# Team766/ros_vision

Hardware: AMD Instinct MI355X
Metric: frames/sec + p50 per-frame latency, 1280x720 AprilTag detect at 1/2/4/8 MI355X (higher is better)
Workload: dtype u8

## Files before the change

ros_vision_amd/csrc/at_api.cpp:

```cpp
#include <hip/hip_runtime.h>

#include <algorithm>
#include <chrono>
#include <cmath>
#include <cstdio>
#include <cstdlib>
#include <cstring>
#include <map>
#include <string>
#include <thread>
#include <vector>

#include "../../include/at_api.h"
#include "at_common.h"
#include "at_gp.h"
#include "at_mjpg.h"
#include "at_mjpg_entropy.h"

namespace at {
hipError_t launch_tap_sizes(const uint8_t* thr, const uint32_t* par, const uint32_t* size, uint32_t* out, int Wd,
                            int Hd, hipStream_t st);
hipError_t launch_tap_labels(const uint8_t* thr, const uint32_t* par, uint32_t* out, int Wd, int Hd, hipStream_t st);
hipError_t launch_gp_preprocess(const uint8_t* src, int w, int h, float* out, int ow, int oh, int c, hipStream_t st);
hipError_t launch_draw(const DrawPrim* prims, int n, uint32_t* last, uint8_t* bgr, int W, int H, hipStream_t st);
// ... 72 lines not shown
    fd.bitx[n] = (int8_t)(d / 2 + 1);
    fd.bity[n] = (int8_t)(d / 2 + 1);
  }
  return fd;
}
}

using namespace at;

static_assert(kMjpgInvalid == AT_E_INVALID && kMjpgUnsupported == AT_E_UNSUPPORTED && kMjpgOk == AT_OK,
              "at_mjpg.h carries the ABI's codes");
static_assert(kJpg420 == AT_JPEG_420 && kJpg422 == AT_JPEG_422 && kJpg444 == AT_JPEG_444 && AT_E_CAPACITY == -3,
              "at_mjpg.h carries the ABI's sampling codes");

enum { kCtlNpts, kCtlNpairs, kCtlNdets, kCtlNquads, kCtlStatus, kCtlNpent, kCtlNqcand, kCtlCclOvf, kCtlNlr,
       kCtlPerFrame };
enum { kCtlWorkhead = 0, kCtlQhead = 1, kCtlWorkheadSmall = 2, kCtlBlobPts = 3, kCtlNcls = 5,
       kCtlDetHead = kCtlNcls + kNumCls, kCtlDecDone = kCtlDetHead + 1, kCtlWorkheadMid = kCtlDecDone + 1,
       kCtlScalars = kCtlWorkheadMid + 1 };

static constexpr unsigned kTimingEventFlags = hipEventDisableSystemFence;

struct at_detector {
  at_config cfg;
  at_camera cam;
  Geom g;
  Params prm;
  int B;
  int device;
  int nblobwg;
  hipStream_t st;
  hipStream_t st2;
  hipEvent_t ev_fork, ev_join;
  DevBufs d;
  std::vector<void*> allocs;
  uint8_t* d_in;
  size_t in_stride;
  const uint8_t** h_ftab;
  uint32_t* d_ctrl;
  size_t ctrl_words;
  size_t kstamp_word;
  double wclk_khz;
  double kd_ms;
  long long kd_n;
  uint32_t* h_ctrl;
  DevDetection* h_dets;
  std::vector<int> res_idx, res_n;
  std::vector<const DevDetection*> res_base;
  std::vector<std::vector<DevDetection>> res_ovf;
  int last_nframes;
  int last_fmt;
  int last_gray;
  int last_sizes;
  int last_staged;
  int last_gp;
  int last_mj_color;
  int pending;
  hipEvent_t ev_done;
  hipEvent_t ev_ext;
  int use_graphs;
  std::map<int, hipGraphExec_t> graphs;
  struct SplitGraphs { hipGraphExec_t seg[3]; };
  std::map<int, SplitGraphs> split_graphs;
  std::vector<hipGraph_t> cap_segs;
  KernelTimer kt;
  double kt_ms;
  long long kt_n;
  int profiling;
  hipEvent_t ev_stage[kNumStages + 1];
  double stage_ms[kNumStages];
  long stage_batches;
  double host_wait_us, host_tail_us;
  DrawPrim* d_prims;
  size_t prims_cap;
  uint32_t* d_last;
  uint8_t* mj_host[2];
  uint8_t* d_mj;
  size_t mj_slot;
  int mj_cur;
  int mj_threads;
  std::vector<at::MjpgDecoder> mj_dec;
  std::vector<int> mj_rc;
  std::vector<size_t> mj_bytes;
  std::vector<uint8_t> mj_dense;
  uint64_t mj_stats[9];
  hipEvent_t ev_mj[3];
  int mj_timed;
  int mj_color;
  int mj_color_bufs;
  uint8_t* d_mj_planes;
  size_t mj_plane;
  uint8_t* d_mj_bgr;
  int mj_dev_ent;
  int mj_subseq;
  uint8_t* mj_ent_host[2];
  size_t mj_ent_cap;
  at::EntBufs ent;
  uint32_t* h_ent_info;
  int mj_ent_batch;
  hipEvent_t ev_ent[2];
  int mj_ent_timed;
  at::JpgBufs jpg;
  size_t jpg_out_cap;
  uint32_t* h_jpg_total;
  uint8_t jpg_hdr[at::kJpgHeaderMax];
  size_t jpg_hdr_len;
  int jpg_hdr_q, jpg_hdr_s;
  uint64_t jpg_stats[2];
  hipEvent_t ev_jpg[2];
  at::GpParseBufs gp;
  at::GpBox* h_gp_out;
  uint32_t* h_gp_info;
  uint64_t gp_stats[4];
  hipEvent_t ev_gp[2];
};

static const char* knob(const char* name) {
#ifdef AT_EXPERIMENTS
  return getenv(name);
#else
  (void)name;
  return nullptr;
#endif
}
static int knob_int(const char* name, int dflt) {
  const char* v = knob(name);
  return v ? atoi(v) : dflt;
}

static int hip_fail(hipError_t e) {
  if (e != hipSuccess) {
    fprintf(stderr, "at_api: HIP error %s\n", hipGetErrorString(e));
    return AT_E_HIP;
  }
  return AT_OK;
}
#define HIPCHK(x)                          \
  do {                                     \
    hipError_t e_ = (x);                   \
    if (e_ != hipSuccess) return hip_fail(e_); \
  } while (0)

extern "C" {

int at_abi_version(void) { return AT_ABI_VERSION; }

const char* at_strerror(int code) {
  switch (code) {
    case AT_OK: return "ok";
    case AT_E_INVALID: return "invalid argument or unsupported frame geometry";
    case AT_E_HIP: return "HIP runtime error";
    case AT_E_CAPACITY: return "frame exceeded a fixed capacity";
    case AT_E_FAMILY: return "unknown tag family";
    case AT_E_NOMEM: return "out of memory";
    case AT_E_UNSUPPORTED: return "unsupported JPEG stream (not baseline 8-bit 4:4:4 / 4:2:2 / 4:2:0 / gray)";
    default: return "unknown error";
  }
}

int at_family_num_known(const char* family) {
  const FamilyInfo* f = find_family(family);
  return f ? f->ncodes : AT_E_FAMILY;
}

int at_family_entry(const char* family, int i, int* id, uint64_t* code) {
  const FamilyInfo* f = find_family(family);
  if (!f) return AT_E_FAMILY;
  if (i < 0 || i >= f->ncodes) return AT_E_INVALID;
  if (id) *id = f->codes[i].id;
  if (code) *code = f->codes[i].code;
  return AT_OK;
}

int at_config_default(at_config* cfg, int width, int height) {
  if (!cfg) return AT_E_INVALID;
  memset(cfg, 0, sizeof(*cfg));
  cfg->width = width;
  cfg->height = height;
  cfg->family = "tag36h11";
  cfg->quad_decimate = 2.0f;
  cfg->refine_edges = 1;
  cfg->decode_sharpening = 0.25;
  cfg->min_white_black_diff = 5;
  cfg->min_cluster_pixels = 5;
  cfg->max_nmaxima = 10;
  cfg->max_line_fit_mse = 10.0f;
  cfg->cos_critical_rad = cos(10.0 * M_PI / 180.0);
  cfg->device = 0;
  cfg->max_batch = 1;
  cfg->tag_size = 0.1651;
  return AT_OK;
}

void at_destroy(at_detector* d) {
  if (!d) return;
  (void)hipSetDevice(d->device);
  if (d->st) (void)hipStreamSynchronize(d->st);
  if (d->st2) (void)hipStreamSynchronize(d->st2);
  for (auto& kv : d->graphs) (void)hipGraphExecDestroy(kv.second);
  d->graphs.clear();
  for (auto& kv : d->split_graphs)
    for (auto* g : kv.second.seg) (void)hipGraphExecDestroy(g);
  d->split_graphs.clear();
  for (void* p : d->allocs) (void)hipFree(p);
  if (d->h_ftab) (void)hipHostFree(d->h_ftab);
  if (d->h_ctrl) (void)hipHostFree(d->h_ctrl);
  if (d->h_dets) (void)hipHostFree(d->h_dets);
  if (d->d_prims) (void)hipFree(d->d_prims);
  if (d->d_last) (void)hipFree(d->d_last);
  for (uint8_t* p : d->mj_host)
    if (p) (void)hipHostFree(p);
  for (hipEvent_t e : d->ev_mj)
    if (e) (void)hipEventDestroy(e);
  for (uint8_t* p : d->mj_ent_host)
    if (p) (void)hipHostFree(p);
  if (d->h_ent_info) (void)hipHostFree(d->h_ent_info);
  for (hipEvent_t e : d->ev_ent)
    if (e) (void)hipEventDestroy(e);
  for (hipEvent_t e : d->ev_jpg)
    if (e) (void)hipEventDestroy(e);
  if (d->h_jpg_total) (void)hipHostFree(d->h_jpg_total);
  for (hipEvent_t e : d->ev_gp)
    if (e) (void)hipEventDestroy(e);
  if (d->h_gp_out) (void)hipHostFree(d->h_gp_out);
  if (d->h_gp_info) (void)hipHostFree(d->h_gp_info);
  if (d->ev_done) (void)hipEventDestroy(d->ev_done);
  if (d->ev_ext) (void)hipEventDestroy(d->ev_ext);
  for (int i = 0; i <= kNumStages; i++)
    if (d->ev_stage[i]) (void)hipEventDestroy(d->ev_stage[i]);
  if (d->kt.t0) (void)hipEventDestroy(d->kt.t0);
  if (d->kt.t1) (void)hipEventDestroy(d->kt.t1);
  if (d->ev_fork) (void)hipEventDestroy(d->ev_fork);
  if (d->ev_join) (void)hipEventDestroy(d->ev_join);
  if (d->st2) (void)hipStreamDestroy(d->st2);
  if (d->st) (void)hipStreamDestroy(d->st);
  delete d;
}

int at_create(const at_config* cfg, const at_camera* cam, at_detector** out) {
  if (!cfg || !cam || !out) return AT_E_INVALID;
  *out = nullptr;
  const FamilyInfo* fam = find_family(cfg->family);
  if (!fam || fam->ncodes > kMaxCodes) return AT_E_FAMILY;
  const int W = cfg->width, H = cfg->height;
  if (W <= 16 || H <= 16 || W % 8 || H % 8 || (long)W * H >= (1L << 22)) return AT_E_INVALID;
  if (cfg->quad_decimate != 2.0f || cfg->max_nmaxima != 10 || cfg->max_batch < 1 || cfg->max_batch > kMaxBatch)
    return AT_E_INVALID;
  if (2 * (W + H) > kSortCap) return AT_E_INVALID;
  int ndev = 0;
  if (hipGetDeviceCount(&ndev) != hipSuccess || ndev <= cfg->device) return AT_E_HIP;
  at_detector* d = new at_detector();
  d->cfg = *cfg;
  d->cfg.family = fam->name;
  d->cam = *cam;
  d->device = cfg->device;
  d->B = cfg->max_batch;
  d->mj_threads = 1;
  d->mj_subseq = at::kEntSubseqDefault;
  Geom& g = d->g;
  g.W = W; g.H = H; g.Wd = W / 2; g.Hd = H / 2;
  g.TW = g.Wd / 4; g.TH = g.Hd / 4;
  g.BW = g.Wd / 2; g.BH = g.Hd / 2;
  g.ctw = d->B < kWideBlobMaxBatch ? 32 : 64;
  if (knob("AT_CCL_TILE")) g.ctw = knob_int("AT_CCL_TILE", 64) == 32 ? 32 : 64;
  g.nlarge = g.ctw == 32 ? std::max(kNumLargeCls, std::min(kNumCls, knob_int("AT_NLARGE", kNumLargeCls)))
                        : kNumLargeCls;
  g.CTX = (g.Wd + g.ctw - 1) / g.ctw;
  g.CTY = (g.Hd + kCclTileH - 1) / kCclTileH;
  g.merge_cap = g.ctw == 64 ? std::min(kMergeCapMax, 80 * g.CTX * g.CTY) : 0;
  g.merge_lds = std::min(g.merge_cap * 12 + 8192, kMergeLdsMax);
  if (g.CTX * g.CTY > kMaxCclTiles) {
    at_destroy(d);
    return AT_E_INVALID;
  }
  g.cap_pts = 4 * (g.Wd - 2) * (g.Hd - 2);
  g.BTX = (g.Wd - 2 + 63) / 64;
  g.BTY = (g.Hd - 2 + 4 * kBndRows - 1) / (4 * kBndRows);
  g.ntb = g.BTX * g.BTY;
  g.bnd_region = kBndPts;
  g.bnd_region = std::max(kBndStage, std::min(kBndPts, knob_int("AT_BND_REGION", kBndPts)));
  if (g.ntb > kMaxTilesPerFrame) {
    at_destroy(d);
    return AT_E_INVALID;
  }
  g.min_cluster = (uint32_t)std::max(24, cfg->min_cluster_pixels);
  g.max_cluster = (uint32_t)(2 * (W + H));
  g.min_tag_width = std::max(3, (fam->d + 2) / 2);
  Params& p = d->prm;
  p.min_white_black_diff = cfg->min_white_black_diff;
  p.max_line_fit_mse = cfg->max_line_fit_mse;
  p.cos_critical_rad = cfg->cos_critical_rad;
  p.decode_sharpening = cfg->decode_sharpening;
  p.refine_edges = cfg->refine_edges;
  p.fx = cam->fx; p.fy = cam->fy; p.cx = cam->cx; p.cy = cam->cy;
  p.k1 = cam->k1; p.k2 = cam->k2; p.p1 = cam->p1; p.p2 = cam->p2; p.k3 = cam->k3;
  p.diag_stop = knob_int("AT_DIAG_BLOB_STOP", 0);
  p.probe = knob_int("AT_PHASE_PROBE", 0);
  p.taps = 0;
  p.wide_blob = knob_int("AT_WIDE_BLOB", 0);
  p.pipe_stop = knob_int("AT_DIAG_PIPE_STOP", 0);
  p.lblob_wg = knob("AT_LBLOB_WG") ? std::max(16, knob_int("AT_LBLOB_WG", 0)) : 0;
  p.sblob_wg = knob("AT_SBLOB_WG") ? std::max(16, knob_int("AT_SBLOB_WG", 0)) : 0;
  p.dec_wg = knob("AT_DEC_WG") ? std::max(16, knob_int("AT_DEC_WG", 0)) : 0;
  p.fam = family_desc(*fam);
  d->use_graphs = !knob_int("AT_NO_GRAPH", 0);
  if (!(cfg->tag_size >= 0) || !std::isfinite(cfg->tag_size)) {
    at_destroy(d);
    return AT_E_INVALID;
  }
  p.tag_size = cfg->tag_size;

  auto fail = [&](int code) {
    at_destroy(d);
    return code;
  };
  if (hipSetDevice(d->device) != hipSuccess) return fail(AT_E_HIP);
  if (hipStreamCreateWithFlags(&d->st, hipStreamNonBlocking) != hipSuccess) return fail(AT_E_HIP);
  if (hipEventCreateWithFlags(&d->ev_done, hipEventDisableTiming) != hipSuccess) return fail(AT_E_HIP);
  if (hipEventCreateWithFlags(&d->ev_ext, hipEventDisableTiming) != hipSuccess) return fail(AT_E_HIP);
  const bool fork = d->B < kWideBlobMaxBatch && !knob_int("AT_NO_FORK", 0);
  if (fork && hipStreamCreateWithFlags(&d->st2, hipStreamNonBlocking) != hipSuccess) return fail(AT_E_HIP);
  if (hipEventCreateWithFlags(&d->ev_fork, hipEventDisableTiming) != hipSuccess) return fail(AT_E_HIP);
  if (hipEventCreateWithFlags(&d->ev_join, hipEventDisableTiming) != hipSuccess) return fail(AT_E_HIP);
  d->kt.stage = -1;
  d->kt.split = nullptr;
  d->kt.ctx = nullptr;
  if (hipEventCreateWithFlags(&d->kt.t0, kTimingEventFlags) != hipSuccess ||
      hipEventCreateWithFlags(&d->kt.t1, kTimingEventFlags) != hipSuccess)
    return fail(AT_E_HIP);
  int ncu = 0;
  (void)hipDeviceGetAttribute(&ncu, hipDeviceAttributeMultiprocessorCount, d->device);
  int wclk = 0;
  (void)hipDeviceGetAttribute(&wclk, hipDeviceAttributeWallClockRate, d->device);
  d->wclk_khz = wclk > 0 ? (double)wclk : 100000.0;
  d->nblobwg = std::max(64, ncu * 2);
  if (knob("AT_BLOB_WG")) d->nblobwg = std::max(16, knob_int("AT_BLOB_WG", 0));

  const size_t B = (size_t)d->B;
  const size_t npix = (size_t)W * H, nd = (size_t)g.Wd * g.Hd, nt = (size_t)g.TW * g.TH * 2;
  bool oom = false;
  auto dalloc = [&](size_t bytes) -> void* {
    void* ptr = nullptr;
    if (hipMalloc(&ptr, std::max<size_t>(bytes, 256)) != hipSuccess) {
      oom = true;
      return nullptr;
    }
    d->allocs.push_back(ptr);
    return ptr;
  };
  d->in_stride = (npix * 3 + 255) & ~(size_t)255;
  d->d_in = (uint8_t*)dalloc(B * d->in_stride);
  DevBufs& b = d->d;
  b.gray = (uint8_t*)dalloc(B * npix);
  b.dec = (uint8_t*)dalloc(B * nd);
  b.mm = (uint8_t*)dalloc(B * nt);
  b.thr = (uint8_t*)dalloc(B * nd);
  b.par = (uint32_t*)dalloc(B * nd * 4);
  b.lroot = (uint32_t*)dalloc(B * (size_t)g.CTX * g.CTY * kCclTileNodesMax * 4);
  b.nlroot = (uint32_t*)dalloc(B * (size_t)g.CTX * g.CTY * 4);
  b.lcnt = (uint32_t*)dalloc(B * (size_t)g.CTX * g.CTY * kCclTileNodesMax * 4);
  b.cdesc = (uint32_t*)dalloc(B * (size_t)g.CTX * g.CTY * CclDesc::kWords * 4);
  b.size = (uint32_t*)dalloc(B * nd * 4);
  const size_t ntb = (size_t)g.ntb;
  b.pts = (uint64_t*)dalloc(B * ntb * (size_t)g.bnd_region * 8);
  b.tcnt = (uint32_t*)dalloc(B * ntb * 4);
  b.tent = (uint32_t*)dalloc(B * ntb * 4);
  b.grp = (uint32_t*)dalloc(B * g.cap_pts * 4);
  b.keys = (uint64_t*)dalloc(B * g.cap_pts * 8);
  b.pent_key = (uint64_t*)dalloc(B * ntb * kLdsPairSlots * 8);
  b.pent_cnt = (uint32_t*)dalloc(B * ntb * kLdsPairSlots * 4);
  b.povf_key = (uint64_t*)dalloc(B * kPairEntCap * 8);
  b.povf_cnt = (uint32_t*)dalloc(B * kPairEntCap * 4);
  b.ht_key = (uint64_t*)dalloc(B * kHashSlots * 8);
  b.ht_cnt = (uint32_t*)dalloc(B * kHashSlots * 4);
  b.ht_rank = (uint32_t*)dalloc(B * kHashSlots * 4);
  b.ht_off = (uint32_t*)dalloc(B * kHashSlots * 4);
  b.ht_cur = (uint32_t*)dalloc(B * kHashSlots * 4);
  b.pair_cnt = (uint32_t*)dalloc(B * kMaxPairs * 4);
  b.pair_off = (uint32_t*)dalloc(B * kMaxPairs * 4);
  b.pair_sel = (uint32_t*)dalloc(B * kMaxPairs * 4);
  b.wcap = (uint32_t)(B * kMaxPairs);
  b.work = (uint32_t*)dalloc((size_t)kNumCls * B * kMaxPairs * 4);
  b.probe = (uint64_t*)dalloc(kProbeWords * 8);
  b.dets = (DevDetection*)dalloc(B * kMaxDets * sizeof(DevDetection));
  b.det_work = (uint32_t*)dalloc(B * kMaxDets * 4);
  b.quads = (QuadRecord*)dalloc(B * kMaxPairs * sizeof(QuadRecord));
  b.qpend = (QuadPend*)dalloc(B * kMaxPairs * sizeof(QuadPend));
  d->kstamp_word = (kCtlPerFrame * B + kCtlScalars + 1) & ~(size_t)1;
  d->ctrl_words = d->kstamp_word + 5;
  d->d_ctrl = (uint32_t*)dalloc(((d->ctrl_words * 4 + 15) / 16) * 16);
  b.npts = d->d_ctrl + kCtlNpts * B;
  b.npairs = d->d_ctrl + kCtlNpairs * B;
  b.ndets = d->d_ctrl + kCtlNdets * B;
  b.nquads = d->d_ctrl + kCtlNquads * B;
  b.status = d->d_ctrl + kCtlStatus * B;
  b.npent = d->d_ctrl + kCtlNpent * B;
  b.qc_words = (uint32_t)(B * kQcStride);
  b.nqcand = (uint32_t*)dalloc((size_t)b.qc_words * 4);
  b.ccl_ovf = d->d_ctrl + kCtlCclOvf * B;
  b.nlr_tot = d->d_ctrl + kCtlNlr * B;
  uint32_t* sc = d->d_ctrl + kCtlPerFrame * B;
  b.workhead = sc + kCtlWorkhead;
  b.qhead = sc + kCtlQhead;
  b.workhead_small = sc + kCtlWorkheadSmall;
  b.workhead_mid = sc + kCtlWorkheadMid;
  b.blob_pts = sc + kCtlBlobPts;
  b.ncls = sc + kCtlNcls;
  b.det_head = sc + kCtlDetHead;
  b.dec_done = sc + kCtlDecDone;
  b.kt_stage = -1;
  b.kstamp = reinterpret_cast<uint64_t*>(d->d_ctrl + d->kstamp_word);
  b.kgrid = d->d_ctrl + d->kstamp_word + 4;
  b.kwg_cap = (uint32_t)(B * 1024 + 4096);
  b.kwg = (uint64_t*)dalloc((size_t)b.kwg_cap * 2 * 8);
  b.qcand_cap = (uint32_t)(B * kQuadCandPerFrame);
  b.qcand = (QuadCand*)dalloc((size_t)b.qcand_cap * sizeof(QuadCand));
  b.s_pk = (uint64_t*)dalloc((size_t)2 * d->nblobwg * (kSortCap / 2) * 8);
  b.rsamp = (double*)dalloc((size_t)decode_grid(d->nblobwg, d->B) * 2 * (kMaxRefineSamples - kLdsRefine) * 8);
  if (oom) return fail(AT_E_NOMEM);
  if (prepare_kernels(g) != hipSuccess) return fail(AT_E_HIP);
  if (hipHostMalloc((void**)&d->h_ftab, B * sizeof(void*), hipHostMallocMapped | hipHostMallocCoherent) != hipSuccess)
    return fail(AT_E_NOMEM);
  if (hipHostGetDevicePointer((void**)&b.frames, (void*)d->h_ftab, 0) != hipSuccess) return fail(AT_E_HIP);
  d->res_idx.assign(B * kMaxDets, 0);
  d->res_n.assign(B, 0);
  d->res_base.assign(B, nullptr);
  d->res_ovf.resize(B);
  if (hipHostMalloc((void**)&d->h_ctrl, d->ctrl_words * 4, hipHostMallocMapped) != hipSuccess) return fail(AT_E_NOMEM);
  if (hipHostMalloc((void**)&d->h_dets, B * kDetPoolPerFrame * sizeof(DevDetection), hipHostMallocMapped) != hipSuccess)
    return fail(AT_E_NOMEM);
  if (hipHostGetDevicePointer((void**)&b.hdets, d->h_dets, 0) != hipSuccess ||
      hipHostGetDevicePointer((void**)&b.hctrl, d->h_ctrl, 0) != hipSuccess)
    return fail(AT_E_HIP);
  b.ctrl = d->d_ctrl;
  b.ctrl_words = (uint32_t)d->ctrl_words;
  {
    std::vector<uint64_t> codes(fam->ncodes);
    std::vector<int32_t> ids(fam->ncodes);
    for (int i = 0; i < fam->ncodes; i++) {
      codes[i] = fam->codes[i].code;
      ids[i] = fam->codes[i].id;
    }
    uint64_t* dc = (uint64_t*)dalloc(codes.size() * 8);
    int32_t* di = (int32_t*)dalloc(ids.size() * 4);
    if (oom) return fail(AT_E_NOMEM);
    if (hipMemcpy(dc, codes.data(), codes.size() * 8, hipMemcpyHostToDevice) != hipSuccess ||
        hipMemcpy(di, ids.data(), ids.size() * 4, hipMemcpyHostToDevice) != hipSuccess)
      return fail(AT_E_HIP);
    b.book_code = dc;
    b.book_id = di;
  }
  if (hipMemsetAsync(b.size, 0, B * nd * 4, d->st) != hipSuccess) return fail(AT_E_HIP);
  if (hipStreamSynchronize(d->st) != hipSuccess) return fail(AT_E_HIP);
  *out = d;
  return AT_OK;
}

}

static bool seg_intersect(const double* a0, const double* a1, const double* b0, const double* b1) {
  const double ux = a1[0] - a0[0], uy = a1[1] - a0[1];
  const double vx = b1[0] - b0[0], vy = b1[1] - b0[1];
  const double den = ux * vy - uy * vx;
  if (fabs(den) < 1e-12) return false;
  const double t = ((b0[0] - a0[0]) * vy - (b0[1] - a0[1]) * vx) / den;
  const double w = ((b0[0] - a0[0]) * uy - (b0[1] - a0[1]) * ux) / den;
  return t >= 0 && t <= 1 && w >= 0 && w <= 1;
}
static bool poly_contains(const double poly[4][2], const double* pt) {
  bool inside = false;
  for (int i = 0, j = 3; i < 4; j = i++) {
    if (((poly[i][1] > pt[1]) != (poly[j][1] > pt[1])) &&
        (pt[0] < (poly[j][0] - poly[i][0]) * (pt[1] - poly[i][1]) / (poly[j][1] - poly[i][1]) + poly[i][0]))
      inside = !inside;
  }
  return inside;
}
static bool poly_overlap(const double a[4][2], const double b[4][2]) {
  for (int i = 0; i < 4; i++)
    for (int j = 0; j < 4; j++)
      if (seg_intersect(a[i], a[(i + 1) & 3], b[j], b[(j + 1) & 3])) return true;
  return poly_contains(a, b[0]) || poly_contains(b, a[0]);
}
static int prefer_smaller(int pref, double q0, double q1) {
  if (pref) return pref;
  if (q0 < q1) return -1;
  if (q1 < q0) return 1;
  return 0;
}

static void write_detection(const DevDetection& v, at_detection* o) {
  o->id = v.id;
  o->hamming = v.hamming;
  o->decision_margin = v.decision_margin;
  memcpy(o->H, v.H, sizeof(o->H));
  memcpy(o->c, v.c, sizeof(o->c));
  memcpy(o->p, v.p, sizeof(o->p));
}

static int host_tail(const DevDetection* cand, int* idx, int ncand, at_detection* out, int cap) {
  std::stable_sort(idx, idx + ncand, [&](int a, int b) { return cand[a].blob_rank < cand[b].blob_rank; });
  int n = ncand;
  for (int i0 = 0; i0 < n; i0++) {
    for (int i1 = i0 + 1; i1 < n; i1++) {
      const DevDetection& a = cand[idx[i0]];
      const DevDetection& b = cand[idx[i1]];
      if (a.id != b.id) continue;
      if (!poly_overlap(a.p, b.p)) continue;
      int pref = 0;
      pref = prefer_smaller(pref, a.hamming, b.hamming);
      pref = prefer_smaller(pref, -a.decision_margin, -b.decision_margin);
      for (int k = 0; k < 3; k++) pref = prefer_smaller(pref, a.H[k], b.H[k]);
      if (pref < 0) {
        if (i1 < n - 1) idx[i1] = idx[n - 1];
        n--;
        i1--;
      } else {
        if (i0 < n - 1) idx[i0] = idx[n - 1];
        n--;
        i0--;
        break;
      }
    }
  }
  std::stable_sort(idx, idx + n, [&](int a, int b) { return cand[a].id < cand[b].id; });
  for (int i = 0; i < n && i < cap; i++) write_detection(cand[idx[i]], out + i);
  return n;
}

static hipError_t record_sequence(at_detector* d, int nframes, int fmt, hipStream_t st, hipEvent_t* ev,
                                  const KernelTimer* kt) {
  hipError_t e;
  DevBufs b = d->d;
  b.kt_stage = kt ? kt->stage : -1;
  if ((e = launch_pipeline(b, d->g, d->prm, nframes, fmt, d->nblobwg, st, ev, d->st2, d->ev_fork, d->ev_join, kt)))
    return e;
  if (d->prm.tag_size > 0) return hipSuccess;
  return hipMemcpyAsync(d->h_ctrl, d->d_ctrl, d->ctrl_words * 4, hipMemcpyDeviceToHost, st);
}

static hipError_t split_capture(void* ctx, int ) {
  at_detector* d = (at_detector*)ctx;
  hipGraph_t g = nullptr;
  hipError_t e = hipStreamEndCapture(d->st, &g);
  if (e != hipSuccess) return e;
  d->cap_segs.push_back(g);
  return hipStreamBeginCapture(d->st, hipStreamCaptureModeThreadLocal);
}

static hipError_t instantiate(hipGraph_t g, hipGraphExec_t* exec) {
  const hipError_t e = hipGraphInstantiate(exec, g, nullptr, nullptr, 0);
  (void)hipGraphDestroy(g);
  return e;
}

static int enqueue_split(at_detector* d, int nframes, int fmt) {
  hipStream_t st = d->st;
  const int key = (nframes * 4 + fmt) * 32 + d->kt.stage;
  auto it = d->split_graphs.find(key);
  if (it == d->split_graphs.end()) {
    d->cap_segs.clear();
    KernelTimer kt = d->kt;
    kt.split = split_capture;
    kt.ctx = d;
    HIPCHK(hipStreamBeginCapture(st, hipStreamCaptureModeThreadLocal));
    hipError_t rec = record_sequence(d, nframes, fmt, st, nullptr, &kt);
    hipGraph_t last = nullptr;
    const hipError_t end = hipStreamEndCapture(st, &last);
    if (last) d->cap_segs.push_back(last);
    if (rec == hipSuccess && end == hipSuccess && d->cap_segs.size() != 3) rec = hipErrorInvalidValue;
    if (rec != hipSuccess || end != hipSuccess) {
      for (auto* g : d->cap_segs) (void)hipGraphDestroy(g);
      d->cap_segs.clear();
      HIPCHK(rec);
      HIPCHK(end);
    }
    at_detector::SplitGraphs sg{};
    hipError_t inst = hipSuccess;
    for (int i = 0; i < 3; i++) {
      const hipError_t r = instantiate(d->cap_segs[i], &sg.seg[i]);
      if (r != hipSuccess && inst == hipSuccess) inst = r;
    }
    d->cap_segs.clear();
    if (inst != hipSuccess) {
      for (auto* g : sg.seg)
        if (g) (void)hipGraphExecDestroy(g);
      HIPCHK(inst);
    }
    it = d->split_graphs.emplace(key, sg).first;
  }
  HIPCHK(hipGraphLaunch(it->second.seg[0], st));
  HIPCHK(hipEventRecord(d->kt.t0, st));
  HIPCHK(hipGraphLaunch(it->second.seg[1], st));
  HIPCHK(hipEventRecord(d->kt.t1, st));
  HIPCHK(hipGraphLaunch(it->second.seg[2], st));
  return AT_OK;
}

static int enqueue(at_detector* d, int nframes, int fmt) {
  hipStream_t st = d->st;
  const bool timed = d->kt.stage >= 0;
  const bool timed_on_fork = timed && d->st2 && (d->kt.stage == 8 || d->kt.stage == 9);
  if (d->profiling || !d->use_graphs || timed_on_fork) {
    HIPCHK(record_sequence(d, nframes, fmt, st, d->profiling ? d->ev_stage : nullptr, timed ? &d->kt : nullptr));
  } else if (timed) {
    const int rc = enqueue_split(d, nframes, fmt);
    if (rc != AT_OK) return rc;
  } else {
    const int key = nframes * 4 + fmt;
    auto it = d->graphs.find(key);
    if (it == d->graphs.end()) {
      hipGraph_t graph = nullptr;
      HIPCHK(hipStreamBeginCapture(st, hipStreamCaptureModeThreadLocal));
      const hipError_t rec = record_sequence(d, nframes, fmt, st, nullptr, nullptr);
      const hipError_t end = hipStreamEndCapture(st, &graph);
      HIPCHK(rec);
      HIPCHK(end);
      hipGraphExec_t exec = nullptr;
      HIPCHK(instantiate(graph, &exec));
      it = d->graphs.emplace(key, exec).first;
    }
    HIPCHK(hipGraphLaunch(it->second, st));
  }
  HIPCHK(hipEventRecord(d->ev_done, st));
  d->last_nframes = nframes;
  d->last_fmt = fmt;
  d->last_gray = fmt == AT_FMT_BGR8 || d->prm.taps;
  d->last_sizes = d->g.ctw == 32 || d->prm.taps;
  d->last_gp = d->prm.gp_c && fmt == AT_FMT_BGR8;
  d->last_mj_color = 0;
  d->mj_ent_batch = 0;
  d->pending = 1;
  return AT_OK;
}

static double now_us() {
  return std::chrono::duration<double, std::micro>(std::chrono::steady_clock::now().time_since_epoch()).count();
}

static int collect(at_detector* d, at_detection* out, int cap_per_frame, int* n_per_frame) {
  if (!d->pending) return AT_E_INVALID;
  const double t0 = now_us();
  HIPCHK(hipEventSynchronize(d->ev_done));
  const double t1 = now_us();
  d->host_wait_us += t1 - t0;
  d->pending = 0;
  if (d->profiling) {
    for (int i = 0; i < kNumStages; i++) {
      float ms = 0;
      HIPCHK(hipEventElapsedTime(&ms, d->ev_stage[i], d->ev_stage[i + 1]));
      d->stage_ms[i] += ms;
    }
    d->stage_batches++;
  }
  if (d->mj_timed) {
    float ms = 0;
    HIPCHK(hipEventElapsedTime(&ms, d->ev_mj[0], d->ev_mj[1]));
    d->mj_stats[4] = (uint64_t)((double)ms * 1e6);
    if (d->mj_timed == 2) {
      HIPCHK(hipEventElapsedTime(&ms, d->ev_mj[1], d->ev_mj[2]));
      d->mj_stats[5] = (uint64_t)((double)ms * 1e6);
    }
    d->mj_timed = 0;
  }
  if (d->mj_ent_timed) {
    float ms = 0;
    HIPCHK(hipEventElapsedTime(&ms, d->ev_ent[0], d->ev_ent[1]));
    d->mj_stats[6] = (uint64_t)((double)ms * 1e6);
    d->mj_ent_timed = 0;
  }
  if (d->mj_ent_batch) {
    uint32_t most = 0;
    for (int f = 0; f < d->last_nframes; f++) most = std::max(most, d->h_ent_info[(size_t)f * at::kEntInfoWords + 1]);
    d->mj_stats[8] = most;
  }
  if (d->kt.stage >= 0) {
    float ms = 0;
    HIPCHK(hipEventElapsedTime(&ms, d->kt.t0, d->kt.t1));
    d->kt_ms += ms;
    d->kt_n++;
    uint64_t st[2];
    memcpy(st, d->h_ctrl + d->kstamp_word, sizeof(st));
    st[0] = ~st[0];
    if (st[1] > st[0] && st[0] && d->wclk_khz > 0) {
      d->kd_ms += (double)(st[1] - st[0]) / d->wclk_khz;
      d->kd_n++;
    }
  }
  const int B = d->B;
  int rc = AT_OK;
  bool bad_entropy = false;
  const int nf = d->last_nframes;
  int* cnt = d->res_n.data();
  for (int f = 0; f < nf; f++) {
    cnt[f] = 0;
    if (n_per_frame) n_per_frame[f] = 0;
  }
  for (int f = 0; f < nf; f++) {
    const uint32_t status = d->h_ctrl[kCtlStatus * B + f];
    const int ncand = (int)std::min<uint32_t>(d->h_ctrl[kCtlNdets * B + f], kMaxDets);
    int* idx = d->res_idx.data() + (size_t)f * kMaxDets;
    int n = 0;
    if (status & kStatusPairsCapped) rc = AT_E_CAPACITY;
    if (d->mj_ent_batch && d->h_ent_info[(size_t)f * at::kEntInfoWords]) {
      bad_entropy = true;
    } else if (status & (kStatusPairsOverflow | kStatusHashFull | kStatusPointsOverflow | kStatusQuadsOverflow | kStatusDetsOverflow)) {
      rc = AT_E_CAPACITY;
    } else {
      const DevDetection* cand = d->h_dets + (size_t)f * kDetPoolPerFrame;
      if (ncand > kDetPoolPerFrame) {
        std::vector<DevDetection>& v = d->res_ovf[f];
        v.resize(ncand);
        HIPCHK(hipMemcpyAsync(v.data(), d->d.dets + (size_t)f * kMaxDets, ncand * sizeof(DevDetection),
                              hipMemcpyDeviceToHost, d->st));
        HIPCHK(hipStreamSynchronize(d->st));
        cand = v.data();
      }
      d->res_base[f] = cand;
      for (int i = 0; i < ncand; i++) idx[i] = i;
      n = host_tail(cand, idx, ncand, out ? out + (size_t)f * cap_per_frame : nullptr, out ? cap_per_frame : 0);
    }
// ... 1156 lines not shown
```

ros_vision_amd/csrc/at_common.h:

```cpp
#pragma once

#include <hip/hip_runtime.h>
#include <stdint.h>

#include "at_detmath.h"

namespace at {

template <int TW>
struct CclTile {
  static constexpr int W = TW, H = 32;
  static constexpr int BW = TW / 2, BH = H / 2;
  static constexpr int NT = BW * BH;
  static constexpr int NODES = 3 * NT;
  static constexpr int ROW_NODES = 3 * BW;
};
constexpr int kCclTileH = 32;
constexpr int kCclTileNodesMax = CclTile<64>::NODES;
constexpr int kHashSlots = 4096;
constexpr int kHashBits = 12;
constexpr int kPairEntCap = 65536;
constexpr int kBndRows = 4;
constexpr int kBndPts = 64 * 4 * kBndRows * 4;
constexpr int kBndStage = 2048;
constexpr int kLdsPairSlots = 512;
constexpr uint32_t kTileNarrow = 0x80000000u;
constexpr int kMaxTilesPerFrame = 1024;
constexpr int kMaxCclTiles = 1024;
struct CclDesc {
  static constexpr int Tthr = 0, Bthr = 16, Lthr = 32, Rthr = 40;
  static constexpr int TsF = 48, TsL = 64, TsR = 80, BsF = 96, BsL = 112, BsR = 128;
  static constexpr int LsF = 144, LsL = 152, RsF = 160, RsR = 168;
  static constexpr int kWords = 176;
};
constexpr int kMergeCapMax = 15360;
constexpr int kMergeLdsMax = kMergeCapMax * 10;
constexpr int kMaxPairs = 4096;
constexpr int kSortCap = 8192;
constexpr int kBlobThreads = 256;
constexpr int kWideBlobMaxBatch = 8;
constexpr int kSmallBlob = 512;
constexpr int kNMaxima = 10;
constexpr int kMaxRefineSamples = 1536;
#ifndef AT_LDS_REFINE
#define AT_LDS_REFINE 256
#endif
constexpr int kLdsRefine = AT_LDS_REFINE;
constexpr int kDecodeGridPerBlobWg = 8;
inline int decode_grid(int nblobwg, int B) {
  const int hi = nblobwg * kDecodeGridPerBlobWg, want = 64 * B;
  return nblobwg * 2 > (want < hi ? want : hi) ? nblobwg * 2 : (want < hi ? want : hi);
}

constexpr int kNumStages = 12;
constexpr const char* kStageNames[kNumStages] = {"k_pre",   "k_thr_ccl", "k_ccl_merge", "k_ccl_roots",
                                                 "k_boundary", "k_pairs", "k_group",     "k_extents",
                                                 "k_blob_small", "k_blob", "k_decode",   "k_pose"};

constexpr int kNumCls = 7;
constexpr int kNumLargeCls = 3;

constexpr uint32_t kStatusPairsOverflow = 1u;
constexpr uint32_t kStatusHashFull = 2u;
constexpr uint32_t kStatusDetsOverflow = 4u;
constexpr uint32_t kStatusPointsOverflow = 8u;
constexpr uint32_t kStatusQuadsOverflow = 16u;
constexpr uint32_t kStatusPairsCapped = 32u;
constexpr int kMaxBatch = 256;
constexpr int kQcStride = 32;
constexpr int kQuadCandPerFrame = kMaxPairs;
constexpr int kMaxDets = kQuadCandPerFrame;
constexpr int kDetPoolPerFrame = 128;
constexpr int kMaxCodes = 1024;
constexpr int kMaxFamilyBits = 64;

struct FamilyDesc {
  int nbits;
  int width_at_border;
  int total_width;
  int reversed_border;
  int ncodes;
  int8_t bitx[kMaxFamilyBits], bity[kMaxFamilyBits];
};

struct Geom {
  int W, H, Wd, Hd;
  int TW, TH;
  int BW, BH;
  int CTX, CTY;
  int ctw;
  int merge_cap;
  int merge_lds;
  int nlarge;
  int bnd_region;
  int cap_pts;
  int BTX, BTY, ntb;
  uint32_t min_cluster;
  uint32_t max_cluster;
  int min_tag_width;
};

struct Params {
  int min_white_black_diff;
  float max_line_fit_mse;
  double cos_critical_rad;
  double decode_sharpening;
  int refine_edges;
  double fx, fy, cx, cy, k1, k2, p1, p2, k3;
  int diag_stop;
  double tag_size;
  int probe;
  int taps;
  int wide_blob;
  int pipe_stop;
  int lblob_wg;
  int sblob_wg;
  int dec_wg;
  FamilyDesc fam;
  int gp_w, gp_h, gp_c;
};
constexpr int kProbeWords = 256;

#ifdef AT_EXPERIMENTS
#define AT_DIAG_STOP(prm, n) ((prm).diag_stop == (n))
#define AT_PIPE_STOP(prm) ((prm).pipe_stop)
#define AT_PROBE_ON(prm) ((prm).probe != 0)
#define AT_DIAG_ANY(prm) ((prm).diag_stop != 0)
#else
#define AT_DIAG_STOP(prm, n) false
#define AT_PIPE_STOP(prm) 0
#define AT_PROBE_ON(prm) false
#define AT_DIAG_ANY(prm) false
#endif

struct KernelTimer {
  int stage;
  hipEvent_t t0, t1;
  hipError_t (*split)(void* ctx, int which);
  void* ctx;
};

struct DevDetection {
  int32_t id;
  int16_t hamming;
  uint16_t frame;
  float decision_margin;
  int32_t blob_rank;
  double H[9];
  double c[2];
  double p[4][2];
  double pose_R[9];
  double pose_t[3];
  double pose_err[2];
};

struct QuadCand {
  uint32_t frame, rank;
  float p[4][2];
};

struct QuadRecord {
  uint32_t blob_index, valid, accepted;
  uint16_t indices[4];
  float corners[4][2];
};

struct Moments {
  int32_t Mx, My, W;
  int64_t Mxx, Myy, Mxy;
  int32_t N;
};

struct QuadPend {
  float fit[4][4];
  uint32_t blob_index, valid;
  uint16_t indices[4];
};
static_assert(sizeof(QuadPend) == 80, "QuadPend: 80 B per kept blob");

struct DrawPrim {
  double x0, y0, x1, y1;
  uint8_t bgr[3];
};

struct JpgBufs {
  int16_t* coef;
  const uint32_t* tab;
  uint32_t* blen;
  uint32_t* bits;
  size_t row_words;
  uint32_t* row_raw;
  uint32_t* row_len;
  uint8_t* out;
  uint32_t* total;
};

struct DevBufs {
  const uint8_t* const* frames;
  uint8_t* gray;
  uint8_t* dec;
  uint8_t* mm;
  uint8_t* thr;
  uint32_t* par;
  uint32_t* lroot;
  uint32_t* nlroot;
  uint32_t* lcnt;
  uint32_t* cdesc;
  uint32_t* ccl_ovf;
  uint32_t* nlr_tot;
  uint32_t* size;
  uint64_t* pts;
  uint32_t* tcnt;
  uint32_t* tent;
  uint32_t* grp;
  uint64_t* keys;
  uint64_t* pent_key;
  uint32_t* pent_cnt;
  uint64_t* povf_key;
  uint32_t* povf_cnt;
  uint32_t* npent;
  uint64_t* ht_key;
  uint32_t* ht_cnt;
  uint32_t* ht_rank;
  uint32_t* ht_off;
  uint32_t* ht_cur;
  uint32_t* pair_cnt;
  uint32_t* pair_off;
  uint32_t* pair_sel;
  uint32_t* work;
  uint32_t wcap;
  DevDetection* dets;
  uint32_t* det_work;
  uint32_t* det_head;
  uint32_t* dec_done;
  DevDetection* hdets;
  uint32_t* hctrl;
  uint32_t* ctrl;
  uint32_t ctrl_words;
  QuadRecord* quads;
  QuadPend* qpend;
  uint32_t* npts;
  uint32_t* npairs;
  uint32_t* ndets;
  uint32_t* nquads;
  uint32_t* status;
  uint32_t* ncls;
  uint32_t* workhead;
  uint64_t* probe;
  uint32_t* blob_pts;
  uint32_t* workhead_small;
  uint32_t* workhead_mid;
  uint32_t* nqcand;
  uint32_t qc_words;
  uint32_t* qhead;
  QuadCand* qcand;
  uint32_t qcand_cap;
  double* rsamp;
  const uint64_t* book_code;
  const int32_t* book_id;
  float* gp_out;
  int32_t kt_stage;
  uint64_t* kstamp;
  uint32_t* kgrid;
  uint64_t* kwg;
  uint32_t kwg_cap;
  uint64_t* s_pk;
};

}
```

ros_vision_amd/csrc/at_kernels.hip:

```cpp
#include <limits>
#include <hip/hip_runtime.h>

#include <float.h>
#include <math.h>
#include <stdint.h>

#include "at_common.h"
#include "at_gp.h"
#include "at_mjpg.h"
#include "at_mjpg_entropy.h"
#include "at_pose.h"


namespace at {

__device__ __forceinline__ uint32_t lane_id() { return __lane_id(); }
__device__ __attribute__((noinline)) float det_atan2f_call(float y, float x) { return det_atan2f(y, x); }

__device__ __forceinline__ uint64_t mix_hash(uint64_t k) {
  return (k * 0x9E3779B97F4A7C15ull) >> (64 - kHashBits);
}

__device__ __forceinline__ int dx_of(int dxy) { return dxy == 3 ? -1 : (dxy == 2 ? 0 : 1); }
__device__ __forceinline__ int dy_of(int dxy) { return dxy == 0 ? 0 : 1; }
// ... 1901 lines not shown
      const uint32_t key = lds ? e : 0x80000000u + lane;
      const bool same = lds && wave_shr1(key, 0xffffffffu) == key;
      const uint64_t same_mask = __ballot(same);
      const bool head = lds && !same;
      uint32_t start = 0;
      if (head) start = atomicAdd(&s_cur[e], run_len(same_mask, lane));
      const uint64_t heads = __ballot(head);
      const int hl = (heads & le) ? 63 - __builtin_clzll(heads & le) : (int)lane;
      const uint32_t s0 = (uint32_t)__shfl((int)start, hl);
      if (lds) grp[base + s0 + (lane - (uint32_t)hl)] = narrow_bits(w);
      else if (valid && base == kGrpFallback) place_global(b.pent_key[tb * kLdsPairSlots + e], narrow_bits(w));
    };
#pragma unroll
    for (int k = 0; k < kGrpPre; k++) {
      const uint32_t i = 2 * (tid + 256 * k);
      place((uint32_t)pv[k], i < n);
      place((uint32_t)(pv[k] >> 32), i + 1 < n);
    }
    for (uint32_t i0 = 512 * kGrpPre; i0 < n; i0 += 256) {
      const uint32_t i = i0 + tid;
      place(i < n ? pw[i] : 0u, i < n);
    }
    return;
  }
  for (int i = tid; i < 2 * kGrpEnt; i += 256) s_hk[i] = 0;
  __syncthreads();
  if (tid < kGrpEnt && (uint32_t)tid < ne && ebase != kGrpFallback) {
    s_base[tid] = ebase;
    s_cur[tid] = 0;
    uint32_t h = (uint32_t)(mix_hash(ekey) & (2 * kGrpEnt - 1));
    while (true) {
      const uint64_t prev = atomicCAS((unsigned long long*)&s_hk[h], 0ull, (unsigned long long)ekey);
      if (prev == 0) {
        s_he[h] = (uint32_t)tid;
        break;
      }
      h = (h + 1) & (2 * kGrpEnt - 1);
    }
  }
  __syncthreads();
  const uint32_t lane = lane_id();
  const uint64_t le = lane == 63 ? ~0ull : ((2ull << lane) - 1);
  auto place = [&](uint64_t key, bool valid) {
    const uint64_t r01 = key >> 24;
    uint32_t e = 0xffffffffu;
    if (valid) {
      uint32_t h = (uint32_t)(mix_hash(r01) & (2 * kGrpEnt - 1));
      for (int probe = 0; probe < 2 * kGrpEnt; probe++) {
        const uint64_t k = s_hk[h];
        if (k == r01) { e = s_he[h]; break; }
        if (k == 0) break;
        h = (h + 1) & (2 * kGrpEnt - 1);
      }
    }
    const uint32_t base = e != 0xffffffffu ? s_base[e] : kGrpDrop;
    const bool lds = base != kGrpDrop;
    const uint32_t ek = lds ? e : 0x80000000u + lane;
    const bool same = lds && wave_shr1(ek, 0xffffffffu) == ek;
    const uint64_t same_mask = __ballot(same);
    const bool head = lds && !same;
    uint32_t start = 0;
    if (head) start = atomicAdd(&s_cur[e], run_len(same_mask, lane));
    const uint64_t heads = __ballot(head);
    const int hl = (heads & le) ? 63 - __builtin_clzll(heads & le) : (int)lane;
    const uint32_t s0 = (uint32_t)__shfl((int)start, hl);
    if (lds) grp[base + s0 + (lane - (uint32_t)hl)] = (uint32_t)key & 0xffffffu;
    else if (valid && e == 0xffffffffu) place_global(r01, (uint32_t)key & 0xffffffu);
  };
#pragma unroll
  for (int k = 0; k < kGrpPre; k++) place(pv[k], (uint32_t)(tid + 256 * k) < n);
  for (uint32_t i0 = 256 * kGrpPre; i0 < n; i0 += 256) {
    const uint32_t i = i0 + tid;
    place(i < n ? pts[i] : 0ull, i < n);
  }
}

struct Ext {
  uint32_t min_x, min_y, max_x, max_y, count;
  int32_t gx_sum, gy_sum;
  int64_t pg_sum;
};

__device__ __forceinline__ double ext_cx(const Ext& e) { return (double)((float)(e.min_x + e.max_x) * 0.5f) + 0.05118; }
__device__ __forceinline__ double ext_cy(const Ext& e) {
  return (double)((float)(e.min_y + e.max_y) * 0.5f) + -0.028581;
}
__device__ __forceinline__ float ext_dot(const Ext& e) {
  const int64_t t = e.pg_sum * 2 - (int64_t)((int)(e.min_x + e.max_x) * e.gx_sum) -
                    (int64_t)((int)(e.min_y + e.max_y) * e.gy_sum);
  const double a = (double)t * 0.5;
  const double bq = 0.05118 * (double)e.gx_sum;
  const double c = 0.028581 * (double)e.gy_sum;
  return (float)(a - bq + c);
}

__device__ __forceinline__ int32_t lf_weight(int32_t gx, int32_t gy) {
  const uint32_t sq = (uint32_t)(gx * gx + gy * gy);
  uint32_t r = (uint32_t)__builtin_amdgcn_sqrtf((float)sq);
  r -= r * r > sq ? 1u : 0u;
  r += (r + 1) * (r + 1) <= sq ? 1u : 0u;
  return (int32_t)r + 1;
}

__device__ __forceinline__ void line_normal(float d, float c, float h, double* lp23) {
  const float nx1 = d - h, ny1 = c;
  const float M1 = nx1 * nx1 + ny1 * ny1;
  const float nx2 = c, ny2 = -d - h;
  const float M2 = nx2 * nx2 + ny2 * ny2;
  float nx, ny;
  if (M1 > M2) { nx = nx1; ny = ny1; } else { nx = nx2; ny = ny2; }
  const float len = det_hypotf(nx, ny);
  lp23[0] = (double)(nx / len);
  lp23[1] = (double)(ny / len);
}

__device__ void fit_line(const Moments& m, double* lp01, double* lp23, double* err, double* mse, float* pre = nullptr) {
  const int64_t W = m.W;
  const int64_t Cxx = (int64_t)((uint64_t)m.Mxx * (uint64_t)W - (uint64_t)((int64_t)m.Mx * (int64_t)m.Mx));
  const int64_t Cxy = (int64_t)((uint64_t)m.Mxy * (uint64_t)W - (uint64_t)((int64_t)m.Mx * (int64_t)m.My));
  const int64_t Cyy = (int64_t)((uint64_t)m.Myy * (uint64_t)W - (uint64_t)((int64_t)m.My * (int64_t)m.My));
  const float d = (float)(Cxx - Cyy), c = (float)(2 * Cxy);
  const float px = (float)m.Mx / (float)(m.W * 2), py = (float)m.My / (float)(m.W * 2);
  if (pre) {
    pre[0] = d; pre[1] = c; pre[2] = px; pre[3] = py;
    return;
  }
  const float h = det_hypotf(d, c);
  const float e8 = (float)((double)(W * W) * 8.0);
  const float eig = ((float)(Cxx + Cyy) - h) / e8;
  if (lp01) {
    lp01[0] = (double)px;
    lp01[1] = (double)py;
  }
  if (lp23) line_normal(d, c, h, lp23);
  *err = (double)((float)m.N * eig);
  *mse = (double)eig;
}

template <int NT>
__device__ __forceinline__ void team_sync() {
  if constexpr (NT == 64) {
    __builtin_amdgcn_fence(__ATOMIC_RELEASE, "wavefront");
    __builtin_amdgcn_wave_barrier();
    __builtin_amdgcn_fence(__ATOMIC_ACQUIRE, "wavefront");
  } else {
    __syncthreads();
  }
}

template <int NT>
__device__ __forceinline__ int team_rank() {
  return NT == 64 ? (int)lane_id() : (int)threadIdx.x;
}

template <int NT, typename T, typename Op>
__device__ T team_reduce(T v, Op op, T* s_tmp) {
  if constexpr (NT == 64) {
    return wave_reduce(v, op);
  } else {
    return block_reduce(v, op, s_tmp, NT / 64);
  }
}

template <int NT, typename T>
__device__ T team_incl_scan(T v, T* s_tmp, T* total) {
  if constexpr (NT == 64) {
    v = wave_incl_scan(v, AddOp(), T(0));
    *total = wave_read(v, 63);
    return v;
  } else {
    return block_incl_scan(v, s_tmp, total, NT / 64);
  }
}

template <typename T, int NT>
__device__ void team_bitonic_sort(T* s, int n) {
  const int r = team_rank<NT>();
  for (int k = 2; k <= n; k <<= 1) {
    for (int j = k >> 1; j > 0; j >>= 1) {
      for (int i = r; i < n; i += NT) {
        const int ixj = i ^ j;
        if (ixj > i) {
          const T a = s[i], c = s[ixj];
          const bool up = (i & k) == 0;
          if ((a > c) == up) {
            s[i] = c;
            s[ixj] = a;
          }
        }
      }
      team_sync<NT>();
    }
  }
}


__device__ void redistort(const Params& p, double* x, double* y) {
  const double xP = (*x - p.cx) / p.fx, yP = (*y - p.cy) / p.fy;
  const double rSq = xP * xP + yP * yP;
  const double lin = 1 + p.k1 * rSq + p.k2 * rSq * rSq + p.k3 * rSq * rSq * rSq;
  const double xPP = xP * lin + 2 * p.p1 * xP * yP + p.p2 * (rSq + 2 * xP * xP);
  const double yPP = yP * lin + p.p1 * (rSq + 2 * yP * yP) + 2 * p.p2 * xP * yP;
  *x = xPP * p.fx + p.cx;
  *y = yPP * p.fy + p.cy;
}

__device__ void undistort(const Params& p, double* u, double* v) {
  const double xPP = (*u - p.cx) / p.fx, yPP = (*v - p.cy) / p.fy;
  double xP = xPP, yP = yPP;
  const double x0 = xP, y0 = yP;
  double prev_x, prev_y;
  int it = 0;
  do {
    prev_x = xP;
    prev_y = yP;
    const double rSq = xP * xP + yP * yP;
    const double rad = 1 + (p.k1 * rSq) + (p.k2 * rSq * rSq) + (p.k3 * rSq * rSq * rSq);
    const double rinv = 1 / rad;
    const double tdx = 2 * p.p1 * xP * yP + p.p2 * (rSq + p.k3 * rSq * rSq * rSq);
    const double tdy = p.p1 * (rSq + 2 * yP * yP) + 2 * p.p2 * xP * yP;
    xP = (x0 - tdx) * rinv;
    yP = (y0 - tdy) * rinv;
    if (it > 100) break;
    it++;
  } while (fabs(xP - prev_x) > 1e-6 || fabs(yP - prev_y) > 1e-6);
  *u = xP * p.fx + p.cx;
  *v = yP * p.fy + p.cy;
}

__device__ void hproject(const double* H, double x, double y, double* ox, double* oy) {
  const double xx = H[0] * x + H[1] * y + H[2];
  const double yy = H[3] * x + H[4] * y + H[5];
  const double zz = H[6] * x + H[7] * y + H[8];
  *ox = xx / zz;
  *oy = yy / zz;
}

__device__ int homography_wave(const float (*qc)[2], double* A, double* H) {
  const int lane = (int)lane_id();
  for (int e = lane; e < 72; e += 64) {
    const int row = e / 9, col = e % 9, i = row >> 1;
    const double c0 = (i == 0 || i == 3) ? -1 : 1, c1 = (i == 0 || i == 1) ? -1 : 1;
    const double c2 = qc[i][0], c3 = qc[i][1];
    const int k = (row & 1) ? col - 3 : col;
    const double cz = (row & 1) ? c3 : c2;
    double v = 0;
    if (k == 0) v = c0;
    else if (k == 1) v = c1;
    else if (k == 2) v = 1;
    if (col == 6) v = -c0 * cz;
    else if (col == 7) v = -c1 * cz;
    else if (col == 8) v = cz;
    A[e] = v;
  }
  team_sync<64>();
  for (int col = 0; col < 8; col++) {
    double v = -1.0;
    int row = 64;
    if (lane < 8 - col) {
      row = col + lane;
      v = fabs(A[row * 9 + col]);
      if (!(v > 0.0)) { v = -1.0; row = 64; }
    }
#pragma unroll
    for (int d = 1; d < 8; d <<= 1) {
      const double ov = __shfl_xor(v, d);
      const int orow = __shfl_xor(row, d);
      if (ov > v || (ov == v && orow < row)) { v = ov; row = orow; }
    }
    v = __shfl(v, 0);
    row = __shfl(row, 0);
    if (!(v >= 1e-10)) return -1;
    if (row != col && lane <= 8 - col) {
      const int i = col + lane;
      const double t = A[col * 9 + i];
      A[col * 9 + i] = A[row * 9 + i];
      A[row * 9 + i] = t;
    }
    team_sync<64>();
    const int nc = 8 - col;
    if (lane < (7 - col) * nc) {
      const int i = col + 1 + lane / nc, j = col + 1 + lane % nc;
      const double fct = A[i * 9 + col] / A[col * 9 + col];
      A[i * 9 + j] -= fct * A[col * 9 + j];
    }
    team_sync<64>();
  }
  double x[8];
#pragma unroll
  for (int col = 7; col >= 0; col--) {
    double sum = 0;
#pragma unroll
    for (int i = col + 1; i < 8; i++) sum += A[col * 9 + i] * x[i];
    x[col] = (A[col * 9 + 8] - sum) / A[col * 9 + col];
  }
#pragma unroll
  for (int k = 0; k < 8; k++)
    if (lane == k) H[k] = x[k];
  if (lane == 8) H[8] = 1;
  team_sync<64>();
  return 0;
}

struct GrayModel {
  double A[3][3], B[3], C[3];
};
__device__ void gm_add(GrayModel& g, double x, double y, double gray) {
  g.A[0][0] += x * x; g.A[0][1] += x * y; g.A[0][2] += x;
  g.A[1][1] += y * y; g.A[1][2] += y; g.A[2][2] += 1;
  g.B[0] += x * gray; g.B[1] += y * gray; g.B[2] += gray;
}
__device__ void gm_solve(GrayModel& g) {
  const double* A = &g.A[0][0];
  double L[9], M[9];
  L[0] = sqrt(A[0]); L[3] = A[1] / L[0]; L[6] = A[2] / L[0];
  L[4] = sqrt(A[4] - L[3] * L[3]); L[7] = (A[5] - L[3] * L[6]) / L[4];
  L[8] = sqrt(A[8] - L[6] * L[6] - L[7] * L[7]);
  M[0] = 1 / L[0]; M[3] = -L[3] * M[0] / L[4]; M[4] = 1 / L[4];
  M[6] = (-L[6] * M[0] - L[7] * M[3]) / L[8]; M[7] = -L[7] * M[4] / L[8]; M[8] = 1 / L[8];
  const double t0 = M[0] * g.B[0];
  const double t1 = M[3] * g.B[0] + M[4] * g.B[1];
  const double t2 = M[6] * g.B[0] + M[7] * g.B[1] + M[8] * g.B[2];
  g.C[0] = M[0] * t0 + M[3] * t1 + M[6] * t2;
  g.C[1] = M[4] * t1 + M[7] * t2;
  g.C[2] = M[8] * t2;
}
__device__ __forceinline__ double gm_interp(const GrayModel& g, double x, double y) {
  return g.C[0] * x + g.C[1] * y + g.C[2];
}

__constant__ uint8_t c_combo[210][4] = {{0,1,2,3},{0,1,2,4},{0,1,2,5},{0,1,2,6},{0,1,2,7},{0,1,2,8},{0,1,2,9},{0,1,3,4},{0,1,3,5},{0,1,3,6},{0,1,3,7},{0,1,3,8},{0,1,3,9},{0,1,4,5},{0,1,4,6},{0,1,4,7},{0,1,4,8},{0,1,4,9},{0,1,5,6},{0,1,5,7},{0,1,5,8},{0,1,5,9},{0,1,6,7},{0,1,6,8},{0,1,6,9},{0,1,7,8},{0,1,7,9},{0,1,8,9},{0,2,3,4},{0,2,3,5},{0,2,3,6},{0,2,3,7},{0,2,3,8},{0,2,3,9},{0,2,4,5},{0,2,4,6},{0,2,4,7},{0,2,4,8},{0,2,4,9},{0,2,5,6},{0,2,5,7},{0,2,5,8},{0,2,5,9},{0,2,6,7},{0,2,6,8},{0,2,6,9},{0,2,7,8},{0,2,7,9},{0,2,8,9},{0,3,4,5},{0,3,4,6},{0,3,4,7},{0,3,4,8},{0,3,4,9},{0,3,5,6},{0,3,5,7},{0,3,5,8},{0,3,5,9},{0,3,6,7},{0,3,6,8},{0,3,6,9},{0,3,7,8},{0,3,7,9},{0,3,8,9},{0,4,5,6},{0,4,5,7},{0,4,5,8},{0,4,5,9},{0,4,6,7},{0,4,6,8},{0,4,6,9},{0,4,7,8},{0,4,7,9},{0,4,8,9},{0,5,6,7},{0,5,6,8},{0,5,6,9},{0,5,7,8},{0,5,7,9},{0,5,8,9},{0,6,7,8},{0,6,7,9},{0,6,8,9},{0,7,8,9},{1,2,3,4},{1,2,3,5},{1,2,3,6},{1,2,3,7},{1,2,3,8},{1,2,3,9},{1,2,4,5},{1,2,4,6},{1,2,4,7},{1,2,4,8},{1,2,4,9},{1,2,5,6},{1,2,5,7},{1,2,5,8},{1,2,5,9},{1,2,6,7},{1,2,6,8},{1,2,6,9},{1,2,7,8},{1,2,7,9},{1,2,8,9},{1,3,4,5},{1,3,4,6},{1,3,4,7},{1,3,4,8},{1,3,4,9},{1,3,5,6},{1,3,5,7},{1,3,5,8},{1,3,5,9},{1,3,6,7},{1,3,6,8},{1,3,6,9},{1,3,7,8},{1,3,7,9},{1,3,8,9},{1,4,5,6},{1,4,5,7},{1,4,5,8},{1,4,5,9},{1,4,6,7},{1,4,6,8},{1,4,6,9},{1,4,7,8},{1,4,7,9},{1,4,8,9},{1,5,6,7},{1,5,6,8},{1,5,6,9},{1,5,7,8},{1,5,7,9},{1,5,8,9},{1,6,7,8},{1,6,7,9},{1,6,8,9},{1,7,8,9},{2,3,4,5},{2,3,4,6},{2,3,4,7},{2,3,4,8},{2,3,4,9},{2,3,5,6},{2,3,5,7},{2,3,5,8},{2,3,5,9},{2,3,6,7},{2,3,6,8},{2,3,6,9},{2,3,7,8},{2,3,7,9},{2,3,8,9},{2,4,5,6},{2,4,5,7},{2,4,5,8},{2,4,5,9},{2,4,6,7},{2,4,6,8},{2,4,6,9},{2,4,7,8},{2,4,7,9},{2,4,8,9},{2,5,6,7},{2,5,6,8},{2,5,6,9},{2,5,7,8},{2,5,7,9},{2,5,8,9},{2,6,7,8},{2,6,7,9},{2,6,8,9},{2,7,8,9},{3,4,5,6},{3,4,5,7},{3,4,5,8},{3,4,5,9},{3,4,6,7},{3,4,6,8},{3,4,6,9},{3,4,7,8},{3,4,7,9},{3,4,8,9},{3,5,6,7},{3,5,6,8},{3,5,6,9},{3,5,7,8},{3,5,7,9},{3,5,8,9},{3,6,7,8},{3,6,7,9},{3,6,8,9},{3,7,8,9},{4,5,6,7},{4,5,6,8},{4,5,6,9},{4,5,7,8},{4,5,7,9},{4,5,8,9},{4,6,7,8},{4,6,7,9},{4,6,8,9},{4,7,8,9},{5,6,7,8},{5,6,7,9},{5,6,8,9},{5,7,8,9},{6,7,8,9}};

__constant__ uint8_t c_colex[210] = {0,1,7,28,84,2,8,29,85,13,34,90,49,105,140,3,9,30,86,14,35,91,50,106,141,18,39,95,54,110,145,64,120,155,175,4,10,31,87,15,36,92,51,107,142,19,40,96,55,111,146,65,121,156,176,22,43,99,58,114,149,68,124,159,179,74,130,165,185,195,5,11,32,88,16,37,93,52,108,143,20,41,97,56,112,147,66,122,157,177,23,44,100,59,115,150,69,125,160,180,75,131,166,186,196,25,46,102,61,117,152,71,127,162,182,77,133,168,188,198,80,136,171,191,201,205,6,12,33,89,17,38,94,53,109,144,21,42,98,57,113,148,67,123,158,178,24,45,101,60,116,151,70,126,161,181,76,132,167,187,197,26,47,103,62,118,153,72,128,163,183,78,134,169,189,199,81,137,172,192,202,206,27,48,104,63,119,154,73,129,164,184,79,135,170,190,200,82,138,173,193,203,207,83,139,174,194,204,208,209};

struct LineFitOut {
  double err, mse;
  double p01[2], p23[2];
};

template <bool kP01, bool kP23>
__device__ __forceinline__ LineFitOut fit_line_v(const Moments& m) {
  LineFitOut o;
  fit_line(m, kP01 ? o.p01 : nullptr, kP23 ? o.p23 : nullptr, &o.err, &o.mse);
  return o;
}

struct Mom6 {
  uint32_t Mx, My, W;
  uint64_t Mxx, Myy, Mxy;
};
__device__ __forceinline__ Mom6 mom_zero() { return Mom6{0, 0, 0, 0, 0, 0}; }
__device__ __forceinline__ void mom_add(Mom6& a, const Mom6& c) {
  a.Mx += c.Mx; a.My += c.My; a.W += c.W; a.Mxx += c.Mxx; a.Myy += c.Myy; a.Mxy += c.Mxy;
}
__device__ __forceinline__ void mom_sub(Mom6& a, const Mom6& c) {
  a.Mx -= c.Mx; a.My -= c.My; a.W -= c.W; a.Mxx -= c.Mxx; a.Myy -= c.Myy; a.Mxy -= c.Mxy;
}
__device__ __forceinline__ Mom6 mom_shfl(const Mom6& m, int src) {
  Mom6 r;
  r.Mx = __shfl(m.Mx, src); r.My = __shfl(m.My, src); r.W = __shfl(m.W, src);
  r.Mxx = __shfl(m.Mxx, src); r.Myy = __shfl(m.Myy, src); r.Mxy = __shfl(m.Mxy, src);
  return r;
}
__device__ __forceinline__ Mom6 mom_shfl_up(const Mom6& m, int d) {
  Mom6 r;
  r.Mx = __shfl_up(m.Mx, d); r.My = __shfl_up(m.My, d); r.W = __shfl_up(m.W, d);
  r.Mxx = __shfl_up(m.Mxx, d); r.Myy = __shfl_up(m.Myy, d); r.Mxy = __shfl_up(m.Mxy, d);
  return r;
}

constexpr int kKeyTheta = 32;

__device__ __forceinline__ uint32_t compact_word(uint64_t sk) {
  return (uint32_t)((sk >> 10) & 0x3ff) | ((uint32_t)((sk >> 20) & 0x3ff) << 10) | ((uint32_t)((sk >> 30) & 3) << 20) |
         ((uint32_t)(sk & 0x1ff) << 22);
}

__device__ __forceinline__ Mom6 point_mom(uint32_t cw) {
  const int dxy = (int)((cw >> 20) & 3);
  const uint32_t ix2 = (cw & 0x3ff) * 2 + dx_of(dxy) + 1;
  const uint32_t iy2 = ((cw >> 10) & 0x3ff) * 2 + dy_of(dxy) + 1;
  const uint32_t Wt = cw >> 22;
  Mom6 m;
  m.Mx = Wt * ix2;
  m.My = Wt * iy2;
  m.W = Wt;
  m.Mxx = (uint64_t)(int64_t)(int32_t)(Wt * ix2 * ix2);
  m.Mxy = (uint64_t)(int64_t)(int32_t)(Wt * ix2 * iy2);
  m.Myy = (uint64_t)(int64_t)(int32_t)(Wt * iy2 * iy2);
  return m;
}

__device__ __forceinline__ Moments to_moments(const Mom6& s, int32_t N) {
  Moments m;
  m.Mx = (int32_t)s.Mx; m.My = (int32_t)s.My; m.W = (int32_t)s.W;
  m.Mxx = (int64_t)s.Mxx; m.Myy = (int64_t)s.Myy; m.Mxy = (int64_t)s.Mxy;
  m.N = N;
  return m;
}

__device__ __forceinline__ float window_err(const Mom6& s, int32_t N) {
  const Moments m = to_moments(s, N);
  const uint64_t Wl = (uint32_t)m.W;
  const int64_t Cxx = (int64_t)((uint64_t)m.Mxx * Wl - (uint64_t)((int64_t)m.Mx * (int64_t)m.Mx));
  const int64_t Cxy = (int64_t)((uint64_t)m.Mxy * Wl - (uint64_t)((int64_t)m.Mx * (int64_t)m.My));
  const int64_t Cyy = (int64_t)((uint64_t)m.Myy * Wl - (uint64_t)((int64_t)m.My * (int64_t)m.My));
  auto tof = [](int64_t v) { return (float)(double)v; };
  const float h = det_hypotf(tof(Cxx - Cyy), tof(2 * Cxy));
  const float eig = (tof(Cxx + Cyy) - h) / (float)(8u * (uint32_t)Wl * (uint32_t)Wl);
  return (float)m.N * eig;
}


template <int NT, int CAP>
constexpr int kKeySlots = (NT >= 512 && CAP <= 4096) ? 2 * CAP
                          : CAP < 400 ? 400
                                      : CAP;

struct SegFits {
  double err[kNMaxima][kNMaxima];
  double mse[kNMaxima][kNMaxima];
  double p[kNMaxima][kNMaxima][2];
};

template <int NT, int CAP>
struct BlobShared {
  uint64_t keys[kKeySlots<NT, CAP>];
  uint32_t bcnt[kKeySlots<NT, CAP> / 4];
  uint64_t pks[16];
  uint64_t wtop[NT > 64 ? NT / 64 * 10 : 1];
  uint32_t tMx[21], tMy[21], tW[21];
  uint64_t tMxx[21], tMyy[21], tMxy[21];
  uint32_t bMx[NT > 64 ? NT : 1], bMy[NT > 64 ? NT : 1], bW[NT > 64 ? NT : 1];
  uint64_t bMxx[NT > 64 ? NT : 1], bMyy[NT > 64 ? NT : 1], bMxy[NT > 64 ? NT : 1];
  Mom6 wsum[NT / 64];
  int64_t red7[NT / 64][8];
  double red_f64[16];
  uint32_t red_u32[16];
  uint32_t red_idx[16];
  uint32_t item, nwork, npeaks;
  int32_t pi[16];
  double lines[4][4];
  uint32_t pacc[22];
  uint32_t ph[10];
  uint32_t slow_dt, slow_n, slow_ph[10];
  uint64_t t_last, t_item;
};

constexpr uint64_t kThetaSpan = 50265600;

template <int NT, int CAP>
__device__ bool team_bucket_sort(BlobShared<NT, CAP>& S, int n) {
  constexpr int KEYS = kKeySlots<NT, CAP>;
  if (n < 64 || 2 * n > KEYS) return false;
  const int tid = team_rank<NT>();
  int nb = 32;
  while (2 * nb < n) nb <<= 1;
  auto bucket = [&](uint64_t k) { return (uint32_t)(((k >> kKeyTheta) * (uint64_t)nb) / kThetaSpan); };
  uint32_t* bcnt = S.bcnt;
  for (int i = tid; i < nb / 2; i += NT) bcnt[i] = 0;
  team_sync<NT>();
  for (int t = tid; t < n; t += NT) {
    const uint32_t bk = bucket(S.keys[t]);
    atomicAdd(&bcnt[bk >> 1], 1u << ((bk & 1) * 16));
  }
  team_sync<NT>();
  const int per = nb >= NT ? nb / NT : 1;
  const int b0 = tid * per;
  uint32_t loc = 0, mx = 0;
  uint32_t cval[16];
#pragma unroll
  for (int j = 0; j < 16; j++) {
    cval[j] = 0;
    if (j < per && b0 + j < nb) {
      const uint32_t bb = (uint32_t)(b0 + j);
      cval[j] = (bcnt[bb >> 1] >> ((bb & 1) * 16)) & 0xffffu;
      loc += cval[j];
      mx = cval[j] > mx ? cval[j] : mx;
    }
  }
  uint32_t tot;
  const uint32_t incl = team_incl_scan<NT>(loc, S.red_u32, &tot);
  mx = team_reduce<NT>(mx, MaxOp(), S.red_u32);
  if (mx > 32) return false;
  team_sync<NT>();
  uint32_t run = incl - loc;
#pragma unroll
  for (int j = 0; j < 16; j++) {
    if (j < per && b0 + j < nb && (j & 1) == 0) {
      const uint32_t bb = (uint32_t)(b0 + j);
      if (per >= 2) {
        const uint32_t s0 = run, s1 = run + cval[j];
        bcnt[bb >> 1] = s0 | (s1 << 16);
      }
    }
    if (j < per && b0 + j < nb) run += cval[j];
  }
  if (per == 1 && b0 < nb) {
    const uint32_t mine = incl - loc;
    const uint32_t other = __shfl_down(mine, 1);
    if ((b0 & 1) == 0) bcnt[b0 >> 1] = mine | (other << 16);
  }
  team_sync<NT>();
  uint64_t* T = S.keys + KEYS / 2;
  for (int t = tid; t < n; t += NT) {
    const uint64_t k = S.keys[t];
    const uint32_t bk = bucket(k);
    const uint32_t old = atomicAdd(&bcnt[bk >> 1], 1u << ((bk & 1) * 16));
    T[(old >> ((bk & 1) * 16)) & 0xffffu] = k;
  }
  team_sync<NT>();
  for (int s = tid; s < n; s += NT) {
    const uint64_t k = T[s];
    const uint32_t bk = bucket(k);
    int lo = s, hi = s + 1;
    while (lo > 0 && bucket(T[lo - 1]) == bk) lo--;
    while (hi < n && bucket(T[hi]) == bk) hi++;
    int r = lo;
    for (int j = lo; j < hi; j++) r += T[j] < k;
    S.keys[r] = k;
  }
  team_sync<NT>();
  return true;
}

template <bool kGlob>
__device__ __forceinline__ uint64_t pk_get(const uint64_t* lds, const uint64_t* gpk, int cap, int i) {
  if constexpr (kGlob) return i < cap ? lds[i] : gpk[i - cap];
  else return lds[i];
}
template <bool kGlob>
__device__ __forceinline__ void pk_put(uint64_t* lds, uint64_t* gpk, int cap, int i, uint64_t v) {
  if constexpr (kGlob) {
    if (i < cap) lds[i] = v;
    else gpk[i - cap] = v;
  } else {
    lds[i] = v;
  }
}
template <int NT, bool kGlob>
__device__ void team_bitonic_sort_pk(uint64_t* lds, uint64_t* gpk, int cap, int n) {
  const int r = team_rank<NT>();
  for (int k = 2; k <= n; k <<= 1) {
    for (int j = k >> 1; j > 0; j >>= 1) {
      for (int i = r; i < n; i += NT) {
        const int ixj = i ^ j;
        if (ixj > i) {
          const uint64_t a = pk_get<kGlob>(lds, gpk, cap, i), c = pk_get<kGlob>(lds, gpk, cap, ixj);
          const bool up = (i & k) == 0;
          if ((a > c) == up) {
            pk_put<kGlob>(lds, gpk, cap, i, c);
            pk_put<kGlob>(lds, gpk, cap, ixj, a);
          }
        }
      }
      team_sync<NT>();
    }
  }
}

template <int NT, int CAP>
__device__ __forceinline__ void team_extents(BlobShared<NT, CAP>& S, uint32_t& mnx, uint32_t& mxx, uint32_t& mny,
                                             uint32_t& mxy, int32_t& sgx, int32_t& sgy, int64_t& spg) {
  mnx = wave_reduce(mnx, MinOp()); mxx = wave_reduce(mxx, MaxOp());
  mny = wave_reduce(mny, MinOp()); mxy = wave_reduce(mxy, MaxOp());
  sgx = wave_reduce(sgx, AddOp()); sgy = wave_reduce(sgy, AddOp());
  spg = wave_reduce(spg, AddOp());
  if constexpr (NT > 64) {
    const int w = threadIdx.x >> 6;
    team_sync<NT>();
    if (lane_id() == 0) {
      S.red7[w][0] = mnx; S.red7[w][1] = mxx; S.red7[w][2] = mny; S.red7[w][3] = mxy;
      S.red7[w][4] = sgx; S.red7[w][5] = sgy; S.red7[w][6] = spg;
    }
    team_sync<NT>();
    for (int i = 0; i < NT / 64; i++) {
      mnx = min(mnx, (uint32_t)S.red7[i][0]); mxx = max(mxx, (uint32_t)S.red7[i][1]);
      mny = min(mny, (uint32_t)S.red7[i][2]); mxy = max(mxy, (uint32_t)S.red7[i][3]);
    }
    int32_t gx = 0, gy = 0;
    int64_t pg = 0;
    for (int i = 0; i < NT / 64; i++) {
      gx += (int32_t)S.red7[i][4]; gy += (int32_t)S.red7[i][5]; pg += S.red7[i][6];
    }
    sgx = gx; sgy = gy; spg = pg;
  }
}

template <int NT, int CAP>
__device__ __forceinline__ Mom6 team_excl_scan_mom(BlobShared<NT, CAP>& S, const Mom6& v, Mom6* total) {
  const uint32_t lane = lane_id();
  Mom6 incl;
  incl.Mx = wave_incl_scan(v.Mx, AddOp(), 0u);
  incl.My = wave_incl_scan(v.My, AddOp(), 0u);
  incl.W = wave_incl_scan(v.W, AddOp(), 0u);
  incl.Mxx = wave_incl_scan(v.Mxx, AddOp(), (uint64_t)0);
  incl.Myy = wave_incl_scan(v.Myy, AddOp(), (uint64_t)0);
  incl.Mxy = wave_incl_scan(v.Mxy, AddOp(), (uint64_t)0);
  Mom6 ex = incl;
  mom_sub(ex, v);
  if constexpr (NT > 64) {
    const int w = threadIdx.x >> 6;
    team_sync<NT>();
    if (lane == 63) S.wsum[w] = incl;
    team_sync<NT>();
    Mom6 tot = mom_zero();
// ... 1151 lines not shown
    [[clang::always_inline]] blob_item<64, CAP, FUSE>(b, g, prm, S, nullptr, s_combo, w, pi, pacc);
    w = w1;
    pi = pi1;
    w1 = w2;
  }
  probe_flush(b, prm, pacc, 64, lane == 0);
  probe_flush_slow(b, prm, S, lane == 0);
  if (lane == 0 && pacc[20]) atomicAdd(b.blob_pts + 0, pacc[20]);
  if (lane == 0 && pacc[21]) atomicAdd(b.nquads, pacc[21]);
}

template <int NT, int CAP, bool FUSE = false>
__global__ __launch_bounds__(NT) __attribute__((amdgpu_waves_per_eu(NT == 256 && CAP == 4096 && !FUSE ? 3 : 1))) void k_blob(DevBufs b, Geom g, Params prm, uint32_t nlo, int c0, int c1, int launch) {
  __shared__ BlobShared<NT, CAP> S;
  const int tid = threadIdx.x;
  uint32_t kt_slot = ~0u;
  if (!launch) {
    kt_begin(b, 9);
  } else if (b.kt_stage == 9 && tid == 0) {
    kt_slot = atomicAdd(b.kgrid, 1u);
    if (kt_slot < b.kwg_cap) b.kwg[kt_slot] = wall_clock64();
  }
  __shared__ uint32_t s_combo[420], s_cnt[kNumCls];
  load_combos(s_combo, tid, NT);
  if (tid < kNumCls) s_cnt[tid] = min(b.ncls[tid], b.wcap);
  large_blob_loop<NT, CAP, FUSE>(b, g, prm, S, s_combo, s_cnt, nlo, blockIdx.x, c0, c1, launch);
  if (tid == 0 && !launch) kt_end(b, 9);
  if (tid == 0 && launch && kt_slot < b.kwg_cap) b.kwg[b.kwg_cap + kt_slot] = wall_clock64();
}

#ifndef AT_BS_WAVES
#define AT_BS_WAVES 4
#endif

template <bool FUSE, int CAP = kSmallBlob, int WAVES = AT_BS_WAVES, int STAGE = 8>
__global__ __launch_bounds__(256) __attribute__((amdgpu_waves_per_eu(FUSE ? 2 : WAVES))) void k_blob_small(DevBufs b, Geom g, Params prm,
                                                                                                         int c0, int c1, int launch) {
  __shared__ BlobShared<64, CAP> Ss[4];
  const int wave = threadIdx.x >> 6;
  uint32_t kt_slot = ~0u;
  if (!launch) {
    kt_begin(b, STAGE);
  } else if (b.kt_stage == STAGE && threadIdx.x == 0) {
    kt_slot = atomicAdd(b.kgrid, 1u);
    if (kt_slot < b.kwg_cap) b.kwg[kt_slot] = wall_clock64();
  }
  __shared__ uint32_t s_combo[420], s_cnt[kNumCls];
  load_combos(s_combo, threadIdx.x, 256);
  if (threadIdx.x < kNumCls) s_cnt[threadIdx.x] = min(b.ncls[threadIdx.x], b.wcap);
  __syncthreads();
  small_blob_loop<FUSE, CAP>(b, g, prm, Ss[wave], s_combo, s_cnt, blockIdx.x * 4 + wave, gridDim.x * 4, c0, c1);
  if (b.kt_stage == STAGE) {
    __syncthreads();
    if (threadIdx.x == 0 && !launch) kt_end(b, STAGE);
    if (threadIdx.x == 0 && launch && kt_slot < b.kwg_cap) b.kwg[b.kwg_cap + kt_slot] = wall_clock64();
  }
}

__global__ __launch_bounds__(512) void k_blob_lat(DevBufs b, Geom g, Params prm) {
  using SL = BlobShared<512, 4096>;
  using SS = BlobShared<64, kSmallBlob>;
  static_assert(8 * sizeof(SS) <= sizeof(SL), "eight small-blob waves fit in a large team's LDS");
  __shared__ __attribute__((aligned(16))) unsigned char s_raw[sizeof(SL)];
  __shared__ uint32_t s_combo[420], s_cnt[kNumCls];
  const int tid = threadIdx.x;
  kt_begin(b, 9);
  load_combos(s_combo, tid, 512);
  if (tid < kNumCls) s_cnt[tid] = min(b.ncls[tid], b.wcap);
  const uint32_t team = blockIdx.x >> 1, nteam = gridDim.x >> 1;
  if ((blockIdx.x & 1) == 0) {
    large_blob_loop<512, 4096, true>(b, g, prm, *reinterpret_cast<SL*>(s_raw), s_combo, s_cnt, 0u, team, 0, g.nlarge, 0);
  } else {
    __syncthreads();
    const int wave = tid >> 6;
    small_blob_loop<true>(b, g, prm, reinterpret_cast<SS*>(s_raw)[wave], s_combo, s_cnt, team * 8 + wave, nteam * 8,
                          g.nlarge, kNumCls);
  }
  if (b.kt_stage == 9) {
    __syncthreads();
    if (tid == 0) kt_end(b, 9);
  }
}

__global__ __launch_bounds__(256) void k_quad_fin(DevBufs b, Geom g, Params prm, int c0, int c1) {
  __shared__ uint32_t s_cnt[kNumCls];
  if (threadIdx.x < kNumCls) s_cnt[threadIdx.x] = min(b.ncls[threadIdx.x], b.wcap);
  __syncthreads();
  uint32_t nwork = 0;
  for (int c = c0; c < c1; c++) nwork += s_cnt[c];
  const uint32_t lane = lane_id(), base = lane & ~3u;
  const int k = (int)(lane & 3);
  auto from = [&](double v, int j) { return __shfl(v, (int)base + j); };
  auto fromf = [&](float v, int j) { return __shfl(v, (int)base + j); };
  auto quad_or = [&](int v) {
    v |= __shfl_xor(v, 1);
    return v | __shfl_xor(v, 2);
  };
  for (uint32_t it = (blockIdx.x * 256 + threadIdx.x) >> 2; it < nwork; it += gridDim.x * 64) {
    uint32_t w = 0;
    work_item(b, s_cnt, c0, c1, it, &w);
    const uint32_t f = w >> 16, rank = w & 0xffff;
    const size_t slot = (size_t)f * kMaxPairs + rank;
    if (b.pair_sel[slot] == 0) continue;
    const QuadPend& qp = b.qpend[slot];
    const bool valid = qp.valid != 0;
    float cx = 0.f, cy = 0.f;
    int bad = 0;
    {
      double l[4] = {0, 0, 0, 0};
      if (valid) {
        const float4 pre = *reinterpret_cast<const float4*>(qp.fit[k]);
        l[0] = (double)pre.z;
        l[1] = (double)pre.w;
        line_normal(pre.x, pre.y, det_hypotf(pre.x, pre.y), l + 2);
      }
      double m[4];
#pragma unroll
      for (int j = 0; j < 4; j++) m[j] = from(l[j], (k + 1) & 3);
      if (valid) {
        const double A00 = l[3], A01 = -m[3];
        const double A10 = -l[2], A11 = m[2];
        const double B0 = -l[0] + m[0];
        const double B1 = -l[1] + m[1];
        const double det = A00 * A11 - A10 * A01;
        const double W00 = A11 / det, W01 = -A01 / det;
        if (fabs(det) < 0.001) {
          bad = 1;
        } else {
          const double L0 = W00 * B0 + W01 * B1;
          cx = (float)(l[0] + L0 * A00);
          cy = (float)(l[1] + L0 * A10);
        }
      }
    }
    bool ok = valid && !quad_or(bad);
    float qc[4][2];
#pragma unroll
    for (int j = 0; j < 4; j++) {
      qc[j][0] = fromf(cx, j);
      qc[j][1] = fromf(cy, j);
    }
    if (ok) {
      auto side = [&](int j) {
        const int a2 = j == 0 ? 0 : j == 1 ? 1 : j == 2 ? 2 : j == 3 ? 2 : j == 4 ? 3 : 0;
        const int b2 = j == 0 ? 1 : j == 1 ? 2 : j == 2 ? 0 : j == 3 ? 3 : j == 4 ? 0 : 2;
        return det_hypotf(qc[b2][0] - qc[a2][0], qc[b2][1] - qc[a2][1]);
      };
      const float s0 = side(k), s1 = side(4 + (k & 1));
      float len[6];
#pragma unroll
      for (int j = 0; j < 4; j++) len[j] = fromf(s0, j);
      len[4] = fromf(s1, 0);
      len[5] = fromf(s1, 1);
      float area = 0, pp;
      pp = (len[0] + len[1] + len[2]) / 2;
      area += sqrtf(pp * (pp - len[0]) * (pp - len[1]) * (pp - len[2]));
      pp = (len[3] + len[4] + len[5]) / 2;
      area += sqrtf(pp * (pp - len[3]) * (pp - len[4]) * (pp - len[5]));
      if ((double)area < 0.95 * g.min_tag_width * g.min_tag_width) ok = false;
    }
    if (ok) {
      const int i0 = k, i1 = (i0 + 1) & 3, i2 = (i0 + 2) & 3;
      const float dx1 = qc[i1][0] - qc[i0][0], dy1 = qc[i1][1] - qc[i0][1];
      const float dx2 = qc[i2][0] - qc[i1][0], dy2 = qc[i2][1] - qc[i1][1];
      const float cosd = (dx1 * dx2 + dy1 * dy2) / sqrtf((dx1 * dx1 + dy1 * dy1) * (dx2 * dx2 + dy2 * dy2));
      const int abad = (double)fabsf(cosd) > prm.cos_critical_rad || dx1 * dy2 < dy1 * dx2;
      if (quad_or(abad)) ok = false;
    }
    if (k == 0) {
      QuadRecord rec;
      rec.blob_index = qp.blob_index;
      rec.valid = valid;
      for (int j = 0; j < 4; j++) rec.indices[j] = qp.indices[j];
      QuadCand qcand;
      for (int j = 0; j < 4; j++) {
        const float x = ok ? (qc[j][0] - 0.5f) * 2.0f + 0.5f : 0.f;
        const float y = ok ? (qc[j][1] - 0.5f) * 2.0f + 0.5f : 0.f;
        rec.corners[j][0] = qcand.p[j][0] = x;
        rec.corners[j][1] = qcand.p[j][1] = y;
      }
      rec.accepted = ok;
      if (prm.taps) b.quads[slot] = rec;
      if (ok && !AT_DIAG_STOP(prm, 5)) {
        qcand.frame = f;
        qcand.rank = rank;
        const uint32_t ci = atomicAdd(b.nqcand + (size_t)f * kQcStride, 1u);
        if (ci < (uint32_t)kQuadCandPerFrame) b.qcand[(size_t)f * kQuadCandPerFrame + ci] = qcand;
        else atomicOr(b.status + f, kStatusQuadsOverflow);
      }
    }
  }
}

constexpr int kDecodeThreads = 64;
__device__ __forceinline__ void border_pattern(int p, float wab, float& x0, float& y0, float& dx, float& dy) {
  const float far_ = (p & 1) ? wab - 0.5f : wab + 0.5f;
  const float near_ = (p & 1) ? 0.5f : -0.5f;
  const int side = p >> 1;
  const float a = (side == 0 || side == 2) ? near_ : far_;
  if (side < 2) { x0 = a; y0 = 0.5f; dx = 0; dy = 1; }
  else { x0 = 0.5f; y0 = a; dx = 1; dy = 0; }
}

__device__ __forceinline__ uint64_t rotate90_n(uint64_t w, int nbits) {
  int p = nbits;
  uint64_t l = 0;
  if (nbits % 4 == 1) { p = nbits - 1; l = 1; }
  w = ((w >> l) << (p / 4 + l)) | (w >> (3 * p / 4 + l) << l) | (w & l);
  return w & ((1ull << nbits) - 1);
}
constexpr int kMaxTotalWidth = 12;

__device__ __forceinline__ double readlane_f64(double v, int l) {
  const uint64_t u = __builtin_bit_cast(uint64_t, v);
  const uint32_t lo = (uint32_t)__builtin_amdgcn_readlane((int)(uint32_t)u, l);
  const uint32_t hi = (uint32_t)__builtin_amdgcn_readlane((int)(uint32_t)(u >> 32), l);
  return __builtin_bit_cast(double, (uint64_t)lo | ((uint64_t)hi << 32));
}
__constant__ double c_rot_c[4] = {1.0, 6.123233995736766e-17, -1.0, -1.8369701987210297e-16};
__constant__ double c_rot_s[4] = {0.0, 1.0, 1.2246467991473532e-16, -1.0};

struct DecodeShared {
  double sx[kLdsRefine], sy[kLdsRefine];
  float qc[4][2];
  int nsamp[4], samp_off[4];
  float enx[4], eny[4];
  double lines[4][4];
  double H[9];
  double A[72];
  double gmx[64], gmy[64], gmv[64];
  int gmvalid[64];
  double wC[3], bC[3];
  double values[kMaxTotalWidth * kMaxTotalWidth];
  int ok;
  uint32_t item;
  uint32_t qpre[kMaxBatch + 1];
};

struct PoseHandoff {
  double H[9], p[4][2];
  double R[9], t[3], err[2];
  uint32_t seq, ack, exit;
};
__device__ void pose_worker(PoseHandoff& P, const Params& prm) {
  const uint32_t lane = lane_id();
  uint32_t seen = 0;
  while (true) {
    uint32_t sq;
    bool done = false;
    while ((sq = __hip_atomic_load(&P.seq, __ATOMIC_ACQUIRE, __HIP_MEMORY_SCOPE_WORKGROUP)) == seen) {
      if (__hip_atomic_load(&P.exit, __ATOMIC_ACQUIRE, __HIP_MEMORY_SCOPE_WORKGROUP)) { done = true; break; }
      __builtin_amdgcn_s_sleep(1);
    }
    if (done) return;
    seen = sq;
    double H[9], pc[4][2];
#pragma unroll
    for (int k = 0; k < 9; k++) H[k] = P.H[k];
#pragma unroll
    for (int k = 0; k < 4; k++) { pc[k][0] = P.p[k][0]; pc[k][1] = P.p[k][1]; }
    double R[9], t[3], err[2];
    pose::estimate_tag_pose<true>(H, pc, prm.fx, prm.fy, prm.cx, prm.cy, prm.tag_size, R, t, err, (int)(lane & 3));
    if (lane == 0) {
#pragma unroll
      for (int k = 0; k < 9; k++) P.R[k] = R[k];
#pragma unroll
      for (int k = 0; k < 3; k++) P.t[k] = t[k];
      P.err[0] = err[0];
      P.err[1] = err[1];
      __hip_atomic_store(&P.ack, seen, __ATOMIC_RELEASE, __HIP_MEMORY_SCOPE_WORKGROUP);
    }
  }
}
__device__ void decode_finish(const DevBufs& b, int lane, uint32_t nq) {
  const uint32_t nwg = min(gridDim.x, nq);
  if (blockIdx.x >= max(nwg, 1u)) return;
  uint32_t last = nwg == 0;
  if (lane == 0 && nwg) {
    __threadfence();
    last = atomicAdd(b.dec_done, 1u) == nwg - 1;
  }
  last = __shfl(last, 0);
  if (!last) return;
  __threadfence();
  for (uint32_t w = (uint32_t)lane; w < b.ctrl_words; w += 64)
    b.hctrl[w] = __hip_atomic_load(b.ctrl + w, __ATOMIC_RELAXED, __HIP_MEMORY_SCOPE_AGENT);
}

#ifndef AT_BIG_BLOB_WG
#define AT_BIG_BLOB_WG 256
#endif
#ifndef AT_BIG_NT
#define AT_BIG_NT 512
#endif
#ifndef AT_FORK_SMALL
#define AT_FORK_SMALL 1
#endif
#ifndef AT_POSE_IN_DECODE
#define AT_POSE_IN_DECODE 1
#endif
#ifndef AT_DEC_WAVES
#define AT_DEC_WAVES 4
#endif
template <bool POSE>
__global__ __launch_bounds__(POSE ? 128 : kDecodeThreads) __attribute__((amdgpu_waves_per_eu(POSE ? 1 : AT_DEC_WAVES))) void k_decode(DevBufs b, Geom g, Params prm, int B, int fmt) {
  constexpr int RCAP = kMaxRefineSamples;
  __shared__ DecodeShared S;
  __shared__ PoseHandoff P;
  const int tid = threadIdx.x;
  kt_begin(b, 10);
  if (POSE) {
    if (tid == 0) { P.seq = 0; P.ack = 0; P.exit = 0; }
    __syncthreads();
    if (tid >= 64) {
      pose_worker(P, prm);
      return;
    }
  }
  double* gsx = b.rsamp + (size_t)blockIdx.x * (2 * (kMaxRefineSamples - kLdsRefine));
  double* gsy = gsx + (kMaxRefineSamples - kLdsRefine);
  uint32_t* qpre = S.qpre;
  {
    uint32_t c[kMaxBatch / 64], sum = 0;
#pragma unroll
    for (int k = 0; k < kMaxBatch / 64; k++) {
      const int f = tid * (kMaxBatch / 64) + k;
      c[k] = f < B ? min(b.nqcand[(size_t)f * kQcStride], (uint32_t)kQuadCandPerFrame) : 0u;
      sum += c[k];
    }
    const uint32_t incl = wave_incl_scan(sum, AddOp(), 0u);
    uint32_t acc = incl - sum;
#pragma unroll
    for (int k = 0; k < kMaxBatch / 64; k++) {
      const int f = tid * (kMaxBatch / 64) + k;
      if (f < B) qpre[f] = acc;
      acc += c[k];
    }
    if (tid == 63) qpre[B] = incl;
  }
  team_sync<64>();
  const uint32_t nq = qpre[B];

  uint32_t pacc[21] = {0};
  uint64_t t_last = 0;
  auto phase = [&](int k) {
    if (AT_PROBE_ON(prm) && tid == 0) {
      const uint64_t now = wall_clock64();
      if (k > 0) {
        pacc[k] += (uint32_t)(now - t_last);
        pacc[10 + k] += 1;
      }
      t_last = now;
    }
  };
  const uint32_t G = gridDim.x;
  uint32_t pose_seq = 0;
  struct ItemPre {
    int f;
    uint32_t rank;
    float px, py;
    const uint8_t* gsrc;
  };
  auto prefetch = [&](uint32_t it) -> ItemPre {
    int lo = 0, hi = B - 1;
    while (lo < hi) {
      const int mid = (lo + hi + 1) >> 1;
      if (qpre[mid] <= it) lo = mid;
      else hi = mid - 1;
    }
    const QuadCand* q = &b.qcand[(size_t)lo * kQuadCandPerFrame + (it - qpre[lo])];
    ItemPre p;
    p.f = lo;
    p.rank = q->rank;
    p.px = tid < 4 ? q->p[tid & 3][0] : 0.f;
    p.py = tid < 4 ? q->p[tid & 3][1] : 0.f;
    p.gsrc = fmt == 1 ? b.gray + (size_t)lo * g.W * g.H : b.frames[lo];
    return p;
  };
  ItemPre nxt = {};
  if (blockIdx.x < nq) nxt = prefetch(blockIdx.x);
  for (uint32_t item = blockIdx.x; item < nq; item += G) {
    const ItemPre cur = nxt;
    if (item + G < nq) nxt = prefetch(item + G);
    const int f = cur.f;
    const uint32_t qrank = cur.rank;
    const uint8_t* gsrc = cur.gsrc;
    const int gsh = fmt == 0 ? 1 : 0;
    auto pix = [&](size_t i) -> uint32_t { return gsrc[i << gsh]; };
    if (tid < 4) { S.qc[tid][0] = cur.px; S.qc[tid][1] = cur.py; }
    team_sync<64>();
    phase(0);
    if (prm.refine_edges) {
      if (tid < 4) {
        const int a2 = tid, b2 = (tid + 1) & 3;
        float nx = S.qc[b2][1] - S.qc[a2][1];
        float ny = -S.qc[b2][0] + S.qc[a2][0];
        const float mag = sqrtf(nx * nx + ny * ny);
        nx /= mag;
        ny /= mag;
        const int nsf = (int)(mag / 8);
        S.nsamp[tid] = nsf > 16 ? nsf : 16;
        S.enx[tid] = nx;
        S.eny[tid] = ny;
      }
      team_sync<64>();
      if (tid == 0) {
        int acc = 0;
        for (int k = 0; k < 4; k++) { S.samp_off[k] = acc; acc += S.nsamp[k]; }
      }
      team_sync<64>();
      const int total = min(S.samp_off[3] + S.nsamp[3], RCAP);
      if (tid == 0 && S.samp_off[3] + S.nsamp[3] > RCAP) atomicOr(b.status + f, kStatusQuadsOverflow);
      for (int t = tid; t < total; t += kDecodeThreads) {
        int edge = 0;
        while (edge < 3 && t >= S.samp_off[edge + 1]) edge++;
        const int s = t - S.samp_off[edge];
        const int a2 = edge, b2 = (edge + 1) & 3;
        const int nsamples = S.nsamp[edge];
        const float nx = S.enx[edge], ny = S.eny[edge];
        const double alpha = (1.0 + s) / (nsamples + 1);
        const double x0 = alpha * S.qc[a2][0] + (1 - alpha) * S.qc[b2][0];
        const double y0 = alpha * S.qc[a2][1] + (1 - alpha) * S.qc[b2][1];
        constexpr int kSteps = 25;
        int g1v[kSteps], g2v[kSteps];
#pragma unroll
        for (int k = 0; k < kSteps; k++) {
          const double nn = -3.0 + 0.25 * k;
          const int x1 = (int)(x0 + (nn + 1) * nx);
          const int y1 = (int)(y0 + (nn + 1) * ny);
          const int x2 = (int)(x0 + (nn - 1) * nx);
          const int y2 = (int)(y0 + (nn - 1) * ny);
          const bool in = !(x1 < 0 || x1 >= g.W || y1 < 0 || y1 >= g.H) && !(x2 < 0 || x2 >= g.W || y2 < 0 || y2 >= g.H);
          g1v[k] = -1;
          g2v[k] = 0;
          if (in) {
            g1v[k] = (int)pix((size_t)y1 * g.W + x1);
            g2v[k] = (int)pix((size_t)y2 * g.W + x2);
          }
        }
        double Mn = 0, Mcount = 0;
#pragma unroll
        for (int k = 0; k < kSteps; k++) {
          const double nn = -3.0 + 0.25 * k;
          const int g1 = g1v[k], g2 = g2v[k];
          if (g1 < g2) continue;
          const double weight = (double)((g2 - g1) * (g2 - g1));
          Mn += weight * nn;
          Mcount += weight;
        }
        double bx = __longlong_as_double(0x7ff8deadbeef0000ll), by = 0;
        if (Mcount != 0) {
          const double n0 = Mn / Mcount;
          bx = x0 + n0 * nx;
          by = y0 + n0 * ny;
          undistort(prm, &bx, &by);
        }
        if (t < kLdsRefine) {
          S.sx[t] = bx;
          S.sy[t] = by;
        } else {
          gsx[t - kLdsRefine] = bx;
          gsy[t - kLdsRefine] = by;
        }
      }
      team_sync<64>();
      phase(1);
      if (tid < 4) {
        double Mx = 0, My = 0, Mxx = 0, Mxy = 0, Myy = 0, N = 0;
        const int o = S.samp_off[tid];
        const int ns = min(S.nsamp[tid], RCAP - o);
        for (int c = 0; c < ns; c += 8) {
          double xs[8], ys[8];
#pragma unroll
          for (int k = 0; k < 8; k++) {
            const int i = o + c + k;
            xs[k] = __longlong_as_double(0x7ff8deadbeef0000ll);
            ys[k] = 0;
            if (c + k < ns) {
              xs[k] = i < kLdsRefine ? S.sx[i] : gsx[i - kLdsRefine];
              ys[k] = i < kLdsRefine ? S.sy[i] : gsy[i - kLdsRefine];
            }
          }
#pragma unroll
          for (int k = 0; k < 8; k++) {
            const double bx = xs[k], by = ys[k];
            if (isnan(bx)) continue;
            Mx += bx; My += by; Mxx += bx * bx; Mxy += bx * by; Myy += by * by; N++;
          }
        }
        const double Ex = Mx / N, Ey = My / N;
        const double Cxx = Mxx / N - Ex * Ex, Cxy = Mxy / N - Ex * Ey, Cyy = Myy / N - Ey * Ey;
        const double nt = .5 * (double)det_atan2f_call((float)(-2 * Cxy), (float)(Cyy - Cxx));
        S.lines[tid][0] = Ex;
        S.lines[tid][1] = Ey;
        S.lines[tid][2] = (double)det_cosf((float)nt);
        S.lines[tid][3] = (double)det_sinf((float)nt);
      }
      team_sync<64>();
      phase(2);
      if (tid == 0) {
        float qp[4][2];
        for (int k = 0; k < 4; k++) { qp[k][0] = S.qc[k][0]; qp[k][1] = S.qc[k][1]; }
        for (int i = 0; i < 4; i++) {
          const int i1 = (i + 1) & 3;
          const double A00 = S.lines[i][3], A01 = -S.lines[i1][3];
          const double A10 = -S.lines[i][2], A11 = S.lines[i1][2];
          const double B0 = -S.lines[i][0] + S.lines[i1][0];
          const double B1 = -S.lines[i][1] + S.lines[i1][1];
          const double det = A00 * A11 - A10 * A01;
          if (fabs(det) > 0.001) {
            const double W00 = A11 / det, W01 = -A01 / det;
            const double L0 = W00 * B0 + W01 * B1;
            double px = S.lines[i][0] + L0 * A00, py = S.lines[i][1] + L0 * A10;
            redistort(prm, &px, &py);
            qp[i1][0] = (float)px;
            qp[i1][1] = (float)py;
          }
        }
        for (int k = 0; k < 4; k++) { S.qc[k][0] = qp[k][0]; S.qc[k][1] = qp[k][1]; }
      }
      team_sync<64>();
      phase(3);
    }
    if (AT_DIAG_STOP(prm, 6)) continue;
    if (homography_wave(S.qc, S.A, S.H) != 0) continue;
    if (tid == 0) {
      const double* H = S.H;
      const double hdet = H[0] * (H[4] * H[8] - H[5] * H[7]) - H[1] * (H[3] * H[8] - H[5] * H[6]) +
                          H[2] * (H[3] * H[7] - H[4] * H[6]);
      S.ok = hdet != 0;
    }
    team_sync<64>();
    phase(4);
    if (!S.ok) continue;
    uint32_t seq = 0;
    if (POSE) {
      if (tid < 9) P.H[tid] = S.H[tid];
      if (tid < 4) {
        const int tcx = (tid == 1 || tid == 2) ? 1 : -1, tcy = tid < 2 ? 1 : -1;
        hproject(S.H, tcx, tcy, &P.p[tid][0], &P.p[tid][1]);
      }
      seq = ++pose_seq;
      team_sync<64>();
      if (tid == 0) __hip_atomic_store(&P.seq, seq, __ATOMIC_RELEASE, __HIP_MEMORY_SCOPE_WORKGROUP);
    }
    uint32_t bc = 0xffffffffu;
    double margin_d = -1;
    do {
    const int wab = prm.fam.width_at_border, tw = prm.fam.total_width, nbits = prm.fam.nbits;
    const int minc = (wab - tw) / 2;
    {
      const int pidx = tid >> 3, i = tid & 7;
      float p0, p1, p2, p3;
      border_pattern(pidx, (float)wab, p0, p1, p2, p3);
      const double tagx01 = (double)((p0 + (float)i * p2) / (float)wab);
      const double tagy01 = (double)((p1 + (float)i * p3) / (float)wab);
      const double tagx = 2 * (tagx01 - 0.5), tagy = 2 * (tagy01 - 0.5);
      double px, py;
      hproject(S.H, tagx, tagy, &px, &py);
      const int ix = (int)px, iy = (int)py;
      S.gmx[tid] = tagx;
      S.gmy[tid] = tagy;
      S.gmvalid[tid] = i < wab && !(ix < 0 || iy < 0 || ix >= g.W || iy >= g.H);
      S.gmv[tid] = S.gmvalid[tid] ? (double)pix((size_t)iy * g.W + ix) : 0.0;
    }
    for (int t = tid; t < tw * tw; t += kDecodeThreads) S.values[t] = 0;
    team_sync<64>();
    phase(5);
    double interp00 = 0;
    if (tid < 2) {
      GrayModel m;
      for (int k = 0; k < 3; k++) {
        m.B[k] = 0;
        for (int j = 0; j < 3; j++) m.A[k][j] = 0;
      }
      for (int grp = 0; grp < 4; grp++) {
        const int t0 = 16 * grp + 8 * tid;
        double xs[8], ys[8], vs[8];
        int ok[8];
#pragma unroll
        for (int i = 0; i < 8; i++) {
          xs[i] = S.gmx[t0 + i];
          ys[i] = S.gmy[t0 + i];
          vs[i] = S.gmv[t0 + i];
          ok[i] = S.gmvalid[t0 + i];
        }
#pragma unroll
        for (int i = 0; i < 8; i++)
          if (ok[i]) gm_add(m, xs[i], ys[i], vs[i]);
      }
      gm_solve(m);
      double* C = tid == 0 ? S.wC : S.bC;
      for (int k = 0; k < 3; k++) C[k] = m.C[k];
      interp00 = gm_interp(m, 0, 0);
    }
    const double w00 = __shfl(interp00, 0), b00 = __shfl(interp00, 1);
    team_sync<64>();
    if (w00 - b00 < 0) break;
    phase(6);
    if (tid < nbits) {
      const int bity = prm.fam.bity[tid], bitx = prm.fam.bitx[tid];
      const double tagx01 = (bitx + 0.5) / wab, tagy01 = (bity + 0.5) / wab;
      const double tagx = 2 * (tagx01 - 0.5), tagy = 2 * (tagy01 - 0.5);
      double px, py;
      hproject(S.H, tagx, tagy, &px, &py);
      const int x1 = (int)floor(px - 0.5), x2 = (int)ceil(px - 0.5);
      const double xx = px - 0.5 - x1;
      const int y1 = (int)floor(py - 0.5), y2 = (int)ceil(py - 0.5);
      const double yy = py - 0.5 - y1;
      if (!(x1 < 0 || x2 >= g.W || y1 < 0 || y2 >= g.H)) {
        const double v = (int)pix((size_t)y1 * g.W + x1) * (1 - xx) * (1 - yy) + (int)pix((size_t)y1 * g.W + x2) * xx * (1 - yy) +
                         (int)pix((size_t)y2 * g.W + x1) * (1 - xx) * yy + (int)pix((size_t)y2 * g.W + x2) * xx * yy;
        const double bth = S.bC[0] * tagx + S.bC[1] * tagy + S.bC[2];
        const double wth = S.wC[0] * tagx + S.wC[1] * tagy + S.wC[2];
        S.values[tw * (bity - minc) + bitx - minc] = v - (bth + wth) / 2.0;
      }
    }
    team_sync<64>();
    phase(7);
    constexpr int kShR = (kMaxTotalWidth * kMaxTotalWidth + kDecodeThreads - 1) / kDecodeThreads;
    double shv[kShR];
    int tl = tid;
    __asm__ volatile("" : "+v"(tl));
#pragma unroll
    for (int r = 0; r < kShR; r++) {
      const int t = tl + 64 * r;
      shv[r] = 0;
      if (t < tw * tw) {
        const int y = t / tw, x = t % tw;
        const double up = S.values[y > 0 ? t - tw : t], left = S.values[x > 0 ? t - 1 : t], c = S.values[t];
        const double right = S.values[x < tw - 1 ? t + 1 : t], down = S.values[y < tw - 1 ? t + tw : t];
        double acc = 0;
        if (y > 0) acc = acc - up;
        if (x > 0) acc = acc - left;
        acc = acc + c * 4;
        if (x < tw - 1) acc = acc - right;
        if (y < tw - 1) acc = acc - down;
        shv[r] = acc;
      }
    }
    team_sync<64>();
#pragma unroll
    for (int r = 0; r < kShR; r++) {
      const int t = tid + 64 * r;
      if (t < tw * tw) S.values[t] = S.values[t] + prm.decode_sharpening * shv[r];
    }
    team_sync<64>();
    double bitv = 0;
    if (tid < nbits) bitv = S.values[tw * (prm.fam.bity[tid] - minc) + prm.fam.bitx[tid] - minc];
    const uint64_t white_bits = __ballot(tid < nbits && bitv > 0);
    const uint64_t rcode0 = __builtin_bitreverse64(white_bits) >> (64 - nbits);
    {
      float black_score = 0, white_score = 0, black_cnt = 1, white_cnt = 1;
      for (int i = 0; i < nbits; i++) {
        const double v = readlane_f64(bitv, i);
        if (v > 0) { white_score = (float)(white_score + v); white_cnt++; }
        else { black_score = (float)(black_score - v); black_cnt++; }
      }
      margin_d = fmin((double)(white_score / white_cnt), (double)(black_score / black_cnt));
    }
    phase(8);
    {
      uint64_t r[4];
      r[0] = rcode0;
#pragma unroll
      for (int k = 1; k < 4; k++) r[k] = rotate90_n(r[k - 1], nbits);
      constexpr int kBookChunk = 10;
      for (int e0 = 0; e0 < prm.fam.ncodes; e0 += kBookChunk * kDecodeThreads) {
        uint64_t cw[kBookChunk];
#pragma unroll
        for (int k = 0; k < kBookChunk; k++) {
          const int ent = e0 + tid + kDecodeThreads * k;
          cw[k] = ent < prm.fam.ncodes ? b.book_code[ent] : 0ull;
        }
#pragma unroll
        for (int k = 0; k < kBookChunk; k++) {
          const int ent = e0 + tid + kDecodeThreads * k;
#pragma unroll
          for (int rot = 0; rot < 4; rot++) {
            const int hd = __popcll(r[rot] ^ cw[k]);
            if (ent < prm.fam.ncodes && hd <= 2) bc = min(bc, (uint32_t)((rot << 24) | (hd << 16) | ent));
          }
        }
      }
#pragma unroll
      for (int d = 32; d > 0; d >>= 1) bc = min(bc, (uint32_t)__shfl_xor(bc, d));
    }
    } while (false);
    if (POSE) {
      while (__hip_atomic_load(&P.ack, __ATOMIC_ACQUIRE, __HIP_MEMORY_SCOPE_WORKGROUP) != seq)
        __builtin_amdgcn_s_sleep(1);
    }
    if (tid == 0) {
      const float margin = (float)margin_d;
      if (margin >= 0 && bc != 0xffffffffu) {
        const int rot = bc >> 24, hd = (bc >> 16) & 0xff, ent = bc & 0xffff;
        DevDetection d;
        d.id = b.book_id[ent];
        d.hamming = hd;
        d.decision_margin = margin;
        d.blob_rank = (int32_t)qrank;
        const double R[9] = {c_rot_c[rot], -c_rot_s[rot], 0, c_rot_s[rot], c_rot_c[rot], 0, 0, 0, 1};
        for (int i = 0; i < 3; i++)
          for (int j = 0; j < 3; j++) {
            double acc = 0;
            for (int k = 0; k < 3; k++) acc += S.H[i * 3 + k] * R[k * 3 + j];
            d.H[i * 3 + j] = acc;
          }
        hproject(d.H, 0, 0, &d.c[0], &d.c[1]);
        for (int i = 0; i < 4; i++) {
          const int tcx = (i == 1 || i == 2) ? 1 : -1;
          const int tcy = (i < 2) ? 1 : -1;
          hproject(d.H, tcx, tcy, &d.p[i][0], &d.p[i][1]);
        }
        d.frame = (uint16_t)f;
        if (POSE) {
          const int c = rot == 0 ? 1 : rot == 2 ? -1 : 0, sn = rot == 1 ? 1 : rot == 3 ? -1 : 0;
          for (int i = 0; i < 3; i++) {
            d.pose_R[i * 3 + 0] = P.R[i * 3 + 0] * c + P.R[i * 3 + 1] * sn;
            d.pose_R[i * 3 + 1] = -P.R[i * 3 + 0] * sn + P.R[i * 3 + 1] * c;
            d.pose_R[i * 3 + 2] = P.R[i * 3 + 2];
          }
          for (int k = 0; k < 3; k++) d.pose_t[k] = P.t[k];
          d.pose_err[0] = P.err[0];
          d.pose_err[1] = P.err[1];
        }
        const uint32_t k = atomicAdd(b.ndets + f, 1u);
        if (k < (uint32_t)kMaxDets) {
          const uint32_t slot = (uint32_t)f * kMaxDets + k;
          b.dets[slot] = d;
          if (k < (uint32_t)kDetPoolPerFrame) b.hdets[(uint32_t)f * kDetPoolPerFrame + k] = d;
          if (!POSE) b.det_work[atomicAdd(b.det_head, 1u)] = slot;
        } else {
          atomicOr(b.status + f, kStatusDetsOverflow);
        }
      }
    }
    team_sync<64>();
    phase(9);
  }
  probe_flush(b, prm, pacc, 128, tid == 0);
  if (tid == 0) kt_end(b, 10);
  if (POSE) {
    if (tid == 0) __hip_atomic_store(&P.exit, 1u, __ATOMIC_RELEASE, __HIP_MEMORY_SCOPE_WORKGROUP);
    decode_finish(b, tid, nq);
  }
}

__global__ __launch_bounds__(256) void k_tap_sizes(const uint8_t* thr, const uint32_t* par, const uint32_t* size,
                                                   uint32_t* out, int Wd, int Hd) {
  const int i = blockIdx.x * 256 + threadIdx.x;
  if (i >= Wd * Hd) return;
  const int y = i / Wd, x = i % Wd;
  const int F = (y & ~1) * Wd + (x & ~1);
  const int BW = Wd / 2;
  uint32_t v = 0;
  bool node = true, has = false;
  uint32_t n = 0;
  if ((y & 1) == 0) {
    if (x & 1) node = false;
    else has = thr[F] == 255 || thr[F + 1] == 255 || (y + 1 < Hd && (thr[F + Wd] == 255 || thr[F + Wd + 1] == 255));
    n = (uint32_t)((y >> 1) * 3 * BW + (x >> 1));
  } else {
    has = thr[i] == 0 || thr[i - Wd] == 0;
    n = (uint32_t)((y >> 1) * 3 * BW + BW + x);
  }
  if (node && has && (par[n] & ~kKeptBit) == n) v = size[n];
  out[i] = v;
}

__global__ __launch_bounds__(256) void k_tap_labels(const uint8_t* thr, const uint32_t* par, uint32_t* out, int Wd,
                                                    int Hd) {
  const int i = blockIdx.x * 256 + threadIdx.x;
  if (i >= Wd * Hd) return;
  const int y = i / Wd, x = i % Wd;
  const int F = (y & ~1) * Wd + (x & ~1);
  const bool all127 = thr[F] == 127 && thr[F + 1] == 127 && thr[F + Wd] == 127 && thr[F + Wd + 1] == 127;
  uint32_t lab;
  if (all127) lab = (uint32_t)i;
  else if (thr[i] == 127) lab = 0;
  else {
    const int BW = Wd / 2;
    const uint32_t n = thr[i] == 255 ? (uint32_t)((y >> 1) * 3 * BW + (x >> 1)) : (uint32_t)((y >> 1) * 3 * BW + BW + x);
    lab = node_pixel(BW, Wd, par[par[n] & ~kKeptBit] & ~kKeptBit);
  }
  out[i] = lab;
}

hipError_t launch_tap_labels(const uint8_t* thr, const uint32_t* par, uint32_t* out, int Wd, int Hd,
                             hipStream_t st) {
  hipLaunchKernelGGL(k_tap_labels, dim3((Wd * Hd + 255) / 256), dim3(256), 0, st, thr, par, out, Wd, Hd);
  return hipGetLastError();
}

hipError_t launch_tap_sizes(const uint8_t* thr, const uint32_t* par, const uint32_t* size, uint32_t* out, int Wd,
                            int Hd, hipStream_t st) {
  hipLaunchKernelGGL(k_tap_sizes, dim3((Wd * Hd + 255) / 256), dim3(256), 0, st, thr, par, size, out, Wd, Hd);
  return hipGetLastError();
}


constexpr int kPoseLanes = 4;
constexpr int kPoseGroupsPerFrame = 8;
#ifndef AT_POSE_WAVES
#define AT_POSE_WAVES 1
#endif
template <bool WAVE>
__global__ __launch_bounds__(64) __attribute__((amdgpu_waves_per_eu(AT_POSE_WAVES))) void k_pose(DevBufs b, Params prm) {
  const int sub = (int)(threadIdx.x % kPoseLanes);
  if (blockIdx.x == 0)
    for (uint32_t w = threadIdx.x; w < b.ctrl_words; w += 64) b.hctrl[w] = b.ctrl[w];
  const uint32_t n = *b.det_head;
  constexpr uint32_t kPer = WAVE ? 1 : 64 / kPoseLanes;
  for (uint32_t i = blockIdx.x * kPer + (WAVE ? 0 : threadIdx.x / kPoseLanes); i < n;
       i += gridDim.x * kPer) {
    const uint32_t slot = b.det_work[i];
    DevDetection& d = b.dets[slot];
    double R[9], t[3], err[2];
    pose::estimate_tag_pose<WAVE>(d.H, d.p, prm.fx, prm.fy, prm.cx, prm.cy, prm.tag_size, R, t, err, sub,
                                  (AT_PROBE_ON(prm) && i == 0 && threadIdx.x == 0) ? b.probe + 16 : nullptr);
    if (WAVE ? threadIdx.x == 0 : sub == 0) {
#pragma unroll
      for (int k = 0; k < 9; k++) d.pose_R[k] = R[k];
#pragma unroll
      for (int k = 0; k < 3; k++) d.pose_t[k] = t[k];
      d.pose_err[0] = err[0];
      d.pose_err[1] = err[1];
      const uint32_t f = slot / kMaxDets, k = slot % kMaxDets;
      if (k < (uint32_t)kDetPoolPerFrame) {
        DevDetection& h = b.hdets[f * kDetPoolPerFrame + k];
#pragma unroll
        for (int j = 0; j < 9; j++) h.pose_R[j] = R[j];
#pragma unroll
        for (int j = 0; j < 3; j++) h.pose_t[j] = t[j];
        h.pose_err[0] = err[0];
        h.pose_err[1] = err[1];
      }
    }
  }
}

struct GpGeom {
  int w, h, ow, oh, c;
  double sx, sy;
  int area2;
};
__device__ __forceinline__ int gp_coef(float c) { return (int)__builtin_rintf(c * 2048.f); }

__device__ __forceinline__ void gp_pixel(const uint8_t* src, const GpGeom& q, int dx, int dy, float* out) {
  int v[3];
  if (q.area2) {
    const uint8_t* s0 = src + ((size_t)(2 * dy) * q.w + 2 * dx) * 3;
    const uint8_t* s1 = s0 + (size_t)q.w * 3;
#pragma unroll
    for (int c = 0; c < 3; c++) v[c] = (s0[c] + s0[c + 3] + s1[c] + s1[c + 3] + 2) >> 2;
  } else {
    float fx = (float)((dx + 0.5) * q.sx - 0.5);
    int sx = (int)floorf(fx);
    fx -= (float)sx;
    if (sx < 0) { fx = 0.f; sx = 0; }
    const bool one = sx + 1 >= q.w;
    if (one && sx >= q.w - 1) { fx = 0.f; sx = q.w - 1; }
    const int a0 = gp_coef(1.f - fx), a1 = gp_coef(fx);
    float fy = (float)((dy + 0.5) * q.sy - 0.5);
    const int sy = (int)floorf(fy);
    fy -= (float)sy;
    const int b0 = gp_coef(1.f - fy), b1 = gp_coef(fy);
    const int r0 = min(max(sy, 0), q.h - 1), r1 = min(max(sy + 1, 0), q.h - 1);
    const uint8_t* S0 = src + ((size_t)r0 * q.w + sx) * 3;
    const uint8_t* S1 = src + ((size_t)r1 * q.w + sx) * 3;
#pragma unroll
    for (int c = 0; c < 3; c++) {
      const int h0 = one ? S0[c] * 2048 : S0[c] * a0 + S0[c + 3] * a1;
      const int h1 = one ? S1[c] * 2048 : S1[c] * a0 + S1[c + 3] * a1;
      v[c] = (((b0 * (h0 >> 4)) >> 16) + ((b1 * (h1 >> 4)) >> 16) + 2) >> 2;
    }
  }
  const float a = (float)(1.0 / 255.0);
  const size_t plane = (size_t)q.ow * q.oh, i = (size_t)dy * q.ow + dx;
  if (q.c == 3) {
    out[i] = (float)v[2] * a;
    out[plane + i] = (float)v[1] * a;
    out[2 * plane + i] = (float)v[0] * a;
  } else {
    out[i] = (float)((v[0] * 1868 + v[1] * 9617 + v[2] * 4899 + (1 << 13)) >> 14) * a;
  }
}

__device__ __forceinline__ GpGeom gp_geom(int w, int h, int ow, int oh, int c) {
  GpGeom q;
  q.w = w; q.h = h; q.ow = ow; q.oh = oh; q.c = c;
  q.sx = 1. / ((double)ow / w);
  q.sy = 1. / ((double)oh / h);
  q.area2 = q.sx == 2.0 && q.sy == 2.0;
  return q;
}

__global__ __launch_bounds__(256) void k_gp_pre(DevBufs b, Geom g, Params prm) {
  const int f = blockIdx.z;
  const int dx = blockIdx.x * 64 + threadIdx.x, dy = blockIdx.y * 4 + threadIdx.y;
  if (dx >= prm.gp_w || dy >= prm.gp_h) return;
  const GpGeom q = gp_geom(g.W, g.H, prm.gp_w, prm.gp_h, prm.gp_c);
  gp_pixel(b.frames[f], q, dx, dy, b.gp_out + (size_t)f * prm.gp_c * prm.gp_w * prm.gp_h);
}

__global__ __launch_bounds__(256) void k_gp_pre_one(const uint8_t* src, int w, int h, float* out, int ow, int oh, int c) {
  const int dx = blockIdx.x * 64 + threadIdx.x, dy = blockIdx.y * 4 + threadIdx.y;
  if (dx >= ow || dy >= oh) return;
  gp_pixel(src, gp_geom(w, h, ow, oh, c), dx, dy, out);
}

hipError_t launch_gp_preprocess(const uint8_t* src, int w, int h, float* out, int ow, int oh, int c, hipStream_t st) {
  hipLaunchKernelGGL(k_gp_pre_one, dim3((ow + 63) / 64, (oh + 3) / 4), dim3(64, 4), 0, st, src, w, h, out, ow, oh, c);
  return hipGetLastError();
}

__device__ __forceinline__ bool seg_box(const DrawPrim& q, int W, int H, int* x0, int* y0, int* bw, int* bh) {
  const double r = 1.0;
  const int xa = (int)floor(fmin(q.x0, q.x1) - r), xb = (int)ceil(fmax(q.x0, q.x1) + r);
  const int ya = (int)floor(fmin(q.y0, q.y1) - r), yb = (int)ceil(fmax(q.y0, q.y1) + r);
  *x0 = max(xa, 0);
  *y0 = max(ya, 0);
  *bw = min(xb, W - 1) - *x0 + 1;
  *bh = min(yb, H - 1) - *y0 + 1;
  return *bw > 0 && *bh > 0;
}
__device__ __forceinline__ bool seg_covers(const DrawPrim& q, int x, int y) {
  const double r = 1.0;
  const double dx = q.x1 - q.x0, dy = q.y1 - q.y0, l2 = dx * dx + dy * dy;
  double u = l2 > 0 ? ((x - q.x0) * dx + (y - q.y0) * dy) / l2 : 0.0;
  u = fmin(1.0, fmax(0.0, u));
  const double ex = q.x0 + u * dx - x, ey = q.y0 + u * dy - y;
  return ex * ex + ey * ey <= r * r;
}
template <bool PAINT>
__global__ __launch_bounds__(256) void k_draw(const DrawPrim* prims, uint32_t* last, uint8_t* bgr, int W, int H) {
  const int p = blockIdx.x;
  const DrawPrim q = prims[p];
  int x0, y0, bw, bh;
  if (!seg_box(q, W, H, &x0, &y0, &bw, &bh)) return;
  for (int i = threadIdx.x; i < bw * bh; i += 256) {
    const int x = x0 + i % bw, y = y0 + i / bw;
    if (!seg_covers(q, x, y)) continue;
    const size_t o = (size_t)y * W + x;
    if (!PAINT) {
      atomicMax(last + o, (uint32_t)(p + 1));
    } else if (last[o] == (uint32_t)(p + 1)) {
      bgr[3 * o + 0] = q.bgr[0];
      bgr[3 * o + 1] = q.bgr[1];
      bgr[3 * o + 2] = q.bgr[2];
      last[o] = 0;
    }
  }
}

hipError_t launch_draw(const DrawPrim* prims, int n, uint32_t* last, uint8_t* bgr, int W, int H, hipStream_t st) {
  if (n <= 0) return hipSuccess;
  hipLaunchKernelGGL(k_draw<false>, dim3(n), dim3(256), 0, st, prims, last, bgr, W, H);
  hipLaunchKernelGGL(k_draw<true>, dim3(n), dim3(256), 0, st, prims, last, bgr, W, H);
  return hipGetLastError();
}

constexpr int kMjpgBlocksPerWg = 32, kMjpgLdsStride = 72;
__constant__ uint8_t c_mjpg_zigzag[64] = AT_MJPG_ZIGZAG;

__device__ __forceinline__ void mjpg_idct_blocks(const uint8_t* __restrict__ fr, uint8_t* __restrict__ out, int W,
                                                 int bw, uint32_t nb, int32_t* ws) {
  const uint16_t* q = reinterpret_cast<const uint16_t*>(fr);
  const uint32_t mode = *reinterpret_cast<const uint32_t*>(fr + kMjpgModeOff);
  const uint32_t ntok = *reinterpret_cast<const uint32_t*>(fr + kMjpgNtokOff);
  const uint8_t* pay = fr + kMjpgHdrBytes;
  const int t = threadIdx.x;
  const uint32_t blk0 = blockIdx.x * kMjpgBlocksPerWg;
  {
    const int lb = t >> 3, j = t & 7;
    const uint32_t blk = blk0 + lb;
    int32_t* w = ws + lb * kMjpgLdsStride + 8 * j;
    if (mode == kMjpgDense) {
      uint4 v = make_uint4(0, 0, 0, 0);
      if (blk < nb) v = *reinterpret_cast<const uint4*>(pay + ((size_t)blk * 64 + 8 * j) * 2);
      const uint32_t u[4] = {v.x, v.y, v.z, v.w};
#pragma unroll
      for (int k = 0; k < 4; k++) {
        w[2 * k] = (int32_t)(int16_t)(u[k] & 0xffffu) * (int32_t)q[8 * j + 2 * k];
        w[2 * k + 1] = (int32_t)(int16_t)(u[k] >> 16) * (int32_t)q[8 * j + 2 * k + 1];
      }
      __syncthreads();
    } else {
#pragma unroll
      for (int k = 0; k < 8; k++) w[k] = 0;
      __syncthreads();
      if (blk < nb) {
        const uint32_t* off = reinterpret_cast<const uint32_t*>(pay);
        const uint32_t* tok = off + nb + 1;
        const uint32_t end = min(off[blk + 1], ntok);
        int32_t* wb = ws + lb * kMjpgLdsStride;
        for (uint32_t i = off[blk] + j; i < end; i += 8) {
          const uint32_t tk = tok[i];
          const int nat = c_mjpg_zigzag[(tk >> 16) & 63];
          wb[nat] = (int32_t)(int16_t)(tk & 0xffffu) * (int32_t)q[nat];
        }
      }
      __syncthreads();
    }
    int32_t* col = ws + lb * kMjpgLdsStride + j;
    int32_t v[8];
#pragma unroll
    for (int r = 0; r < 8; r++) v[r] = col[8 * r];
    mjpg_idct_1d<11>(v);
#pragma unroll
    for (int r = 0; r < 8; r++) col[8 * r] = v[r];
  }
  __syncthreads();
  {
    const int l = t & 63, lb = (t >> 6) * 8 + (l & 7), r = l >> 3;
    const uint32_t blk = blk0 + lb;
    const int4* row = reinterpret_cast<const int4*>(ws + lb * kMjpgLdsStride + 8 * r);
    const int4 a = row[0], b4 = row[1];
    int32_t v[8] = {a.x, a.y, a.z, a.w, b4.x, b4.y, b4.z, b4.w};
    mjpg_idct_1d<18>(v);
    uint2 px;
    px.x = mjpg_pixel(v[0]) | (mjpg_pixel(v[1]) << 8) | (mjpg_pixel(v[2]) << 16) | (mjpg_pixel(v[3]) << 24);
    px.y = mjpg_pixel(v[4]) | (mjpg_pixel(v[5]) << 8) | (mjpg_pixel(v[6]) << 16) | (mjpg_pixel(v[7]) << 24);
    if (blk < nb) {
      const uint32_t by = blk / (uint32_t)bw, bx = blk - by * (uint32_t)bw;
      *reinterpret_cast<uint2*>(out + ((size_t)by * 8 + r) * W + (size_t)bx * 8) = px;
    }
  }
}

__global__ __launch_bounds__(256) void k_mjpg_idct(const uint8_t* __restrict__ coef, size_t slot,
                                                   uint8_t* __restrict__ out, size_t out_stride, int W, int bw,
                                                   uint32_t nb) {
  __shared__ __attribute__((aligned(16))) int32_t ws[kMjpgBlocksPerWg * kMjpgLdsStride];
  const int f = blockIdx.y;
  mjpg_idct_blocks(coef + (size_t)f * slot, out + (size_t)f * out_stride, W, bw, nb, ws);
}

__global__ __launch_bounds__(256) void k_mjpg_idct_chroma(const uint8_t* __restrict__ coef, size_t slot,
                                                          uint8_t* __restrict__ planes, size_t plane_stride,
                                                          uint32_t max_nb) {
  __shared__ __attribute__((aligned(16))) int32_t ws[kMjpgBlocksPerWg * kMjpgLdsStride];
  const int f = blockIdx.y, c = blockIdx.z;
  const uint8_t* fr = coef + (size_t)f * slot;
  const uint32_t off = *reinterpret_cast<const uint32_t*>(fr + (c ? kMjpgCrOff : kMjpgCbOff));
  if (!off || (size_t)off + kMjpgHdrBytes > slot) return;
  const uint8_t* sub = fr + off;
  uint32_t nb = min(*reinterpret_cast<const uint32_t*>(sub + kMjpgNblkOff), max_nb);
// ... 584 lines not shown
  const uint32_t slot = base + lanes_below(m);
  if (cand && slot < (uint32_t)kGpMaxCand) {
    b.key[(size_t)f * kGpMaxCand + slot] = gp_key(best, (uint32_t)i);
    b.cls[(size_t)f * kGpMaxCand + slot] = cls;
  }
}

constexpr int kGpNmsThreads = 1024;
constexpr int kGpPer = kGpMaxCand / kGpNmsThreads;
constexpr int kGpLiveWords = kGpMaxCand / 64;
constexpr int kGpWaves = kGpNmsThreads / 64;
static_assert(kGpLiveWords == 64 && kGpPer * kGpWaves == kGpLiveWords, "k_gp_nms: one live word per (k, wave)");

__global__ __launch_bounds__(kGpNmsThreads) void k_gp_nms(const float* __restrict__ raw, size_t frame_stride, int P,
                                                          float iou_thr, float sx, float sy, GpParseBufs b) {
  __shared__ uint64_t s_key[kGpMaxCand];
  __shared__ uint16_t s_slot[kGpMaxCand];
  __shared__ uint64_t s_live[kGpLiveWords];
  __shared__ uint32_t s_rank[kGpLiveWords];
  __shared__ GpCorners s_piv;
  __shared__ uint32_t s_n;
  const int f = blockIdx.x, tid = threadIdx.x;
  const uint32_t lane = lane_id(), wave = (uint32_t)tid >> 6;
  if (tid == 0) {
    const uint32_t c = b.cnt[(size_t)f * kGpCntStride];
    s_n = c;
    b.cnt[(size_t)f * kGpCntStride] = 0;
    b.info[2 * f + 1] = c;
    if (c == 0 || c > (uint32_t)kGpMaxCand) b.info[2 * f] = 0;
  }
  __syncthreads();
  const uint32_t ncand = s_n;
  if (ncand == 0 || ncand > (uint32_t)kGpMaxCand) return;

  const uint64_t* gkey = b.key + (size_t)f * kGpMaxCand;
  uint32_t n2 = 2;
  if (ncand <= (uint32_t)kGpNmsThreads) {
    const uint64_t mine = (uint32_t)tid < ncand ? gkey[tid] : ~0ull;
    if ((uint32_t)tid < ncand) s_key[tid] = mine;
    __syncthreads();
    uint32_t rank = 0;
    if ((uint32_t)tid < ncand) {
#pragma unroll 8
      for (uint32_t i = 0; i < ncand; i++) rank += s_key[i] < mine ? 1u : 0u;
    }
    __syncthreads();
    if ((uint32_t)tid < ncand) {
      s_key[rank] = mine;
      s_slot[rank] = (uint16_t)tid;
    }
    __syncthreads();
    n2 = 0;
  } else {
    while (n2 < ncand) n2 <<= 1;
    for (uint32_t j = tid; j < n2; j += kGpNmsThreads) {
      s_key[j] = j < ncand ? gkey[j] : ~0ull;
      s_slot[j] = (uint16_t)j;
    }
    __syncthreads();
  }
  for (uint32_t k = 2; k <= n2; k <<= 1) {
    for (uint32_t j = k >> 1; j > 0; j >>= 1) {
      for (uint32_t i = tid; i < n2; i += kGpNmsThreads) {
        const uint32_t ixj = i ^ j;
        if (ixj > i) {
          const uint64_t a = s_key[i], c = s_key[ixj];
          const bool up = (i & k) == 0;
          if ((a > c) == up) {
            s_key[i] = c;
            s_key[ixj] = a;
            const uint16_t t = s_slot[i];
            s_slot[i] = s_slot[ixj];
            s_slot[ixj] = t;
          }
        }
      }
      __syncthreads();
    }
  }

  const float* fr = raw + (size_t)f * frame_stride;
  const int32_t* gcls = b.cls + (size_t)f * kGpMaxCand;
  float bx[kGpPer], by[kGpPer], bw[kGpPer], bh[kGpPer], bconf[kGpPer];
  GpCorners bc[kGpPer];
  bool live[kGpPer];
#pragma unroll
  for (int k = 0; k < kGpPer; k++) {
    const uint32_t j = (uint32_t)tid + (uint32_t)k * kGpNmsThreads;
    live[k] = j < ncand;
    bx[k] = by[k] = bw[k] = bh[k] = bconf[k] = 0.0f;
    int32_t c = 0;
    if (live[k]) {
      const uint64_t key = s_key[j];
      const size_t i = gp_key_index(key);
      bconf[k] = gp_key_conf(key);
      bx[k] = fr[i];
      by[k] = fr[(size_t)P + i];
      bw[k] = fr[2 * (size_t)P + i];
      bh[k] = fr[3 * (size_t)P + i];
      c = gcls[s_slot[j]];
    }
    bc[k] = gp_corners(bx[k], by[k], bw[k], bh[k], c);
    const uint64_t m = __ballot(live[k]);
    if (lane == 0) s_live[k * kGpWaves + wave] = m;
  }

  const uint32_t nwords = (ncand + 63) >> 6;
  uint32_t pos = 0;
  for (;;) {
    __syncthreads();
    int p = -1;
    for (uint32_t w = pos >> 6; w < nwords; w++) {
      uint64_t m = s_live[w];
      if (w == (pos >> 6)) m &= ~0ull << (pos & 63);
      if (m) {
        p = (int)(w * 64 + (uint32_t)__builtin_ctzll(m));
        break;
      }
    }
    if (p < 0) break;
#pragma unroll
    for (int k = 0; k < kGpPer; k++)
      if ((uint32_t)p == (uint32_t)tid + (uint32_t)k * kGpNmsThreads) s_piv = bc[k];
    __syncthreads();
    const GpCorners a = s_piv;
#pragma unroll
    for (int k = 0; k < kGpPer; k++) {
      const uint32_t j = (uint32_t)tid + (uint32_t)k * kGpNmsThreads;
      const bool sup = live[k] && j > (uint32_t)p && gp_suppresses(a, bc[k], iou_thr);
      const uint64_t m = __ballot(sup);
      if (m && lane == 0) s_live[k * kGpWaves + wave] &= ~m;
      if (sup) live[k] = false;
    }
    pos = (uint32_t)p + 1;
  }

  if (wave == 0) {
    const uint32_t c = lane < nwords ? (uint32_t)__popcll(s_live[lane]) : 0u;
    const uint32_t incl = wave_incl_scan(c, AddOp(), 0u);
    s_rank[lane] = incl - c;
    if (lane == 63) b.info[2 * f] = incl;
  }
  __syncthreads();
  GpBox* out = b.out + (size_t)f * kGpMaxCand;
#pragma unroll
  for (int k = 0; k < kGpPer; k++) {
    if (!live[k]) continue;
    const uint32_t w = k * kGpWaves + wave;
    const uint32_t r = s_rank[w] + (uint32_t)__popcll(s_live[w] & ((1ull << lane) - 1));
    out[r] = gp_scaled(bx[k], by[k], bw[k], bh[k], bconf[k], bc[k].cls, sx, sy);
  }
}

hipError_t launch_gp_parse(const float* raw, size_t frame_stride, int nframes, int P, int C, float conf_thr,
                           float iou_thr, float sx, float sy, const GpParseBufs& b, hipStream_t st) {
  hipLaunchKernelGGL(k_gp_cand, dim3(((unsigned)P + 255u) / 256u, nframes), dim3(256), 0, st, raw, frame_stride, P, C,
                     conf_thr, b);
  hipLaunchKernelGGL(k_gp_nms, dim3(nframes), dim3(kGpNmsThreads), 0, st, raw, frame_stride, P, iou_thr, sx, sy, b);
  return hipGetLastError();
}

static size_t merge_lds_bytes(const Geom& g) { return (size_t)g.merge_lds; }

hipError_t prepare_kernels(const Geom& g) {
  if (!g.merge_cap) return hipSuccess;
  return hipFuncSetAttribute((const void*)k_ccl_merge<64>, hipFuncAttributeMaxDynamicSharedMemorySize,
                             kMergeLdsMax);
}

hipError_t launch_pipeline(const DevBufs& b, const Geom& g, const Params& prm, int B, int fmt, int nblobwg,
                           hipStream_t st, hipEvent_t* ev, hipStream_t st2, hipEvent_t fork, hipEvent_t join,
                           const KernelTimer* kt) {
  int e = 0;
  auto on = [&](int stage) { return AT_PIPE_STOP(prm) <= 0 || stage < AT_PIPE_STOP(prm); };
  auto mark = [&]() {
    if (ev) (void)hipEventRecord(ev[e++], st);
  };
  hipError_t split_err = hipSuccess;
  auto tk = [&](int stage, hipStream_t s, int which) {
    if (!kt || kt->stage != stage) return;
    if (kt->split) {
      const hipError_t r = kt->split(kt->ctx, which);
      if (r != hipSuccess && split_err == hipSuccess) split_err = r;
    } else {
      (void)hipEventRecord(which ? kt->t1 : kt->t0, s);
    }
  };
  mark();
  {
    dim3 blk(64, 4), grd((g.TW + 63) / 64, (g.TH + 3) / 4, B);
    tk(0, st, 0);
    if (!on(0) || g.ctw == 32) {}
    else if (fmt == 0) hipLaunchKernelGGL(k_pre<0>, grd, blk, 0, st, b, g, prm.taps);
    else if (fmt == 1) hipLaunchKernelGGL(k_pre<1>, grd, blk, 0, st, b, g, 1);
    else hipLaunchKernelGGL(k_pre<2>, grd, blk, 0, st, b, g, prm.taps);
    tk(0, st, 1);
    if (on(0) && prm.gp_c && fmt == 1)
      hipLaunchKernelGGL(k_gp_pre, dim3((prm.gp_w + 63) / 64, (prm.gp_h + 3) / 4, B), dim3(64, 4), 0, st, b, g, prm);
  }
  mark();
  {
    dim3 grd(g.CTX, g.CTY, B);
    tk(1, st, 0);
    if (!on(1)) {}
    else if (g.ctw != 32) hipLaunchKernelGGL((k_thr_ccl<64, -1>), grd, dim3(CclTile<64>::NT), 0, st, b, g, prm);
    else if (fmt == 0) hipLaunchKernelGGL((k_thr_ccl<32, 0>), grd, dim3(CclTile<32>::NT), 0, st, b, g, prm);
    else if (fmt == 1) hipLaunchKernelGGL((k_thr_ccl<32, 1>), grd, dim3(CclTile<32>::NT), 0, st, b, g, prm);
    else hipLaunchKernelGGL((k_thr_ccl<32, 2>), grd, dim3(CclTile<32>::NT), 0, st, b, g, prm);
    tk(1, st, 1);
    mark();
    tk(2, st, 0);
    if (!on(2)) {}
    else if (g.ctw == 32) hipLaunchKernelGGL(k_ccl_border<32>, grd, dim3(BorderRoles<32>::NT), 0, st, b, g);
    else hipLaunchKernelGGL(k_ccl_merge<64>, dim3(B), dim3(1024), merge_lds_bytes(g), st, b, g, prm);
    tk(2, st, 1);
    mark();
  }
  tk(3, st, 0);
  if (on(3) && g.ctw == 32)
    hipLaunchKernelGGL(k_ccl_roots, dim3(g.CTX * g.CTY, B), dim3(64), 0, st, b, g);
  tk(3, st, 1);
  mark();
  {
    dim3 blk(64, 4), grd(g.BTX, g.BTY, B);
    tk(4, st, 0);
    if (!on(4)) {}
    else if (g.ctw != 32) hipLaunchKernelGGL(k_boundary<true>, grd, blk, 0, st, b, g);
    else hipLaunchKernelGGL(k_boundary<false>, grd, blk, 0, st, b, g);
    tk(4, st, 1);
    mark();
  }
  tk(5, st, 0);
  if (on(5)) hipLaunchKernelGGL(k_pairs, dim3(B), dim3(1024), 0, st, b, g, AT_PROBE_ON(prm));
  tk(5, st, 1);
  mark();
  tk(6, st, 0);
  if (on(6)) hipLaunchKernelGGL(k_group, dim3(g.ntb, B), dim3(256), 0, st, b, g);
  tk(6, st, 1);
  mark();
  tk(7, st, 0);
  const bool fuse_small = g.ctw == 32;
  const bool lat_fused = g.ctw == 32 && g.max_cluster <= 4096 && !ev && !kt;
  if (on(7) && !(g.ctw == 32 && g.max_cluster <= 4096)) hipLaunchKernelGGL(k_extents, dim3(std::max(16, std::min(AT_EXT_GRID, 96 * B))), dim3(256), 0, st, b, g);
  tk(7, st, 1);
  mark();
  auto blob_large = [&](hipStream_t s) {
    tk(9, s, 0);
    const bool cap4k = g.max_cluster <= 4096;
    if (!on(9)) return;
    if (lat_fused) {
      hipLaunchKernelGGL(k_blob_lat, dim3(nblobwg), dim3(512), 0, s, b, g, prm);
    } else if (g.ctw == 32 && cap4k) {
      hipLaunchKernelGGL((k_blob<512, 4096, true>), dim3(nblobwg), dim3(512), 0, s, b, g, prm, 0u, 0, g.nlarge, 0);
    } else if (B < kWideBlobMaxBatch || prm.wide_blob) {
      if (cap4k) hipLaunchKernelGGL((k_blob<512, 4096>), dim3(nblobwg), dim3(512), 0, s, b, g, prm, 0u, 0, g.nlarge, 0);
      else hipLaunchKernelGGL((k_blob<512, kSortCap>), dim3(nblobwg), dim3(512), 0, s, b, g, prm, 0u, 0, g.nlarge, 0);
    } else {
      const int lo = prm.lblob_wg ? std::min(prm.lblob_wg, nblobwg) : nblobwg;
      hipLaunchKernelGGL((k_blob<256, 4096>), dim3(lo), dim3(256), 0, s, b, g, prm, 0u, 0, g.nlarge - 1, 0);
      hipLaunchKernelGGL((k_blob_small<false, 1024, 3, 9>), dim3(nblobwg), dim3(256), 0, s, b, g, prm, g.nlarge - 1, g.nlarge, 1);
      if (!cap4k)
        hipLaunchKernelGGL((k_blob<AT_BIG_NT, kSortCap>), dim3(std::min(nblobwg, AT_BIG_BLOB_WG)), dim3(AT_BIG_NT), 0, s, b, g,
                           prm, 4096u, 0, 1, 2);
    }
    tk(9, s, 1);
  };
  auto blob_small = [&](hipStream_t s) {
    tk(8, s, 0);
    if (!on(8) || lat_fused) {}
    else if (fuse_small) hipLaunchKernelGGL(k_blob_small<true>, dim3(nblobwg * 2), dim3(256), 0, s, b, g, prm, g.nlarge, kNumCls, 0);
    else hipLaunchKernelGGL(k_blob_small<false>, dim3(prm.sblob_wg ? prm.sblob_wg : nblobwg * 2), dim3(256), 0, s, b, g, prm, g.nlarge, kNumCls, 0);
    tk(8, s, 1);
  };
  const int fin_c1 = g.ctw != 32 ? kNumCls : g.max_cluster > 4096 ? g.nlarge : 0;
  auto quad_fin = [&](hipStream_t s) {
    if (fin_c1 > 0 && on(9) && (!AT_DIAG_ANY(prm) || AT_DIAG_STOP(prm, 5)))
      hipLaunchKernelGGL(k_quad_fin, dim3(std::max(1, std::min(2048, 8 * B))), dim3(256), 0, s, b, g, prm, 0, fin_c1);
  };
  if (ev || !st2 || lat_fused) {
    blob_small(st);
    mark();
    blob_large(st);
    quad_fin(st);
    mark();
  } else {
    hipError_t e;
    if ((e = hipEventRecord(fork, st))) return e;
    if ((e = hipStreamWaitEvent(st2, fork, 0))) return e;
    if (AT_FORK_SMALL) {
      blob_large(st);
      blob_small(st2);
    } else {
      blob_small(st);
      blob_large(st2);
    }
    if ((e = hipEventRecord(join, st2))) return e;
    if ((e = hipStreamWaitEvent(st, join, 0))) return e;
    quad_fin(st);
  }
  const bool pose_fused = AT_POSE_IN_DECODE && prm.tag_size > 0 && on(11) && B < kWideBlobMaxBatch && !ev && b.kt_stage < 0 && !kt;
  tk(10, st, 0);
  {
    const dim3 grd(prm.dec_wg ? std::min(prm.dec_wg, decode_grid(nblobwg, B)) : decode_grid(nblobwg, B));
    if (on(10) && pose_fused) hipLaunchKernelGGL(k_decode<true>, grd, dim3(128), 0, st, b, g, prm, B, fmt);
    else if (on(10)) hipLaunchKernelGGL(k_decode<false>, grd, dim3(kDecodeThreads), 0, st, b, g, prm, B, fmt);
  }
  tk(10, st, 1);
  mark();
  if (b.kt_stage >= 1 && b.kt_stage <= 10 && b.kt_stage != 3 && b.kt_stage != 5 && b.kt_stage != 6)
    hipLaunchKernelGGL(k_kt_span, dim3(kKtSpanWgs), dim3(256), 0, st, b);
  tk(11, st, 0);
  if (prm.tag_size > 0 && on(11) && !pose_fused) {
    if (B < kWideBlobMaxBatch) hipLaunchKernelGGL(k_pose<true>, dim3(32 * B), dim3(64), 0, st, b, prm);
    else hipLaunchKernelGGL(k_pose<false>, dim3(kPoseGroupsPerFrame * B), dim3(64), 0, st, b, prm);
  }
  tk(11, st, 1);
  mark();
  if (split_err != hipSuccess) return split_err;
  return hipGetLastError();
}

}
```

Baseline: 149,100.

## Decode four quads per wavefront using 16-lane rows in k_decode

Adds a row-packed decode path in which each 64-lane wavefront is split into rows of 16 lanes, and each row decodes its own quad candidate. Per-quad shared state moves into a union-based DecodeRow struct, and a new lane-parallel homography solve works within a row. Edge refinement now samples each pixel position once and reuses duplicates instead of issuing two loads per step. The aim is to cut idle lanes when per-quad work is too small to fill a wave, at the cost of more per-row global scratch, more LDS, and lower per-quad parallelism.

```diff
diff --git a/ros_vision_amd/csrc/at_api.cpp b/ros_vision_amd/csrc/at_api.cpp
--- a/ros_vision_amd/csrc/at_api.cpp
+++ b/ros_vision_amd/csrc/at_api.cpp
@@ -398,6 +398,7 @@
   p.lblob_wg = knob("AT_LBLOB_WG") ? std::max(16, knob_int("AT_LBLOB_WG", 0)) : 0;
   p.sblob_wg = knob("AT_SBLOB_WG") ? std::max(16, knob_int("AT_SBLOB_WG", 0)) : 0;
   p.dec_wg = knob("AT_DEC_WG") ? std::max(16, knob_int("AT_DEC_WG", 0)) : 0;
+  p.dec_lpq = knob_int("AT_DEC_LPQ", 0) == 64 ? 64 : 0;
   p.fam = family_desc(*fam);
   d->use_graphs = !knob_int("AT_NO_GRAPH", 0);
   if (!(cfg->tag_size >= 0) || !std::isfinite(cfg->tag_size)) {
@@ -512,7 +513,7 @@
   b.qcand_cap = (uint32_t)(B * kQuadCandPerFrame);
   b.qcand = (QuadCand*)dalloc((size_t)b.qcand_cap * sizeof(QuadCand));
   b.s_pk = (uint64_t*)dalloc((size_t)2 * d->nblobwg * (kSortCap / 2) * 8);
-  b.rsamp = (double*)dalloc((size_t)decode_grid(d->nblobwg, d->B) * 2 * (kMaxRefineSamples - kLdsRefine) * 8);
+  b.rsamp = (double*)dalloc(decode_scratch_doubles(d->nblobwg, d->B, g.ctw == 64) * 8);
   if (oom) return fail(AT_E_NOMEM);
   if (prepare_kernels(g) != hipSuccess) return fail(AT_E_HIP);
   if (hipHostMalloc((void**)&d->h_ftab, B * sizeof(void*), hipHostMallocMapped | hipHostMallocCoherent) != hipSuccess)
diff --git a/ros_vision_amd/csrc/at_common.h b/ros_vision_amd/csrc/at_common.h
--- a/ros_vision_amd/csrc/at_common.h
+++ b/ros_vision_amd/csrc/at_common.h
@@ -51,6 +51,13 @@
   const int hi = nblobwg * kDecodeGridPerBlobWg, want = 64 * B;
   return nblobwg * 2 > (want < hi ? want : hi) ? nblobwg * 2 : (want < hi ? want : hi);
 }
+constexpr int kDecRowLanes = 16;
+constexpr int kRowRefine = 64;
+inline size_t decode_scratch_doubles(int nblobwg, int B, bool packed) {
+  const size_t one = 2 * (size_t)(kMaxRefineSamples - kLdsRefine);
+  const size_t rows = (64 / kDecRowLanes) * 2 * (size_t)(kMaxRefineSamples - kRowRefine);
+  return (size_t)decode_grid(nblobwg, B) * (packed && rows > one ? rows : one);
+}
 
 constexpr int kNumStages = 12;
 constexpr const char* kStageNames[kNumStages] = {"k_pre",   "k_thr_ccl", "k_ccl_merge", "k_ccl_roots",
@@ -116,6 +123,7 @@
   int lblob_wg;
   int sblob_wg;
   int dec_wg;
+  int dec_lpq;
   FamilyDesc fam;
   int gp_w, gp_h, gp_c;
 };
diff --git a/ros_vision_amd/csrc/at_kernels.hip b/ros_vision_amd/csrc/at_kernels.hip
--- a/ros_vision_amd/csrc/at_kernels.hip
+++ b/ros_vision_amd/csrc/at_kernels.hip
@@ -2227,6 +2227,80 @@
   return 0;
 }
 
+template <int LPQ>
+__device__ bool homography_rows(bool live, int rl, const float (*qc)[2], double* A, double* H) {
+  static_assert(LPQ >= 16 && 64 % LPQ == 0, "a row holds the 9 lanes of a swap and of H");
+  if (live) {
+    for (int e = rl; e < 72; e += LPQ) {
+      const int row = e / 9, col = e % 9, i = row >> 1;
+      const double c0 = (i == 0 || i == 3) ? -1 : 1, c1 = (i == 0 || i == 1) ? -1 : 1;
+      const double c2 = qc[i][0], c3 = qc[i][1];
+      const int k = (row & 1) ? col - 3 : col;
+      const double cz = (row & 1) ? c3 : c2;
+      double v = 0;
+      if (k == 0) v = c0;
+      else if (k == 1) v = c1;
+      else if (k == 2) v = 1;
+      if (col == 6) v = -c0 * cz;
+      else if (col == 7) v = -c1 * cz;
+      else if (col == 8) v = cz;
+      A[e] = v;
+    }
+  }
+  team_sync<64>();
+  for (int col = 0; col < 8; col++) {
+    double v = -1.0;
+    int row = 64;
+    if (live && rl < 8 - col) {
+      row = col + rl;
+      v = fabs(A[row * 9 + col]);
+      if (!(v > 0.0)) { v = -1.0; row = 64; }
+    }
+#pragma unroll
+    for (int d = 1; d < 8; d <<= 1) {
+      const double ov = __shfl_xor(v, d);
+      const int orow = __shfl_xor(row, d);
+      if (ov > v || (ov == v && orow < row)) { v = ov; row = orow; }
+    }
+    v = __shfl(v, 0, LPQ);
+    row = __shfl(row, 0, LPQ);
+    if (!(v >= 1e-10)) live = false;
+    if (live && row != col && rl <= 8 - col) {
+      const int i = col + rl;
+      const double t = A[col * 9 + i];
+      A[col * 9 + i] = A[row * 9 + i];
+      A[row * 9 + i] = t;
+    }
+    team_sync<64>();
+    if (live && (rl >> 1) < 7 - col) {
+      const int i = col + 1 + (rl >> 1);
+      const double fct = A[i * 9 + col] / A[col * 9 + col];
+#pragma unroll
+      for (int q = 0; q < 4; q++) {
+        const int j = col + 1 + 4 * (rl & 1) + q;
+        if (j <= 8) A[i * 9 + j] -= fct * A[col * 9 + j];
+      }
+    }
+    team_sync<64>();
+  }
+  double x[8];
+#pragma unroll
+  for (int col = 7; col >= 0; col--) {
+    double sum = 0;
+#pragma unroll
+    for (int i = col + 1; i < 8; i++) sum += A[col * 9 + i] * x[i];
+    x[col] = (A[col * 9 + 8] - sum) / A[col * 9 + col];
+  }
+  if (live) {
+#pragma unroll
+    for (int k = 0; k < 8; k++)
+      if (rl == k) H[k] = x[k];
+    if (rl == 8) H[8] = 1;
+  }
+  team_sync<64>();
+  return live;
+}
+
 struct GrayModel {
   double A[3][3], B[3], C[3];
 };
@@ -3984,24 +4058,35 @@
 #ifndef AT_DEC_WAVES
 #define AT_DEC_WAVES 4
 #endif
-template <bool POSE>
-__global__ __launch_bounds__(POSE ? 128 : kDecodeThreads) __attribute__((amdgpu_waves_per_eu(POSE ? 1 : AT_DEC_WAVES))) void k_decode(DevBufs b, Geom g, Params prm, int B, int fmt) {
+
+struct DecodeRow {
+  union {
+    struct { double sx[kRowRefine], sy[kRowRefine]; } ref;
+    double A[72];
+    struct { double x[64], y[64], v[64]; uint8_t valid[64]; } gm;
+    double values[kMaxTotalWidth * kMaxTotalWidth];
+  } u;
+  float qc[4][2];
+  int nsamp[4], samp_off[4];
+  float enx[4], eny[4];
+  double lines[4][4];
+  double H[9];
+  double wC[3], bC[3];
+  int f;
+  uint32_t rank;
+};
+
+template <int LPQ>
+__device__ __forceinline__ void decode_rows(const DevBufs& b, const Geom& g, const Params& prm, int B, int fmt) {
+  constexpr int NR = 64 / LPQ;
   constexpr int RCAP = kMaxRefineSamples;
-  __shared__ DecodeShared S;
-  __shared__ PoseHandoff P;
+  constexpr int kBitRounds = kMaxFamilyBits / LPQ;
+  __shared__ DecodeRow rows[NR];
+  __shared__ uint32_t qpre[kMaxBatch + 1];
   const int tid = threadIdx.x;
+  const int row = tid / LPQ, rl = tid % LPQ;
   kt_begin(b, 10);
-  if (POSE) {
-    if (tid == 0) { P.seq = 0; P.ack = 0; P.exit = 0; }
-    __syncthreads();
-    if (tid >= 64) {
-      pose_worker(P, prm);
-      return;
-    }
-  }
-  double* gsx = b.rsamp + (size_t)blockIdx.x * (2 * (kMaxRefineSamples - kLdsRefine));
-  double* gsy = gsx + (kMaxRefineSamples - kLdsRefine);
-  uint32_t* qpre = S.qpre;
+  constexpr int kGy = kMaxRefineSamples - kRowRefine;
   {
     uint32_t c[kMaxBatch / 64], sum = 0;
 #pragma unroll
@@ -4035,65 +4120,77 @@
       t_last = now;
     }
   };
-  const uint32_t G = gridDim.x;
-  uint32_t pose_seq = 0;
   struct ItemPre {
     int f;
     uint32_t rank;
     float px, py;
     const uint8_t* gsrc;
   };
-  auto prefetch = [&](uint32_t it) -> ItemPre {
-    int lo = 0, hi = B - 1;
-    while (lo < hi) {
-      const int mid = (lo + hi + 1) >> 1;
-      if (qpre[mid] <= it) lo = mid;
-      else hi = mid - 1;
-    }
-    const QuadCand* q = &b.qcand[(size_t)lo * kQuadCandPerFrame + (it - qpre[lo])];
-    ItemPre p;
-    p.f = lo;
-    p.rank = q->rank;
-    p.px = tid < 4 ? q->p[tid & 3][0] : 0.f;
-    p.py = tid < 4 ? q->p[tid & 3][1] : 0.f;
-    p.gsrc = fmt == 1 ? b.gray + (size_t)lo * g.W * g.H : b.frames[lo];
+  auto prefetch = [&](uint32_t it, int rl) -> ItemPre {
+    ItemPre p = {};
+    if (it < nq) {
+      int lo = 0, hi = B - 1;
+      while (lo < hi) {
+        const int mid = (lo + hi + 1) >> 1;
+        if (qpre[mid] <= it) lo = mid;
+        else hi = mid - 1;
+      }
+      const QuadCand* q = &b.qcand[(size_t)lo * kQuadCandPerFrame + (it - qpre[lo])];
+      p.f = lo;
+      p.rank = q->rank;
+      p.px = rl < 4 ? q->p[rl & 3][0] : 0.f;
+      p.py = rl < 4 ? q->p[rl & 3][1] : 0.f;
+      p.gsrc = fmt == 1 ? b.gray + (size_t)lo * g.W * g.H : b.frames[lo];
+    }
     return p;
   };
-  ItemPre nxt = {};
-  if (blockIdx.x < nq) nxt = prefetch(blockIdx.x);
-  for (uint32_t item = blockIdx.x; item < nq; item += G) {
+  const uint32_t G = gridDim.x;
+  const int wab = prm.fam.width_at_border, tw = prm.fam.total_width, nbits = prm.fam.nbits;
+  const int minc = (wab - tw) / 2;
+  const uint32_t gsh = fmt == 0 ? 1 : 0, wsh = (uint32_t)g.W << gsh;
+  ItemPre nxt = prefetch(NR * blockIdx.x + row, rl);
+  for (uint32_t base = NR * blockIdx.x; base < nq; base += NR * G) {
+    int tq = tid;
+    __asm__ volatile("" : "+v"(tq));
+    const int rowq = tq / LPQ;
+    int rlq = tq % LPQ;
+    DecodeRow& S = rows[rowq];
+    auto gref = [&](int i) -> double* {
+      return b.rsamp + ((size_t)blockIdx.x * NR + rowq) * (2 * kGy) + (i - kRowRefine);
+    };
+    const uint32_t item = base + rowq;
     const ItemPre cur = nxt;
-    if (item + G < nq) nxt = prefetch(item + G);
-    const int f = cur.f;
-    const uint32_t qrank = cur.rank;
+    bool live = item < nq;
     const uint8_t* gsrc = cur.gsrc;
-    const int gsh = fmt == 0 ? 1 : 0;
-    auto pix = [&](size_t i) -> uint32_t { return gsrc[i << gsh]; };
-    if (tid < 4) { S.qc[tid][0] = cur.px; S.qc[tid][1] = cur.py; }
+    typedef const __attribute__((address_space(1))) uint8_t* gbytes;
+    auto pix = [&](int x, int y) -> uint32_t { return ((gbytes)gsrc)[(uint32_t)y * wsh + ((uint32_t)x << gsh)]; };
+    if (live && rlq < 4) { S.qc[rlq][0] = cur.px; S.qc[rlq][1] = cur.py; }
+    if (live && rlq == 0) { S.f = cur.f; S.rank = cur.rank; }
     team_sync<64>();
     phase(0);
     if (prm.refine_edges) {
-      if (tid < 4) {
-        const int a2 = tid, b2 = (tid + 1) & 3;
+      if (live && rlq < 4) {
+        const int a2 = rlq, b2 = (rlq + 1) & 3;
         float nx = S.qc[b2][1] - S.qc[a2][1];
         float ny = -S.qc[b2][0] + S.qc[a2][0];
         const float mag = sqrtf(nx * nx + ny * ny);
         nx /= mag;
         ny /= mag;
         const int nsf = (int)(mag / 8);
-        S.nsamp[tid] = nsf > 16 ? nsf : 16;
-        S.enx[tid] = nx;
-        S.eny[tid] = ny;
+        S.nsamp[rlq] = nsf > 16 ? nsf : 16;
+        S.enx[rlq] = nx;
+        S.eny[rlq] = ny;
       }
       team_sync<64>();
-      if (tid == 0) {
+      if (live && rlq == 0) {
         int acc = 0;
         for (int k = 0; k < 4; k++) { S.samp_off[k] = acc; acc += S.nsamp[k]; }
       }
       team_sync<64>();
-      const int total = min(S.samp_off[3] + S.nsamp[3], RCAP);
-      if (tid == 0 && S.samp_off[3] + S.nsamp[3] > RCAP) atomicOr(b.status + f, kStatusQuadsOverflow);
-      for (int t = tid; t < total; t += kDecodeThreads) {
+      const int want = live ? S.samp_off[3] + S.nsamp[3] : 0;
+      const int total = min(want, RCAP);
+      if (rlq == 0 && want > RCAP) atomicOr(b.status + S.f, kStatusQuadsOverflow);
+      for (int t = rlq; t < total; t += LPQ) {
         int edge = 0;
         while (edge < 3 && t >= S.samp_off[edge + 1]) edge++;
         const int s = t - S.samp_off[edge];
@@ -4103,29 +4200,29 @@
         const double alpha = (1.0 + s) / (nsamples + 1);
         const double x0 = alpha * S.qc[a2][0] + (1 - alpha) * S.qc[b2][0];
         const double y0 = alpha * S.qc[a2][1] + (1 - alpha) * S.qc[b2][1];
-        constexpr int kSteps = 25;
-        int g1v[kSteps], g2v[kSteps];
+        constexpr int kSteps = 25, kPos = kSteps + 8;
+        int pv[kPos];
+        int xp = 0, yp = 0;
+#pragma unroll
+        for (int j = 0; j < kPos; j++) {
+          const double m = -4.0 + 0.25 * j;
+          const int x = (int)(x0 + m * nx);
+          const int y = (int)(y0 + m * ny);
+          const bool same = j > 0 && x == xp && y == yp;
+          pv[j] = same ? -2 : -1;
+          if (!same && !(x < 0 || x >= g.W || y < 0 || y >= g.H)) pv[j] = (int)pix(x, y);
+          xp = x;
+          yp = y;
+        }
+#pragma unroll
+        for (int j = 1; j < kPos; j++)
+          if (pv[j] == -2) pv[j] = pv[j - 1];
+        double Mn = 0, Mcount = 0;
 #pragma unroll
         for (int k = 0; k < kSteps; k++) {
           const double nn = -3.0 + 0.25 * k;
-          const int x1 = (int)(x0 + (nn + 1) * nx);
-          const int y1 = (int)(y0 + (nn + 1) * ny);
-          const int x2 = (int)(x0 + (nn - 1) * nx);
-          const int y2 = (int)(y0 + (nn - 1) * ny);
-          const bool in = !(x1 < 0 || x1 >= g.W || y1 < 0 || y1 >= g.H) && !(x2 < 0 || x2 >= g.W || y2 < 0 || y2 >= g.H);
-          g1v[k] = -1;
-          g2v[k] = 0;
-          if (in) {
-            g1v[k] = (int)pix((size_t)y1 * g.W + x1);
-            g2v[k] = (int)pix((size_t)y2 * g.W + x2);
-          }
-        }
-        double Mn = 0, Mcount = 0;
-#pragma unroll
-        for (int k = 0; k < kSteps; k++) {
-          const double nn = -3.0 + 0.25 * k;
-          const int g1 = g1v[k], g2 = g2v[k];
-          if (g1 < g2) continue;
+          const int g1 = pv[k + 8], g2 = pv[k];
+          if (g1 < 0 || g2 < 0 || g1 < g2) continue;
           const double weight = (double)((g2 - g1) * (g2 - g1));
           Mn += weight * nn;
           Mcount += weight;
@@ -4137,20 +4234,20 @@
           by = y0 + n0 * ny;
           undistort(prm, &bx, &by);
         }
-        if (t < kLdsRefine) {
-          S.sx[t] = bx;
-          S.sy[t] = by;
+        if (t < kRowRefine) {
+          S.u.ref.sx[t] = bx;
+          S.u.ref.sy[t] = by;
         } else {
-          gsx[t - kLdsRefine] = bx;
-          gsy[t - kLdsRefine] = by;
+          gref(t)[0] = bx;
+          gref(t)[kGy] = by;
         }
       }
       team_sync<64>();
       phase(1);
-      if (tid < 4) {
+      if (live && rlq < 4) {
         double Mx = 0, My = 0, Mxx = 0, Mxy = 0, Myy = 0, N = 0;
-        const int o = S.samp_off[tid];
-        const int ns = min(S.nsamp[tid], RCAP - o);
+        const int o = S.samp_off[rlq];
+        const int ns = min(S.nsamp[rlq], RCAP - o);
         for (int c = 0; c < ns; c += 8) {
           double xs[8], ys[8];
 #pragma unroll
@@ -4159,8 +4256,8 @@
             xs[k] = __longlong_as_double(0x7ff8deadbeef0000ll);
             ys[k] = 0;
             if (c + k < ns) {
-              xs[k] = i < kLdsRefine ? S.sx[i] : gsx[i - kLdsRefine];
-              ys[k] = i < kLdsRefine ? S.sy[i] : gsy[i - kLdsRefine];
+              xs[k] = i < kRowRefine ? S.u.ref.sx[i] : gref(i)[0];
+              ys[k] = i < kRowRefine ? S.u.ref.sy[i] : gref(i)[kGy];
             }
           }
 #pragma unroll
@@ -4173,14 +4270,14 @@
         const double Ex = Mx / N, Ey = My / N;
         const double Cxx = Mxx / N - Ex * Ex, Cxy = Mxy / N - Ex * Ey, Cyy = Myy / N - Ey * Ey;
         const double nt = .5 * (double)det_atan2f_call((float)(-2 * Cxy), (float)(Cyy - Cxx));
-        S.lines[tid][0] = Ex;
-        S.lines[tid][1] = Ey;
-        S.lines[tid][2] = (double)det_cosf((float)nt);
-        S.lines[tid][3] = (double)det_sinf((float)nt);
+        S.lines[rlq][0] = Ex;
+        S.lines[rlq][1] = Ey;
+        S.lines[rlq][2] = (double)det_cosf((float)nt);
+        S.lines[rlq][3] = (double)det_sinf((float)nt);
       }
       team_sync<64>();
       phase(2);
-      if (tid == 0) {
+      if (live && rlq == 0) {
         float qp[4][2];
         for (int k = 0; k < 4; k++) { qp[k][0] = S.qc[k][0]; qp[k][1] = S.qc[k][1]; }
         for (int i = 0; i < 4; i++) {
@@ -4204,184 +4301,196 @@
       team_sync<64>();
       phase(3);
     }
-    if (AT_DIAG_STOP(prm, 6)) continue;
-    if (homography_wave(S.qc, S.A, S.H) != 0) continue;
-    if (tid == 0) {
-      const double* H = S.H;
-      const double hdet = H[0] * (H[4] * H[8] - H[5] * H[7]) - H[1] * (H[3] * H[8] - H[5] * H[6]) +
-                          H[2] * (H[3] * H[7] - H[4] * H[6]);
-      S.ok = hdet != 0;
-    }
-    team_sync<64>();
+    if (AT_DIAG_STOP(prm, 6)) {
+      nxt = prefetch(item + NR * G, rlq);
+      continue;
+    }
+    live = homography_rows<LPQ>(live, rlq, S.qc, S.u.A, S.H);
+    {
+      int ok = 0;
+      if (live && rlq == 0) {
+        const double* H = S.H;
+        const double hdet = H[0] * (H[4] * H[8] - H[5] * H[7]) - H[1] * (H[3] * H[8] - H[5] * H[6]) +
+                            H[2] * (H[3] * H[7] - H[4] * H[6]);
+        ok = hdet != 0;
+      }
+      live = __shfl(ok, 0, LPQ) != 0;
+    }
     phase(4);
-    if (!S.ok) continue;
-    uint32_t seq = 0;
-    if (POSE) {
-      if (tid < 9) P.H[tid] = S.H[tid];
-      if (tid < 4) {
-        const int tcx = (tid == 1 || tid == 2) ? 1 : -1, tcy = tid < 2 ? 1 : -1;
-        hproject(S.H, tcx, tcy, &P.p[tid][0], &P.p[tid][1]);
-      }
-      seq = ++pose_seq;
-      team_sync<64>();
-      if (tid == 0) __hip_atomic_store(&P.seq, seq, __ATOMIC_RELEASE, __HIP_MEMORY_SCOPE_WORKGROUP);
-    }
-    uint32_t bc = 0xffffffffu;
-    double margin_d = -1;
-    do {
-    const int wab = prm.fam.width_at_border, tw = prm.fam.total_width, nbits = prm.fam.nbits;
-    const int minc = (wab - tw) / 2;
-    {
-      const int pidx = tid >> 3, i = tid & 7;
-      float p0, p1, p2, p3;
-      border_pattern(pidx, (float)wab, p0, p1, p2, p3);
-      const double tagx01 = (double)((p0 + (float)i * p2) / (float)wab);
-      const double tagy01 = (double)((p1 + (float)i * p3) / (float)wab);
-      const double tagx = 2 * (tagx01 - 0.5), tagy = 2 * (tagy01 - 0.5);
-      double px, py;
-      hproject(S.H, tagx, tagy, &px, &py);
-      const int ix = (int)px, iy = (int)py;
-      S.gmx[tid] = tagx;
-      S.gmy[tid] = tagy;
-      S.gmvalid[tid] = i < wab && !(ix < 0 || iy < 0 || ix >= g.W || iy >= g.H);
-      S.gmv[tid] = S.gmvalid[tid] ? (double)pix((size_t)iy * g.W + ix) : 0.0;
-    }
-    for (int t = tid; t < tw * tw; t += kDecodeThreads) S.values[t] = 0;
+    __asm__ volatile("" : "+v"(rlq));
+    if (live) {
+#pragma unroll 1
+      for (int r = 0; r < 64 / LPQ; r++) {
+        const int t = rlq + LPQ * r;
+        const int pidx = t >> 3, i = t & 7;
+        float p0, p1, p2, p3;
+        border_pattern(pidx, (float)wab, p0, p1, p2, p3);
+        const double tagx01 = (double)((p0 + (float)i * p2) / (float)wab);
+        const double tagy01 = (double)((p1 + (float)i * p3) / (float)wab);
+        const double tagx = 2 * (tagx01 - 0.5), tagy = 2 * (tagy01 - 0.5);
+        double px, py;
+        hproject(S.H, tagx, tagy, &px, &py);
+        const int ix = (int)px, iy = (int)py;
+        const bool valid = i < wab && !(ix < 0 || iy < 0 || ix >= g.W || iy >= g.H);
+        S.u.gm.x[t] = tagx;
+        S.u.gm.y[t] = tagy;
+        S.u.gm.valid[t] = valid;
+        S.u.gm.v[t] = valid ? (double)pix(ix, iy) : 0.0;
+      }
+    }
     team_sync<64>();
     phase(5);
     double interp00 = 0;
-    if (tid < 2) {
+    if (live && rlq < 2) {
       GrayModel m;
       for (int k = 0; k < 3; k++) {
         m.B[k] = 0;
         for (int j = 0; j < 3; j++) m.A[k][j] = 0;
       }
       for (int grp = 0; grp < 4; grp++) {
-        const int t0 = 16 * grp + 8 * tid;
+        const int t0 = 16 * grp + 8 * rlq;
         double xs[8], ys[8], vs[8];
         int ok[8];
 #pragma unroll
         for (int i = 0; i < 8; i++) {
-          xs[i] = S.gmx[t0 + i];
-          ys[i] = S.gmy[t0 + i];
-          vs[i] = S.gmv[t0 + i];
-          ok[i] = S.gmvalid[t0 + i];
+          xs[i] = S.u.gm.x[t0 + i];
+          ys[i] = S.u.gm.y[t0 + i];
+          vs[i] = S.u.gm.v[t0 + i];
+          ok[i] = S.u.gm.valid[t0 + i];
         }
 #pragma unroll
         for (int i = 0; i < 8; i++)
           if (ok[i]) gm_add(m, xs[i], ys[i], vs[i]);
       }
       gm_solve(m);
-      double* C = tid == 0 ? S.wC : S.bC;
+      double* C = rlq == 0 ? S.wC : S.bC;
       for (int k = 0; k < 3; k++) C[k] = m.C[k];
       interp00 = gm_interp(m, 0, 0);
     }
-    const double w00 = __shfl(interp00, 0), b00 = __shfl(interp00, 1);
+    {
+      const double w00 = __shfl(interp00, 0, LPQ), b00 = __shfl(interp00, 1, LPQ);
+      if (w00 - b00 < 0) live = false;
+    }
     team_sync<64>();
-    if (w00 - b00 < 0) break;
     phase(6);
-    if (tid < nbits) {
-      const int bity = prm.fam.bity[tid], bitx = prm.fam.bitx[tid];
-      const double tagx01 = (bitx + 0.5) / wab, tagy01 = (bity + 0.5) / wab;
-      const double tagx = 2 * (tagx01 - 0.5), tagy = 2 * (tagy01 - 0.5);
-      double px, py;
-      hproject(S.H, tagx, tagy, &px, &py);
-      const int x1 = (int)floor(px - 0.5), x2 = (int)ceil(px - 0.5);
-      const double xx = px - 0.5 - x1;
-      const int y1 = (int)floor(py - 0.5), y2 = (int)ceil(py - 0.5);
-      const double yy = py - 0.5 - y1;
-      if (!(x1 < 0 || x2 >= g.W || y1 < 0 || y2 >= g.H)) {
-        const double v = (int)pix((size_t)y1 * g.W + x1) * (1 - xx) * (1 - yy) + (int)pix((size_t)y1 * g.W + x2) * xx * (1 - yy) +
-                         (int)pix((size_t)y2 * g.W + x1) * (1 - xx) * yy + (int)pix((size_t)y2 * g.W + x2) * xx * yy;
-        const double bth = S.bC[0] * tagx + S.bC[1] * tagy + S.bC[2];
-        const double wth = S.wC[0] * tagx + S.wC[1] * tagy + S.wC[2];
-        S.values[tw * (bity - minc) + bitx - minc] = v - (bth + wth) / 2.0;
+    if (live)
+      for (int t = rlq; t < tw * tw; t += LPQ) S.u.values[t] = 0;
+    team_sync<64>();
+    __asm__ volatile("" : "+v"(rlq));
+#pragma unroll 1
+    for (int r = 0; r * LPQ < nbits; r++) {
+      const int bi = rlq + LPQ * r;
+      if (live && bi < nbits) {
+        const int bity = prm.fam.bity[bi], bitx = prm.fam.bitx[bi];
+        const double tagx01 = (bitx + 0.5) / wab, tagy01 = (bity + 0.5) / wab;
+        const double tagx = 2 * (tagx01 - 0.5), tagy = 2 * (tagy01 - 0.5);
+        double px, py;
+        hproject(S.H, tagx, tagy, &px, &py);
+        const int x1 = (int)floor(px - 0.5), x2 = (int)ceil(px - 0.5);
+        const double xx = px - 0.5 - x1;
+        const int y1 = (int)floor(py - 0.5), y2 = (int)ceil(py - 0.5);
+        const double yy = py - 0.5 - y1;
+        if (!(x1 < 0 || x2 >= g.W || y1 < 0 || y2 >= g.H)) {
+          const double v = (int)pix(x1, y1) * (1 - xx) * (1 - yy) + (int)pix(x2, y1) * xx * (1 - yy) +
+                           (int)pix(x1, y2) * (1 - xx) * yy + (int)pix(x2, y2) * xx * yy;
+          const double bth = S.bC[0] * tagx + S.bC[1] * tagy + S.bC[2];
+          const double wth = S.wC[0] * tagx + S.wC[1] * tagy + S.wC[2];
+          S.u.values[tw * (bity - minc) + bitx - minc] = v - (bth + wth) / 2.0;
+        }
       }
     }
     team_sync<64>();
     phase(7);
-    constexpr int kShR = (kMaxTotalWidth * kMaxTotalWidth + kDecodeThreads - 1) / kDecodeThreads;
-    double shv[kShR];
-    int tl = tid;
-    __asm__ volatile("" : "+v"(tl));
-#pragma unroll
-    for (int r = 0; r < kShR; r++) {
-      const int t = tl + 64 * r;
-      shv[r] = 0;
-      if (t < tw * tw) {
+    double bitv[kBitRounds];
+    uint64_t white_bits = 0;
+    __asm__ volatile("" : "+v"(rlq));
+#pragma unroll
+    for (int r = 0; r < kBitRounds; r++) {
+      const int bi = rlq + LPQ * r;
+      bitv[r] = 0;
+      if (live && bi < nbits) {
+        const int t = tw * (prm.fam.bity[bi] - minc) + prm.fam.bitx[bi] - minc;
         const int y = t / tw, x = t % tw;
-        const double up = S.values[y > 0 ? t - tw : t], left = S.values[x > 0 ? t - 1 : t], c = S.values[t];
-        const double right = S.values[x < tw - 1 ? t + 1 : t], down = S.values[y < tw - 1 ? t + tw : t];
+        const double up = S.u.values[y > 0 ? t - tw : t], left = S.u.values[x > 0 ? t - 1 : t], c = S.u.values[t];
+        const double right = S.u.values[x < tw - 1 ? t + 1 : t], down = S.u.values[y < tw - 1 ? t + tw : t];
         double acc = 0;
         if (y > 0) acc = acc - up;
         if (x > 0) acc = acc - left;
         acc = acc + c * 4;
         if (x < tw - 1) acc = acc - right;
         if (y < tw - 1) acc = acc - down;
-        shv[r] = acc;
-      }
-    }
+        bitv[r] = c + prm.decode_sharpening * acc;
+      }
+      const uint64_t m = __ballot(live && bi < nbits && bitv[r] > 0);
+      white_bits |= ((m >> (rowq * LPQ)) & ((1ull << LPQ) - 1)) << (LPQ * r);
+    }
+    const uint64_t rcode0 = __builtin_bitreverse64(white_bits) >> (64 - nbits);
     team_sync<64>();
 #pragma unroll
-    for (int r = 0; r < kShR; r++) {
-      const int t = tid + 64 * r;
-      if (t < tw * tw) S.values[t] = S.values[t] + prm.decode_sharpening * shv[r];
+    for (int r = 0; r < kBitRounds; r++) {
+      const int bi = rlq + LPQ * r;
+      if (live && bi < nbits) S.u.values[bi] = bitv[r];
     }
     team_sync<64>();
-    double bitv = 0;
-    if (tid < nbits) bitv = S.values[tw * (prm.fam.bity[tid] - minc) + prm.fam.bitx[tid] - minc];
-    const uint64_t white_bits = __ballot(tid < nbits && bitv > 0);
-    const uint64_t rcode0 = __builtin_bitreverse64(white_bits) >> (64 - nbits);
+    double margin_d = -1;
     {
       float black_score = 0, white_score = 0, black_cnt = 1, white_cnt = 1;
       for (int i = 0; i < nbits; i++) {
-        const double v = readlane_f64(bitv, i);
+        const double v = S.u.values[i];
         if (v > 0) { white_score = (float)(white_score + v); white_cnt++; }
         else { black_score = (float)(black_score - v); black_cnt++; }
       }
       margin_d = fmin((double)(white_score / white_cnt), (double)(black_score / black_cnt));
     }
     phase(8);
+    uint32_t bc = 0xffffffffu;
+    nxt = prefetch(item + NR * G, rlq);
     {
-      uint64_t r[4];
-      r[0] = rcode0;
-#pragma unroll
-      for (int k = 1; k < 4; k++) r[k] = rotate90_n(r[k - 1], nbits);
+      uint64_t rc[NR][4];
+      uint32_t bcr[NR];
+#pragma unroll
+      for (int j = 0; j < NR; j++) {
+        rc[j][0] = wave_read(rcode0, j * LPQ);
+#pragma unroll
+        for (int k = 1; k < 4; k++) rc[j][k] = rotate90_n(rc[j][k - 1], nbits);
+        bcr[j] = 0xffffffffu;
+      }
       constexpr int kBookChunk = 10;
       for (int e0 = 0; e0 < prm.fam.ncodes; e0 += kBookChunk * kDecodeThreads) {
         uint64_t cw[kBookChunk];
 #pragma unroll
         for (int k = 0; k < kBookChunk; k++) {
-          const int ent = e0 + tid + kDecodeThreads * k;
+          const int ent = e0 + tq + kDecodeThreads * k;
           cw[k] = ent < prm.fam.ncodes ? b.book_code[ent] : 0ull;
         }
 #pragma unroll
         for (int k = 0; k < kBookChunk; k++) {
-          const int ent = e0 + tid + kDecodeThreads * k;
-#pragma unroll
-          for (int rot = 0; rot < 4; rot++) {
-            const int hd = __popcll(r[rot] ^ cw[k]);
-            if (ent < prm.fam.ncodes && hd <= 2) bc = min(bc, (uint32_t)((rot << 24) | (hd << 16) | ent));
-          }
+          const int ent = e0 + tq + kDecodeThreads * k;
+#pragma unroll
+          for (int j = 0; j < NR; j++)
+#pragma unroll
+            for (int rot = 0; rot < 4; rot++) {
+              const int hd = __popcll(rc[j][rot] ^ cw[k]);
+              if (ent < prm.fam.ncodes && hd <= 2) bcr[j] = min(bcr[j], (uint32_t)((rot << 24) | (hd << 16) | ent));
+            }
         }
       }
 #pragma unroll
-      for (int d = 32; d > 0; d >>= 1) bc = min(bc, (uint32_t)__shfl_xor(bc, d));
-    }
-    } while (false);
-    if (POSE) {
-      while (__hip_atomic_load(&P.ack, __ATOMIC_ACQUIRE, __HIP_MEMORY_SCOPE_WORKGROUP) != seq)
-        __builtin_amdgcn_s_sleep(1);
-    }
-    if (tid == 0) {
+      for (int j = 0; j < NR; j++) {
+        const uint32_t m = wave_reduce(bcr[j], MinOp());
+        if (rowq == j) bc = m;
+      }
+    }
+    if (live && rlq == 0) {
       const float margin = (float)margin_d;
       if (margin >= 0 && bc != 0xffffffffu) {
         const int rot = bc >> 24, hd = (bc >> 16) & 0xff, ent = bc & 0xffff;
+        const int f = S.f;
         DevDetection d;
         d.id = b.book_id[ent];
         d.hamming = hd;
         d.decision_margin = margin;
-        d.blob_rank = (int32_t)qrank;
+        d.blob_rank = (int32_t)S.rank;
         const double R[9] = {c_rot_c[rot], -c_rot_s[rot], 0, c_rot_s[rot], c_rot_c[rot], 0, 0, 0, 1};
         for (int i = 0; i < 3; i++)
           for (int j = 0; j < 3; j++) {
@@ -4396,23 +4505,12 @@
           hproject(d.H, tcx, tcy, &d.p[i][0], &d.p[i][1]);
         }
         d.frame = (uint16_t)f;
-        if (POSE) {
-          const int c = rot == 0 ? 1 : rot == 2 ? -1 : 0, sn = rot == 1 ? 1 : rot == 3 ? -1 : 0;
-          for (int i = 0; i < 3; i++) {
-            d.pose_R[i * 3 + 0] = P.R[i * 3 + 0] * c + P.R[i * 3 + 1] * sn;
-            d.pose_R[i * 3 + 1] = -P.R[i * 3 + 0] * sn + P.R[i * 3 + 1] * c;
-            d.pose_R[i * 3 + 2] = P.R[i * 3 + 2];
-          }
-          for (int k = 0; k < 3; k++) d.pose_t[k] = P.t[k];
-          d.pose_err[0] = P.err[0];
-          d.pose_err[1] = P.err[1];
-        }
         const uint32_t k = atomicAdd(b.ndets + f, 1u);
         if (k < (uint32_t)kMaxDets) {
           const uint32_t slot = (uint32_t)f * kMaxDets + k;
           b.dets[slot] = d;
           if (k < (uint32_t)kDetPoolPerFrame) b.hdets[(uint32_t)f * kDetPoolPerFrame + k] = d;
-          if (!POSE) b.det_work[atomicAdd(b.det_head, 1u)] = slot;
+          b.det_work[atomicAdd(b.det_head, 1u)] = slot;
         } else {
           atomicOr(b.status + f, kStatusDetsOverflow);
         }
@@ -4423,9 +4521,454 @@
   }
   probe_flush(b, prm, pacc, 128, tid == 0);
   if (tid == 0) kt_end(b, 10);
-  if (POSE) {
-    if (tid == 0) __hip_atomic_store(&P.exit, 1u, __ATOMIC_RELEASE, __HIP_MEMORY_SCOPE_WORKGROUP);
-    decode_finish(b, tid, nq);
+}
+template <bool POSE, int LPQ = 64>
+__global__ __launch_bounds__(POSE ? 128 : kDecodeThreads) __attribute__((amdgpu_waves_per_eu(POSE ? 1 : AT_DEC_WAVES))) void k_decode(DevBufs b, Geom g, Params prm, int B, int fmt) {
+  if constexpr (LPQ < 64) {
+    static_assert(!POSE, "the pose wave goes with one quad per wave");
+    decode_rows<LPQ>(b, g, prm, B, fmt);
+  } else {
+    constexpr int RCAP = kMaxRefineSamples;
+    __shared__ DecodeShared S;
+    __shared__ PoseHandoff P;
+    const int tid = threadIdx.x;
+    kt_begin(b, 10);
+    if (POSE) {
+      if (tid == 0) { P.seq = 0; P.ack = 0; P.exit = 0; }
+      __syncthreads();
+      if (tid >= 64) {
+        pose_worker(P, prm);
+        return;
+      }
+    }
+    double* gsx = b.rsamp + (size_t)blockIdx.x * (2 * (kMaxRefineSamples - kLdsRefine));
+    double* gsy = gsx + (kMaxRefineSamples - kLdsRefine);
+    uint32_t* qpre = S.qpre;
+    {
+      uint32_t c[kMaxBatch / 64], sum = 0;
+#pragma unroll
+      for (int k = 0; k < kMaxBatch / 64; k++) {
+        const int f = tid * (kMaxBatch / 64) + k;
+        c[k] = f < B ? min(b.nqcand[(size_t)f * kQcStride], (uint32_t)kQuadCandPerFrame) : 0u;
+        sum += c[k];
+      }
+      const uint32_t incl = wave_incl_scan(sum, AddOp(), 0u);
+      uint32_t acc = incl - sum;
+#pragma unroll
+      for (int k = 0; k < kMaxBatch / 64; k++) {
+        const int f = tid * (kMaxBatch / 64) + k;
+        if (f < B) qpre[f] = acc;
+        acc += c[k];
+      }
+      if (tid == 63) qpre[B] = incl;
+    }
+    team_sync<64>();
+    const uint32_t nq = qpre[B];
+
+    uint32_t pacc[21] = {0};
+    uint64_t t_last = 0;
+    auto phase = [&](int k) {
+      if (AT_PROBE_ON(prm) && tid == 0) {
+        const uint64_t now = wall_clock64();
+        if (k > 0) {
+          pacc[k] += (uint32_t)(now - t_last);
+          pacc[10 + k] += 1;
+        }
+        t_last = now;
+      }
+    };
+    const uint32_t G = gridDim.x;
+    uint32_t pose_seq = 0;
+    struct ItemPre {
+      int f;
+      uint32_t rank;
+      float px, py;
+      const uint8_t* gsrc;
+    };
+    auto prefetch = [&](uint32_t it) -> ItemPre {
+      int lo = 0, hi = B - 1;
+      while (lo < hi) {
+        const int mid = (lo + hi + 1) >> 1;
+        if (qpre[mid] <= it) lo = mid;
+        else hi = mid - 1;
+      }
+      const QuadCand* q = &b.qcand[(size_t)lo * kQuadCandPerFrame + (it - qpre[lo])];
+      ItemPre p;
+      p.f = lo;
+      p.rank = q->rank;
+      p.px = tid < 4 ? q->p[tid & 3][0] : 0.f;
+      p.py = tid < 4 ? q->p[tid & 3][1] : 0.f;
+      p.gsrc = fmt == 1 ? b.gray + (size_t)lo * g.W * g.H : b.frames[lo];
+      return p;
+    };
+    ItemPre nxt = {};
+    if (blockIdx.x < nq) nxt = prefetch(blockIdx.x);
+    for (uint32_t item = blockIdx.x; item < nq; item += G) {
+      const ItemPre cur = nxt;
+      if (item + G < nq) nxt = prefetch(item + G);
+      const int f = cur.f;
+      const uint32_t qrank = cur.rank;
+      const uint8_t* gsrc = cur.gsrc;
+      const int gsh = fmt == 0 ? 1 : 0;
+      auto pix = [&](size_t i) -> uint32_t { return gsrc[i << gsh]; };
+      if (tid < 4) { S.qc[tid][0] = cur.px; S.qc[tid][1] = cur.py; }
+      team_sync<64>();
+      phase(0);
+      if (prm.refine_edges) {
+        if (tid < 4) {
+          const int a2 = tid, b2 = (tid + 1) & 3;
+          float nx = S.qc[b2][1] - S.qc[a2][1];
+          float ny = -S.qc[b2][0] + S.qc[a2][0];
+          const float mag = sqrtf(nx * nx + ny * ny);
+          nx /= mag;
+          ny /= mag;
+          const int nsf = (int)(mag / 8);
+          S.nsamp[tid] = nsf > 16 ? nsf : 16;
+          S.enx[tid] = nx;
+          S.eny[tid] = ny;
+        }
+        team_sync<64>();
+        if (tid == 0) {
+          int acc = 0;
+          for (int k = 0; k < 4; k++) { S.samp_off[k] = acc; acc += S.nsamp[k]; }
+        }
+        team_sync<64>();
+        const int total = min(S.samp_off[3] + S.nsamp[3], RCAP);
+        if (tid == 0 && S.samp_off[3] + S.nsamp[3] > RCAP) atomicOr(b.status + f, kStatusQuadsOverflow);
+        for (int t = tid; t < total; t += kDecodeThreads) {
+          int edge = 0;
+          while (edge < 3 && t >= S.samp_off[edge + 1]) edge++;
+          const int s = t - S.samp_off[edge];
+          const int a2 = edge, b2 = (edge + 1) & 3;
+          const int nsamples = S.nsamp[edge];
+          const float nx = S.enx[edge], ny = S.eny[edge];
+          const double alpha = (1.0 + s) / (nsamples + 1);
+          const double x0 = alpha * S.qc[a2][0] + (1 - alpha) * S.qc[b2][0];
+          const double y0 = alpha * S.qc[a2][1] + (1 - alpha) * S.qc[b2][1];
+          constexpr int kSteps = 25;
+          int g1v[kSteps], g2v[kSteps];
+#pragma unroll
+          for (int k = 0; k < kSteps; k++) {
+            const double nn = -3.0 + 0.25 * k;
+            const int x1 = (int)(x0 + (nn + 1) * nx);
+            const int y1 = (int)(y0 + (nn + 1) * ny);
+            const int x2 = (int)(x0 + (nn - 1) * nx);
+            const int y2 = (int)(y0 + (nn - 1) * ny);
+            const bool in = !(x1 < 0 || x1 >= g.W || y1 < 0 || y1 >= g.H) && !(x2 < 0 || x2 >= g.W || y2 < 0 || y2 >= g.H);
+            g1v[k] = -1;
+            g2v[k] = 0;
+            if (in) {
+              g1v[k] = (int)pix((size_t)y1 * g.W + x1);
+              g2v[k] = (int)pix((size_t)y2 * g.W + x2);
+            }
+          }
+          double Mn = 0, Mcount = 0;
+#pragma unroll
+          for (int k = 0; k < kSteps; k++) {
+            const double nn = -3.0 + 0.25 * k;
+            const int g1 = g1v[k], g2 = g2v[k];
+            if (g1 < g2) continue;
+            const double weight = (double)((g2 - g1) * (g2 - g1));
+            Mn += weight * nn;
+            Mcount += weight;
+          }
+          double bx = __longlong_as_double(0x7ff8deadbeef0000ll), by = 0;
+          if (Mcount != 0) {
+            const double n0 = Mn / Mcount;
+            bx = x0 + n0 * nx;
+            by = y0 + n0 * ny;
+            undistort(prm, &bx, &by);
+          }
+          if (t < kLdsRefine) {
+            S.sx[t] = bx;
+            S.sy[t] = by;
+          } else {
+            gsx[t - kLdsRefine] = bx;
+            gsy[t - kLdsRefine] = by;
+          }
+        }
+        team_sync<64>();
+        phase(1);
+        if (tid < 4) {
+          double Mx = 0, My = 0, Mxx = 0, Mxy = 0, Myy = 0, N = 0;
+          const int o = S.samp_off[tid];
+          const int ns = min(S.nsamp[tid], RCAP - o);
+          for (int c = 0; c < ns; c += 8) {
+            double xs[8], ys[8];
+#pragma unroll
+            for (int k = 0; k < 8; k++) {
+              const int i = o + c + k;
+              xs[k] = __longlong_as_double(0x7ff8deadbeef0000ll);
+              ys[k] = 0;
+              if (c + k < ns) {
+                xs[k] = i < kLdsRefine ? S.sx[i] : gsx[i - kLdsRefine];
+                ys[k] = i < kLdsRefine ? S.sy[i] : gsy[i - kLdsRefine];
+              }
+            }
+#pragma unroll
+            for (int k = 0; k < 8; k++) {
+              const double bx = xs[k], by = ys[k];
+              if (isnan(bx)) continue;
+              Mx += bx; My += by; Mxx += bx * bx; Mxy += bx * by; Myy += by * by; N++;
+            }
+          }
+          const double Ex = Mx / N, Ey = My / N;
+          const double Cxx = Mxx / N - Ex * Ex, Cxy = Mxy / N - Ex * Ey, Cyy = Myy / N - Ey * Ey;
+          const double nt = .5 * (double)det_atan2f_call((float)(-2 * Cxy), (float)(Cyy - Cxx));
+          S.lines[tid][0] = Ex;
+          S.lines[tid][1] = Ey;
+          S.lines[tid][2] = (double)det_cosf((float)nt);
+          S.lines[tid][3] = (double)det_sinf((float)nt);
+        }
+        team_sync<64>();
+        phase(2);
+        if (tid == 0) {
+          float qp[4][2];
+          for (int k = 0; k < 4; k++) { qp[k][0] = S.qc[k][0]; qp[k][1] = S.qc[k][1]; }
+          for (int i = 0; i < 4; i++) {
+            const int i1 = (i + 1) & 3;
+            const double A00 = S.lines[i][3], A01 = -S.lines[i1][3];
+            const double A10 = -S.lines[i][2], A11 = S.lines[i1][2];
+            const double B0 = -S.lines[i][0] + S.lines[i1][0];
+            const double B1 = -S.lines[i][1] + S.lines[i1][1];
+            const double det = A00 * A11 - A10 * A01;
+            if (fabs(det) > 0.001) {
+              const double W00 = A11 / det, W01 = -A01 / det;
+              const double L0 = W00 * B0 + W01 * B1;
+              double px = S.lines[i][0] + L0 * A00, py = S.lines[i][1] + L0 * A10;
+              redistort(prm, &px, &py);
+              qp[i1][0] = (float)px;
+              qp[i1][1] = (float)py;
+            }
+          }
+          for (int k = 0; k < 4; k++) { S.qc[k][0] = qp[k][0]; S.qc[k][1] = qp[k][1]; }
+        }
+        team_sync<64>();
+        phase(3);
+      }
+      if (AT_DIAG_STOP(prm, 6)) continue;
+      if (homography_wave(S.qc, S.A, S.H) != 0) continue;
+      if (tid == 0) {
+        const double* H = S.H;
+        const double hdet = H[0] * (H[4] * H[8] - H[5] * H[7]) - H[1] * (H[3] * H[8] - H[5] * H[6]) +
+                            H[2] * (H[3] * H[7] - H[4] * H[6]);
+        S.ok = hdet != 0;
+      }
+      team_sync<64>();
+      phase(4);
+      if (!S.ok) continue;
+      uint32_t seq = 0;
+      if (POSE) {
+        if (tid < 9) P.H[tid] = S.H[tid];
+        if (tid < 4) {
+          const int tcx = (tid == 1 || tid == 2) ? 1 : -1, tcy = tid < 2 ? 1 : -1;
+          hproject(S.H, tcx, tcy, &P.p[tid][0], &P.p[tid][1]);
+        }
+        seq = ++pose_seq;
+        team_sync<64>();
+        if (tid == 0) __hip_atomic_store(&P.seq, seq, __ATOMIC_RELEASE, __HIP_MEMORY_SCOPE_WORKGROUP);
+      }
+      uint32_t bc = 0xffffffffu;
+      double margin_d = -1;
+      do {
+      const int wab = prm.fam.width_at_border, tw = prm.fam.total_width, nbits = prm.fam.nbits;
+      const int minc = (wab - tw) / 2;
+      {
+        const int pidx = tid >> 3, i = tid & 7;
+        float p0, p1, p2, p3;
+        border_pattern(pidx, (float)wab, p0, p1, p2, p3);
+        const double tagx01 = (double)((p0 + (float)i * p2) / (float)wab);
+        const double tagy01 = (double)((p1 + (float)i * p3) / (float)wab);
+        const double tagx = 2 * (tagx01 - 0.5), tagy = 2 * (tagy01 - 0.5);
+        double px, py;
+        hproject(S.H, tagx, tagy, &px, &py);
+        const int ix = (int)px, iy = (int)py;
+        S.gmx[tid] = tagx;
+        S.gmy[tid] = tagy;
+        S.gmvalid[tid] = i < wab && !(ix < 0 || iy < 0 || ix >= g.W || iy >= g.H);
+        S.gmv[tid] = S.gmvalid[tid] ? (double)pix((size_t)iy * g.W + ix) : 0.0;
+      }
+      for (int t = tid; t < tw * tw; t += kDecodeThreads) S.values[t] = 0;
+      team_sync<64>();
+      phase(5);
+      double interp00 = 0;
+      if (tid < 2) {
+        GrayModel m;
+        for (int k = 0; k < 3; k++) {
+          m.B[k] = 0;
+          for (int j = 0; j < 3; j++) m.A[k][j] = 0;
+        }
+        for (int grp = 0; grp < 4; grp++) {
+          const int t0 = 16 * grp + 8 * tid;
+          double xs[8], ys[8], vs[8];
+          int ok[8];
+#pragma unroll
+          for (int i = 0; i < 8; i++) {
+            xs[i] = S.gmx[t0 + i];
+            ys[i] = S.gmy[t0 + i];
+            vs[i] = S.gmv[t0 + i];
+            ok[i] = S.gmvalid[t0 + i];
+          }
+#pragma unroll
+          for (int i = 0; i < 8; i++)
+            if (ok[i]) gm_add(m, xs[i], ys[i], vs[i]);
+        }
+        gm_solve(m);
+        double* C = tid == 0 ? S.wC : S.bC;
+        for (int k = 0; k < 3; k++) C[k] = m.C[k];
+        interp00 = gm_interp(m, 0, 0);
+      }
+      const double w00 = __shfl(interp00, 0), b00 = __shfl(interp00, 1);
+      team_sync<64>();
+      if (w00 - b00 < 0) break;
+      phase(6);
+      if (tid < nbits) {
+        const int bity = prm.fam.bity[tid], bitx = prm.fam.bitx[tid];
+        const double tagx01 = (bitx + 0.5) / wab, tagy01 = (bity + 0.5) / wab;
+        const double tagx = 2 * (tagx01 - 0.5), tagy = 2 * (tagy01 - 0.5);
+        double px, py;
+        hproject(S.H, tagx, tagy, &px, &py);
+        const int x1 = (int)floor(px - 0.5), x2 = (int)ceil(px - 0.5);
+        const double xx = px - 0.5 - x1;
+        const int y1 = (int)floor(py - 0.5), y2 = (int)ceil(py - 0.5);
+        const double yy = py - 0.5 - y1;
+        if (!(x1 < 0 || x2 >= g.W || y1 < 0 || y2 >= g.H)) {
+          const double v = (int)pix((size_t)y1 * g.W + x1) * (1 - xx) * (1 - yy) + (int)pix((size_t)y1 * g.W + x2) * xx * (1 - yy) +
+                           (int)pix((size_t)y2 * g.W + x1) * (1 - xx) * yy + (int)pix((size_t)y2 * g.W + x2) * xx * yy;
+          const double bth = S.bC[0] * tagx + S.bC[1] * tagy + S.bC[2];
+          const double wth = S.wC[0] * tagx + S.wC[1] * tagy + S.wC[2];
+          S.values[tw * (bity - minc) + bitx - minc] = v - (bth + wth) / 2.0;
+        }
+      }
+      team_sync<64>();
+      phase(7);
+      constexpr int kShR = (kMaxTotalWidth * kMaxTotalWidth + kDecodeThreads - 1) / kDecodeThreads;
+      double shv[kShR];
+      int tl = tid;
+      __asm__ volatile("" : "+v"(tl));
+#pragma unroll
+      for (int r = 0; r < kShR; r++) {
+        const int t = tl + 64 * r;
+        shv[r] = 0;
+        if (t < tw * tw) {
+          const int y = t / tw, x = t % tw;
+          const double up = S.values[y > 0 ? t - tw : t], left = S.values[x > 0 ? t - 1 : t], c = S.values[t];
+          const double right = S.values[x < tw - 1 ? t + 1 : t], down = S.values[y < tw - 1 ? t + tw : t];
+          double acc = 0;
+          if (y > 0) acc = acc - up;
+          if (x > 0) acc = acc - left;
+          acc = acc + c * 4;
+          if (x < tw - 1) acc = acc - right;
+          if (y < tw - 1) acc = acc - down;
+          shv[r] = acc;
+        }
+      }
+      team_sync<64>();
+#pragma unroll
+      for (int r = 0; r < kShR; r++) {
+        const int t = tid + 64 * r;
+        if (t < tw * tw) S.values[t] = S.values[t] + prm.decode_sharpening * shv[r];
+      }
+      team_sync<64>();
+      double bitv = 0;
+      if (tid < nbits) bitv = S.values[tw * (prm.fam.bity[tid] - minc) + prm.fam.bitx[tid] - minc];
+      const uint64_t white_bits = __ballot(tid < nbits && bitv > 0);
+      const uint64_t rcode0 = __builtin_bitreverse64(white_bits) >> (64 - nbits);
+      {
+        float black_score = 0, white_score = 0, black_cnt = 1, white_cnt = 1;
+        for (int i = 0; i < nbits; i++) {
+          const double v = readlane_f64(bitv, i);
+          if (v > 0) { white_score = (float)(white_score + v); white_cnt++; }
+          else { black_score = (float)(black_score - v); black_cnt++; }
+        }
+        margin_d = fmin((double)(white_score / white_cnt), (double)(black_score / black_cnt));
+      }
+      phase(8);
+      {
+        uint64_t r[4];
+        r[0] = rcode0;
+#pragma unroll
+        for (int k = 1; k < 4; k++) r[k] = rotate90_n(r[k - 1], nbits);
+        constexpr int kBookChunk = 10;
+        for (int e0 = 0; e0 < prm.fam.ncodes; e0 += kBookChunk * kDecodeThreads) {
+          uint64_t cw[kBookChunk];
+#pragma unroll
+          for (int k = 0; k < kBookChunk; k++) {
+            const int ent = e0 + tid + kDecodeThreads * k;
+            cw[k] = ent < prm.fam.ncodes ? b.book_code[ent] : 0ull;
+          }
+#pragma unroll
+          for (int k = 0; k < kBookChunk; k++) {
+            const int ent = e0 + tid + kDecodeThreads * k;
+#pragma unroll
+            for (int rot = 0; rot < 4; rot++) {
+              const int hd = __popcll(r[rot] ^ cw[k]);
+              if (ent < prm.fam.ncodes && hd <= 2) bc = min(bc, (uint32_t)((rot << 24) | (hd << 16) | ent));
+            }
+          }
+        }
+#pragma unroll
+        for (int d = 32; d > 0; d >>= 1) bc = min(bc, (uint32_t)__shfl_xor(bc, d));
+      }
+      } while (false);
+      if (POSE) {
+        while (__hip_atomic_load(&P.ack, __ATOMIC_ACQUIRE, __HIP_MEMORY_SCOPE_WORKGROUP) != seq)
+          __builtin_amdgcn_s_sleep(1);
+      }
+      if (tid == 0) {
+        const float margin = (float)margin_d;
+        if (margin >= 0 && bc != 0xffffffffu) {
+          const int rot = bc >> 24, hd = (bc >> 16) & 0xff, ent = bc & 0xffff;
+          DevDetection d;
+          d.id = b.book_id[ent];
+          d.hamming = hd;
+          d.decision_margin = margin;
+          d.blob_rank = (int32_t)qrank;
+          const double R[9] = {c_rot_c[rot], -c_rot_s[rot], 0, c_rot_s[rot], c_rot_c[rot], 0, 0, 0, 1};
+          for (int i = 0; i < 3; i++)
+            for (int j = 0; j < 3; j++) {
+              double acc = 0;
+              for (int k = 0; k < 3; k++) acc += S.H[i * 3 + k] * R[k * 3 + j];
+              d.H[i * 3 + j] = acc;
+            }
+          hproject(d.H, 0, 0, &d.c[0], &d.c[1]);
+          for (int i = 0; i < 4; i++) {
+            const int tcx = (i == 1 || i == 2) ? 1 : -1;
+            const int tcy = (i < 2) ? 1 : -1;
+            hproject(d.H, tcx, tcy, &d.p[i][0], &d.p[i][1]);
+          }
+          d.frame = (uint16_t)f;
+          if (POSE) {
+            const int c = rot == 0 ? 1 : rot == 2 ? -1 : 0, sn = rot == 1 ? 1 : rot == 3 ? -1 : 0;
+            for (int i = 0; i < 3; i++) {
+              d.pose_R[i * 3 + 0] = P.R[i * 3 + 0] * c + P.R[i * 3 + 1] * sn;
+              d.pose_R[i * 3 + 1] = -P.R[i * 3 + 0] * sn + P.R[i * 3 + 1] * c;
+              d.pose_R[i * 3 + 2] = P.R[i * 3 + 2];
+            }
+            for (int k = 0; k < 3; k++) d.pose_t[k] = P.t[k];
+            d.pose_err[0] = P.err[0];
+            d.pose_err[1] = P.err[1];
+          }
+          const uint32_t k = atomicAdd(b.ndets + f, 1u);
+          if (k < (uint32_t)kMaxDets) {
+            const uint32_t slot = (uint32_t)f * kMaxDets + k;
+            b.dets[slot] = d;
+            if (k < (uint32_t)kDetPoolPerFrame) b.hdets[(uint32_t)f * kDetPoolPerFrame + k] = d;
+            if (!POSE) b.det_work[atomicAdd(b.det_head, 1u)] = slot;
+          } else {
+            atomicOr(b.status + f, kStatusDetsOverflow);
+          }
+        }
+      }
+      team_sync<64>();
+      phase(9);
+    }
+    probe_flush(b, prm, pacc, 128, tid == 0);
+    if (tid == 0) kt_end(b, 10);
+    if (POSE) {
+      if (tid == 0) __hip_atomic_store(&P.exit, 1u, __ATOMIC_RELEASE, __HIP_MEMORY_SCOPE_WORKGROUP);
+      decode_finish(b, tid, nq);
+    }
   }
 }
 
@@ -5616,7 +6159,9 @@
   tk(10, st, 0);
   {
     const dim3 grd(prm.dec_wg ? std::min(prm.dec_wg, decode_grid(nblobwg, B)) : decode_grid(nblobwg, B));
+    const bool rows = g.ctw == 64 && !pose_fused && prm.dec_lpq != 64;
     if (on(10) && pose_fused) hipLaunchKernelGGL(k_decode<true>, grd, dim3(128), 0, st, b, g, prm, B, fmt);
+    else if (on(10) && rows) hipLaunchKernelGGL((k_decode<false, kDecRowLanes>), grd, dim3(kDecodeThreads), 0, st, b, g, prm, B, fmt);
     else if (on(10)) hipLaunchKernelGGL(k_decode<false>, grd, dim3(kDecodeThreads), 0, st, b, g, prm, B, fmt);
   }
   tk(10, st, 1);
```

After: 156,800, median of 6. 1.05x the previous value.
